# laclouis5/StructureDetector

Measured on AMD Instinct MI355X. Metric: images/sec (train fwd+bwd) and decode us/img at 512x512, higher is better.
Workload: dtype f32

## Files before the change

### include/sdnet_hip.h

```cpp
#ifndef SDNET_HIP_H
#define SDNET_HIP_H

#include <stddef.h>
#include <stdint.h>

#ifdef __cplusplus
extern "C" {
#endif

#define SD_ERR_INVALID   (-1)
#define SD_ERR_WORKSPACE (-2)
#define SD_ERR_ALIGN     (-3)

#define SD_MAX_TOPK 1024

typedef void* sd_stream_t;

int         sd_version(void);
const char* sd_last_error(void);
int         sd_build_flags(void);


int sd_clamped_sigmoid(const float* x, float* y, int64_t n, sd_stream_t stream);

// ... 137 lines not shown
int sd_loss_bwd(const sd_loss_desc* d, const float* out8, const float* grad_out, float* dhead, sd_stream_t stream);



typedef struct sd_conv_desc {
    int B, Hi, Wi, Cin, Ho, Wo, Cout, R, S, stride, pad;
} sd_conv_desc;

size_t sd_conv2d_fwd_workspace_bytes(const sd_conv_desc* d);
int sd_conv2d_fwd(const float* x_nhwc, const float* w_krsc, float* y_nhwc, const sd_conv_desc* d,
                  const float* scale, const float* shift, const float* residual, int res_up2, int relu,
                  void* workspace, size_t workspace_bytes, sd_stream_t stream);
size_t sd_conv2d_stem_fwd_workspace_bytes(const sd_conv_desc* d);
int sd_conv2d_stem_fwd(const float* x_nchw, const float* w_krsc, void* y_nhwc, const sd_conv_desc* d,
                       const float* scale, const float* shift, int relu, int out_bf16, void* workspace,
                       size_t workspace_bytes, sd_stream_t stream);

int    sd_conv2d_fwd_sb_supported(const sd_conv_desc* d, int bf16);
size_t sd_conv2d_fwd_sb_workspace_bytes(const sd_conv_desc* d, int bf16);
size_t sd_conv2d_fwd_sb_state_bytes(const sd_conv_desc* d, int bf16);
int sd_conv2d_fwd_sb(const void* x_nhwc, const void* w_krsc, void* y_nhwc, const sd_conv_desc* d, const float* scale, const float* shift,
                     const void* residual, int res_up2, int relu, int bf16, void* workspace, size_t workspace_bytes, void* state,
                     size_t state_bytes, sd_stream_t stream);

size_t sd_conv2d_stem_fwd_bn_stats_workspace_bytes(const sd_conv_desc* d);
int sd_conv2d_stem_fwd_bn_stats(const float* x_nchw, const float* w, float* y, const sd_conv_desc* d, float eps, float momentum,
                                float* running_mean, float* running_var, float* mean, float* invstd, void* workspace,
                                size_t workspace_bytes, sd_stream_t stream);

size_t sd_conv2d_fwd_bn_stats_workspace_bytes(const sd_conv_desc* d);
int sd_conv2d_fwd_bn_stats(const float* x, const float* w, float* y, const sd_conv_desc* d, float eps, float momentum,
                           float* running_mean, float* running_var, float* mean, float* invstd, void* workspace,
                           size_t workspace_bytes, sd_stream_t stream);
int sd_bn_finalize_scratch_rows(int rows);
int sd_bn_finalize_stats(const float* partial, int rows, int64_t M, int C, float eps, float momentum, float* running_mean,
                         float* running_var, float* mean, float* invstd, float* scratch, sd_stream_t stream);

size_t sd_conv2d_dgrad_bn_reduce_workspace_bytes(const sd_conv_desc* d);
int sd_conv2d_dgrad_bn_reduce(const float* dy, const float* w_t, float* dx, const sd_conv_desc* d, const float* residual,
                              const float* bn_x, const float* bn_y, int relu, const float* mean, const float* invstd,
                              const float* gamma, const float* beta, float* dgamma, float* dbeta, int accumulate,
                              float* means_out, void* workspace, size_t workspace_bytes, sd_stream_t stream);
int sd_bn_bwd_finalize(const float* partial, int rows, int64_t M, int C, float* dgamma, float* dbeta, int accumulate,
                       float* means_out, float* scratch, sd_stream_t stream);
int sd_bn_bwd_apply(const float* dy, const float* x, const float* y, int relu, int64_t M, int C, const float* mean,
                    const float* invstd, const float* gamma, const float* beta, const float* means, float* dx, float* g_out,
                    sd_stream_t stream);

int sd_set_option(const char* name, int value);

const char* sd_conv2d_kernel_name(const sd_conv_desc* d, int pass);

int sd_cast_f32_to_bf16(const float* x, void* y_bf16, int64_t n, sd_stream_t stream);
size_t sd_conv2d_fwd_bf16_workspace_bytes(const sd_conv_desc* d);
int sd_conv2d_fwd_bf16(const void* x_nhwc_bf16, const void* w_krsc_bf16, void* y_nhwc_bf16, const sd_conv_desc* d,
                       const float* scale, const float* shift, const void* residual_bf16, int res_up2, int relu,
                       void* workspace, size_t workspace_bytes, sd_stream_t stream);
int sd_maxpool3x3s2_fwd_bf16(const void* x_bf16, void* y_bf16, int B, int Hi, int Wi, int C, sd_stream_t stream);
int sd_stem_bn_relu_maxpool_fwd_bf16(const float* x_nchw, const float* w, const float* scale, const float* shift, void* y_bf16,
                                     const sd_conv_desc* d, sd_stream_t stream);

int sd_cast_bf16_to_f32(const void* x_bf16, float* y, int64_t n, sd_stream_t stream);
size_t sd_conv2d_fwd_bf16_bn_stats_workspace_bytes(const sd_conv_desc* d);
int sd_conv2d_fwd_bf16_bn_stats(const void* x_nhwc_bf16, const void* w_krsc_bf16, void* y_nhwc_bf16, const sd_conv_desc* d, float eps,
                                float momentum, float* running_mean, float* running_var, float* mean, float* invstd,
                                void* workspace, size_t workspace_bytes, sd_stream_t stream);
int sd_conv2d_stem_fwd_bn_stats_bf16mm(const float* x_nchw, const float* w, float* y, const sd_conv_desc* d, float eps, float momentum,
                                       float* running_mean, float* running_var, float* mean, float* invstd,
                                       void* workspace, size_t workspace_bytes, sd_stream_t stream);
int sd_conv2d_stem_fwd_bn_stats_bf16(const float* x_nchw, const float* w, void* y_bf16, const sd_conv_desc* d, float eps, float momentum,
                                     float* running_mean, float* running_var, float* mean, float* invstd, void* workspace,
                                     size_t workspace_bytes, sd_stream_t stream);
int sd_bn_relu_maxpool_fwd_bf16(const void* x_bf16, int B, int Hi, int Wi, int C, const float* mean, const float* invstd, const float* gamma,
                                const float* beta, void* y_pool_bf16, uint8_t* idx, sd_stream_t stream);
int sd_maxpool_bn_relu_bwd_bf16(const void* dpool_bf16, const uint8_t* idx, const void* x_bf16, int B, int Hi, int Wi, int C, const float* mean,
                                const float* invstd, const float* gamma, const float* beta, float* dx, float* dgamma, float* dbeta, int accumulate,
                                void* workspace, size_t workspace_bytes, sd_stream_t stream);
int sd_maxpool_bn_relu_bwd_bf16_dx16(const void* dpool_bf16, const uint8_t* idx, const void* x_bf16, int B, int Hi, int Wi, int C, const float* mean,
                                     const float* invstd, const float* gamma, const float* beta, void* dx_bf16, float* dgamma, float* dbeta,
                                     int accumulate, void* workspace, size_t workspace_bytes, sd_stream_t stream);
int sd_conv2d_transpose_weights_bf16(const float* w, void* w_t_bf16, int Cout, int taps, int Cin, sd_stream_t stream);

int sd_conv2d_fwd_bf16_head_supported(const sd_conv_desc* d, int head_co);
size_t sd_head_split_bf16_bytes(void);
int sd_head_split_bf16(const float* head_w, const float* head_bias, int head_co, void* prepared, sd_stream_t stream);
int sd_conv2d_fwd_bf16_head(const void* x_bf16, const void* w_bf16, const sd_conv_desc* d, const float* scale, const float* shift, int relu,
                            const void* head_prepared, int head_co, float* head_y, sd_stream_t stream);
int sd_conv2d_dgrad_bf16(const void* dy_bf16, const void* w_t_bf16, void* dx_bf16, const sd_conv_desc* d, const void* residual_bf16,
                         int res_mode, sd_stream_t stream);
size_t sd_conv2d_wgrad_bf16_workspace_bytes(const sd_conv_desc* d);
int sd_conv2d_wgrad_bf16(const void* dy_bf16, const void* x_nhwc_bf16, float* dw_krsc, const sd_conv_desc* d, int accumulate,
                         void* workspace, size_t workspace_bytes, sd_stream_t stream);
int sd_bn_apply_bf16(const void* x, void* y, int64_t M, int C, const float* mean, const float* invstd, const float* gamma,
                     const float* beta, const void* residual, int relu, uint8_t* relu_mask_out, sd_stream_t stream);
int sd_bn_bwd_bf16(const void* dy, const void* x, const void* y, int relu, int64_t M, int C, const float* mean, const float* invstd,
                   const float* gamma, const float* beta, void* dx, void* g_out, float* dgamma, float* dbeta, int accumulate,
                   void* workspace, size_t workspace_bytes, sd_stream_t stream);
int sd_bn_train_stats_bf16(const void* x, int64_t M, int C, float eps, float momentum, float* running_mean, float* running_var,
                           float* mean, float* invstd, void* workspace, size_t workspace_bytes, sd_stream_t stream);
int sd_col_sum_bf16(const void* x, int64_t M, int C, float* out, int accumulate, void* workspace, size_t workspace_bytes, sd_stream_t stream);
int sd_upsample2x_bwd_bf16(const void* dy, const void* add, void* dx, int B, int H, int W, int C, sd_stream_t stream);
int sd_head_fwd_bf16(const void* x_nhwc_bf16, const float* w, const float* bias, float* y_nchw, int B, int HW, int C,
                     int Co, sd_stream_t stream);
int sd_conv2d_dgrad(const float* dy_nhwc, const float* w_t, float* dx_nhwc, const sd_conv_desc* d,
                    const float* residual, sd_stream_t stream);
int sd_conv2d_dgrad_half_res(const float* dy, const float* w_t, float* dx, const sd_conv_desc* d, const float* residual_half,
                             sd_stream_t stream);
int sd_conv2d_transpose_weights(const float* w, float* w_t, int Cout, int taps, int Cin, sd_stream_t stream);
int sd_conv2d_transpose_weights_batched(const float* w_base, void* w_t_base, const int* table, int nconv, int total_blocks, int out_bf16,
                                        sd_stream_t stream);
size_t sd_conv2d_wgrad_workspace_bytes(const sd_conv_desc* d);
int sd_conv2d_wgrad(const float* dy_nhwc, const float* x_nhwc, float* dw_krsc, const sd_conv_desc* d,
                    int accumulate, void* workspace, size_t workspace_bytes, sd_stream_t stream);
size_t sd_conv2d_stem_wgrad_workspace_bytes(const sd_conv_desc* d);
int sd_conv2d_stem_wgrad(const float* dy_nhwc, const float* x_nchw, float* dw_krsc, const sd_conv_desc* d,
                         int accumulate, void* workspace, size_t workspace_bytes, sd_stream_t stream);
int sd_conv2d_stem_wgrad_bf16mm(const float* dy, const float* x_nchw, float* dw, const sd_conv_desc* d, int accumulate, void* workspace,
                                size_t workspace_bytes, sd_stream_t stream);
int sd_conv2d_stem_wgrad_bf16(const void* dy_bf16, const float* x_nchw, float* dw, const sd_conv_desc* d, int accumulate, void* workspace,
                              size_t workspace_bytes, sd_stream_t stream);

size_t sd_col_reduce_workspace_bytes(int64_t M, int C);
int sd_bn_train_stats(const float* x, int64_t M, int C, float eps, float momentum, float* running_mean,
                      float* running_var, float* mean, float* invstd, void* workspace, size_t workspace_bytes,
                      sd_stream_t stream);
int sd_bn_apply(const float* x, float* y, int64_t M, int C, const float* mean, const float* invstd,
                const float* gamma, const float* beta, const float* residual, int relu, uint8_t* relu_mask_out,
                sd_stream_t stream);
int sd_bn_fold(const float* gamma, const float* beta, const float* running_mean, const float* running_var,
               float eps, int C, float* scale, float* shift, sd_stream_t stream);
int sd_bn_bwd(const float* dy, const float* x, const float* y, int relu, int64_t M, int C, const float* mean,
              const float* invstd, const float* gamma, const float* beta, float* dx, float* g_out, float* dgamma,
              float* dbeta, int accumulate, void* workspace, size_t workspace_bytes, sd_stream_t stream);
int sd_col_sum(const float* x, int64_t M, int C, float* out, int accumulate, void* workspace,
               size_t workspace_bytes, sd_stream_t stream);

int sd_maxpool3x3s2_fwd(const float* x, float* y, uint8_t* idx, int B, int Hi, int Wi, int C, sd_stream_t stream);
int sd_maxpool3x3s2_bwd(const float* dy, const uint8_t* idx, float* dx, int B, int Hi, int Wi, int C, sd_stream_t stream);
int sd_bn_relu_maxpool_fwd(const float* x, int B, int Hi, int Wi, int C, const float* mean, const float* invstd, const float* gamma,
                           const float* beta, float* y_pool, uint8_t* idx, sd_stream_t stream);
int sd_maxpool_bn_relu_bwd(const float* dpool, const uint8_t* idx, const float* x, int B, int Hi, int Wi, int C, const float* mean,
                           const float* invstd, const float* gamma, const float* beta, float* dx, float* dgamma, float* dbeta,
                           int accumulate, void* workspace, size_t workspace_bytes, sd_stream_t stream);
int sd_upsample2x_bwd(const float* dy, const float* add, float* dx, int B, int H, int W, int C, sd_stream_t stream);

#define SD_HEAD_MAX_CO 256
int sd_head_fwd(const float* x_nhwc, const float* w, const float* bias, float* y_nchw, int B, int HW, int C, int Co,
                sd_stream_t stream);
size_t sd_head_bwd_workspace_bytes(int B, int HW, int C, int Co);
int sd_head_bwd(const float* dy_nchw, const float* x_nhwc, const float* w, float* dx_nhwc, float* dw, float* dbias,
                int B, int HW, int C, int Co, int accumulate, void* workspace, size_t workspace_bytes, sd_stream_t stream);
int sd_head_bwd_bf16(const float* dy, const void* x_bf16, const float* w, void* dx_bf16, float* dw, float* dbias, int B, int HW, int C, int Co,
                     int accumulate, void* workspace, size_t workspace_bytes, sd_stream_t stream);

int sd_adam_step(float* param, const float* grad, float* exp_avg, float* exp_avg_sq, int64_t n, int step,
                 float lr, float beta1, float beta2, float eps, float grad_scale, sd_stream_t stream);

#define SD_OPTIM_STATUS_BYTES 16
size_t sd_grad_sumsq_workspace_bytes(int64_t n);
int sd_grad_sumsq(const float* grad, int64_t n, void* workspace, size_t workspace_bytes, sd_stream_t stream);
int sd_optim_step(float* param, const float* grad, float* exp_avg, float* exp_avg_sq, int64_t n, int step,
                  float lr, float beta1, float beta2, float eps, float grad_scale, float weight_decay,
                  const uint8_t* decay_mask, float max_norm, const void* partials, int npartials, float* ema,
                  float ema_decay, void* status, sd_stream_t stream);

#define SD_COMM_ID_BYTES 128
int sd_allreduce_unique_id(void* id_out);
int sd_allreduce_init(const void* id, int rank, int world, void** comm_out);
int sd_allreduce_run(void* comm, float* buf, int64_t count, sd_stream_t stream);
int sd_allreduce_destroy(void* comm);

int sd_comm_sim_copy(const void* src, void* dst, size_t src_bytes, size_t move_bytes, int workgroups, float gbps, sd_stream_t stream);

double sd_mfma_bf16_stream_flops(int iters);
int    sd_mfma_bf16_stream(const void* operands64k, float* out, int iters, sd_stream_t stream);

int sd_bn_stats_from_sums(const double* sums, int C, float eps, float momentum, float* running_mean, float* running_var, float* mean,
                          float* invstd, sd_stream_t stream);
int sd_bn_bwd_means_from_sums(const double* sums, int C, float* means_out, sd_stream_t stream);
int sd_bn_stats_sums(const float* partial, int rows, int64_t M, int C, double* sums, float* scratch, sd_stream_t stream);
int sd_bn_bwd_sums(const float* partial, int rows, int64_t M, int C, float* dgamma, float* dbeta, int accumulate, double* sums,
                   float* scratch, sd_stream_t stream);
int sd_bn_train_sums(const float* x, int64_t M, int C, double* sums, void* workspace, size_t workspace_bytes, sd_stream_t stream);
int sd_bn_train_sums_bf16(const void* x, int64_t M, int C, double* sums, void* workspace, size_t workspace_bytes, sd_stream_t stream);
int sd_conv2d_fwd_bn_stats_rows(const sd_conv_desc* d, int bf16);
int sd_conv2d_fwd_bn_sums(const float* x, const float* w, float* y, const sd_conv_desc* d, double* sums, void* workspace,
                          size_t workspace_bytes, sd_stream_t stream);
int sd_conv2d_fwd_bf16_bn_sums(const void* x, const void* w, void* y, const sd_conv_desc* d, double* sums, void* workspace,
                               size_t workspace_bytes, sd_stream_t stream);
int sd_conv2d_stem_fwd_bn_sums(const float* x_nchw, const float* w, float* y, const sd_conv_desc* d, double* sums, void* workspace,
                               size_t workspace_bytes, sd_stream_t stream);
int sd_conv2d_stem_fwd_bn_sums_bf16mm(const float* x_nchw, const float* w, float* y, const sd_conv_desc* d, double* sums, void* workspace,
                                      size_t workspace_bytes, sd_stream_t stream);
int sd_conv2d_stem_fwd_bn_sums_bf16(const float* x_nchw, const float* w, void* y_bf16, const sd_conv_desc* d, double* sums, void* workspace,
                                    size_t workspace_bytes, sd_stream_t stream);
int sd_conv2d_dgrad_bn_reduce_sums(const float* dy, const float* w_t, float* dx, const sd_conv_desc* d, const float* residual,
                                   const float* bn_x, const float* bn_y, int relu, const float* mean, const float* invstd,
                                   const float* gamma, const float* beta, float* dgamma, float* dbeta, int accumulate,
                                   double* sums, void* workspace, size_t workspace_bytes, sd_stream_t stream);
int sd_bn_bwd_reduce(const float* dy, const float* x, const float* y, int relu, int64_t M, int C, const float* mean, const float* invstd,
                     const float* gamma, const float* beta, float* dgamma, float* dbeta, int accumulate, double* sums, void* workspace,
                     size_t workspace_bytes, sd_stream_t stream);
int sd_bn_bwd_reduce_bf16(const void* dy, const void* x, const void* y, int relu, int64_t M, int C, const float* mean, const float* invstd,
                          const float* gamma, const float* beta, float* dgamma, float* dbeta, int accumulate, double* sums, void* workspace,
                          size_t workspace_bytes, sd_stream_t stream);
int sd_bn_bwd_apply_bf16(const void* dy, const void* x, const void* y, int relu, int64_t M, int C, const float* mean, const float* invstd,
                         const float* gamma, const float* beta, const float* means, void* dx, void* g_out, sd_stream_t stream);
int sd_maxpool_bn_relu_bwd_reduce(const float* dpool, const uint8_t* idx, const float* x, int B, int Hi, int Wi, int C, const float* mean,
                                  const float* invstd, const float* gamma, const float* beta, float* dgamma, float* dbeta, int accumulate,
                                  double* sums, void* workspace, size_t workspace_bytes, sd_stream_t stream);
int sd_maxpool_bn_relu_bwd_reduce_bf16(const void* dpool_bf16, const uint8_t* idx, const void* x_bf16, int B, int Hi, int Wi, int C,
                                       const float* mean, const float* invstd, const float* gamma, const float* beta, float* dgamma,
                                       float* dbeta, int accumulate, double* sums, void* workspace, size_t workspace_bytes, sd_stream_t stream);
int sd_maxpool_bn_relu_bwd_apply(const float* dpool, const uint8_t* idx, const float* x, int B, int Hi, int Wi, int C, const float* mean,
                                 const float* invstd, const float* gamma, const float* beta, const float* means, float* dx, sd_stream_t stream);
int sd_maxpool_bn_relu_bwd_apply_bf16(const void* dpool_bf16, const uint8_t* idx, const void* x_bf16, int B, int Hi, int Wi, int C,
                                      const float* mean, const float* invstd, const float* gamma, const float* beta, const float* means, float* dx,
                                      sd_stream_t stream);
int sd_maxpool_bn_relu_bwd_apply_bf16_dx16(const void* dpool_bf16, const uint8_t* idx, const void* x_bf16, int B, int Hi, int Wi, int C,
                                           const float* mean, const float* invstd, const float* gamma, const float* beta, const float* means,
                                           void* dx_bf16, sd_stream_t stream);

int         sd_range_enabled(void);
const char* sd_range_library(void);
int         sd_range_push(const char* name);
int         sd_range_pop(void);
int         sd_range_mark(const char* name);

#ifdef __cplusplus
}
#endif
#endif
```

### structuredetector_amd/_lib.py

```python
from __future__ import annotations

import ctypes as C
import os
from pathlib import Path

import torch

_HERE = Path(__file__).resolve().parent
LIB_PATH = Path(os.environ.get("SDNET_HIP_LIB", _HERE / "csrc" / "libsdnet_hip.so"))

_lib = None

c_f32p = C.c_void_p
c_i64 = C.c_int64
c_int = C.c_int
c_float = C.c_float
c_size = C.c_size_t
c_vp = C.c_void_p


class SdError(RuntimeError):
    pass


class LossDesc(C.Structure):
    _fields_ = [
        ("anchor_hm", c_vp), ("a_sb", c_i64), ("a_sc", c_i64),
        ("part_hm", c_vp), ("p_sb", c_i64), ("p_sc", c_i64),
        ("offsets", c_vp), ("o_sb", c_i64), ("o_sc", c_i64),
        ("embeddings", c_vp), ("e_sb", c_i64), ("e_sc", c_i64),
        ("t_anchor_hm", c_vp), ("ta_sb", c_i64), ("ta_sc", c_i64),
        ("t_part_hm", c_vp), ("tp_sb", c_i64), ("tp_sc", c_i64),
        ("anchor_inds", c_vp), ("part_inds", c_vp),
        ("anchor_offsets", c_vp), ("part_offsets", c_vp), ("t_embeddings", c_vp),
        ("anchor_mask", c_vp), ("part_mask", c_vp),
        ("B", c_int), ("M", c_int), ("N", c_int), ("h", c_int), ("w", c_int), ("K", c_int), ("P", c_int),
        ("hm_loss_fn", c_int),
        ("hm_weight", c_float), ("offset_weight", c_float), ("embedding_weight", c_float),
    ]


class ConvDesc(C.Structure):
    _fields_ = [(n, c_int) for n in ("B", "Hi", "Wi", "Cin", "Ho", "Wo", "Cout", "R", "S", "stride", "pad")]


_MAP = [c_vp, c_i64, c_i64]
_PEAK_OUT = [c_vp, c_vp, c_vp, c_vp, c_vp]

_SIGNATURES = {
    "sd_version": (c_int, []),
    "sd_last_error": (C.c_char_p, []),
    "sd_build_flags": (c_int, []),
    "sd_clamped_sigmoid": (c_int, [c_vp, c_vp, c_i64, c_vp]),
    "sd_nms5": (c_int, _MAP + [c_vp, c_int, c_int, c_int, c_int, c_int, c_vp]),
    "sd_topk_workspace_bytes": (c_size, [c_int] * 5),
    "sd_topk": (c_int, _MAP + [c_int] * 5 + _PEAK_OUT + [c_vp, c_size, c_vp]),
    "sd_transpose_and_gather": (c_int, _MAP + [c_int, c_int, c_i64, c_vp, c_int, c_vp, c_vp]),
    "sd_hypot": (c_int, [c_vp, c_vp, c_i64, c_vp]),
    "sd_decode_peaks_workspace_bytes": (c_size, [c_int] * 5),
    "sd_decode_peaks": (c_int, _MAP + [c_int] * 5 + _PEAK_OUT + [c_vp, c_size, c_vp]),
    "sd_decode_workspace_bytes": (c_size, [c_int] * 7),
    "sd_decode_packed_words": (c_size, [c_int] * 3),
    "sd_decode": (c_int, _MAP * 4 + [c_int] * 7 + [c_float, c_float, c_int, c_vp, c_vp, c_size, c_vp]),
    "sd_decode_state_bytes": (c_size, [c_int] * 5),
    "sd_decode_fused_supported": (c_int, [c_int] * 7),
    "sd_decode_fused_recommended": (c_int, [c_int] * 8),
    "sd_stream_synchronize": (c_int, [c_vp]),
    "sd_selfcheck_sigmoid": (c_int, [c_vp, c_vp]),
    "sd_decode_fused_workspace_bytes": (c_size, [c_int] * 7),
    "sd_decode_fused": (c_int, _MAP * 4 + [c_int] * 7 + [c_float, c_float, c_int, c_vp, c_vp, c_size, c_vp, c_size, c_vp]),
    "sd_decode_group": (c_int, [c_vp] * 6 + _MAP * 2 + [c_int] * 5 + [c_float, c_float, c_vp, c_vp]),
    "sd_tta_views": (c_int, [c_vp, c_vp, c_int, c_int, c_int, c_int, c_vp, c_vp]),
    "sd_tta_merge_nms": (c_int, _MAP + [c_vp, c_int, c_int, c_int, c_int, c_int, c_vp, c_vp]),
    "sd_tta_scale_merge_nms": (c_int, [c_vp] * 6 + [c_int] * 6 + [c_vp, c_vp]),
    "sd_preprocess_workspace_bytes": (c_size, [c_int] * 4),
    "sd_preprocess_images": (c_int, [c_vp] + [c_int] * 5 + [c_vp, c_vp, c_int, c_vp, c_vp, c_int, c_vp, C.POINTER(c_float), C.POINTER(c_float),
                                                c_vp, c_vp, c_size, c_vp]),
    "sd_preprocess_jitter_workspace_bytes": (c_size, [c_int] * 5),
    "sd_preprocess_images_jitter": (c_int, [c_vp] + [c_int] * 5 + [c_vp, c_vp, c_int, c_vp, c_vp, c_int, c_vp, c_vp, c_vp, C.POINTER(c_float), C.POINTER(c_float),
                                            c_vp, c_vp, c_size, c_vp]),
    "sd_preprocess_images_list": (c_int, [c_vp] + [c_int] * 5 + [c_vp, c_vp, c_int, c_vp, c_vp, c_int, c_vp, C.POINTER(c_float), C.POINTER(c_float),
                                                     c_vp, c_vp, c_size, c_vp]),
    "sd_preprocess_images_list_jitter": (c_int, [c_vp] + [c_int] * 5 + [c_vp, c_vp, c_int, c_vp, c_vp, c_int, c_vp, c_vp, c_vp, C.POINTER(c_float),
                                                            C.POINTER(c_float), c_vp, c_vp, c_size, c_vp]),
    "sd_preprocess_affine_workspace_bytes": (c_size, [c_int] * 5),
    "sd_preprocess_images_affine": (c_int, [c_vp] + [c_int] * 5 + [c_vp, c_vp, c_int, c_vp, c_vp, c_int, c_vp, c_vp, c_vp, c_vp, C.POINTER(C.c_ubyte),
                                            C.POINTER(c_float), C.POINTER(c_float), c_vp, c_vp, c_size, c_vp]),
    "sd_preprocess_images_list_affine": (c_int, [c_vp] + [c_int] * 5 + [c_vp, c_vp, c_int, c_vp, c_vp, c_int, c_vp, c_vp, c_vp, c_vp, C.POINTER(C.c_ubyte),
                                                 C.POINTER(c_float), C.POINTER(c_float), c_vp, c_vp, c_size, c_vp]),
    "sd_preprocess_mosaic_workspace_bytes": (c_size, [c_int] * 5),
    "sd_preprocess_images_mosaic": (c_int, [c_vp] + [c_int] * 5 + [c_vp, c_vp, c_int, c_vp, c_vp, c_int, c_vp, c_vp, c_vp, c_vp, c_vp, c_vp,
                                            C.POINTER(C.c_ubyte), C.POINTER(c_float), C.POINTER(c_float), c_vp, c_vp, c_size, c_vp]),
    "sd_preprocess_images_list_mosaic": (c_int, [c_vp] + [c_int] * 5 + [c_vp, c_vp, c_int, c_vp, c_vp, c_int, c_vp, c_vp, c_vp, c_vp, c_vp, c_vp,
                                                 C.POINTER(C.c_ubyte), C.POINTER(c_float), C.POINTER(c_float), c_vp, c_vp, c_size, c_vp]),
    "sd_render_targets": (c_int, [c_vp, c_vp, c_vp, c_int, c_int, c_int, c_int, c_float, c_vp, c_vp]),
    "sd_loss_workspace_bytes": (c_size, [c_int] * 5),
    "sd_loss_fwd": (c_int, [C.POINTER(LossDesc), c_vp, c_vp, c_size, c_vp]),
    "sd_loss_fwd_per_image": (c_int, [C.POINTER(LossDesc), c_vp, c_vp, c_size, c_vp]),
    "sd_loss_bwd": (c_int, [C.POINTER(LossDesc), c_vp, c_vp, c_vp, c_vp]),
    "sd_conv2d_fwd_workspace_bytes": (c_size, [C.POINTER(ConvDesc)]),
    "sd_conv2d_fwd": (c_int, [c_vp, c_vp, c_vp, C.POINTER(ConvDesc), c_vp, c_vp, c_vp, c_int, c_int, c_vp, c_size, c_vp]),
    "sd_conv2d_fwd_sb_supported": (c_int, [C.POINTER(ConvDesc), c_int]),
    "sd_conv2d_fwd_sb_workspace_bytes": (c_size, [C.POINTER(ConvDesc), c_int]),
    "sd_conv2d_fwd_sb_state_bytes": (c_size, [C.POINTER(ConvDesc), c_int]),
    "sd_conv2d_fwd_sb": (c_int, [c_vp, c_vp, c_vp, C.POINTER(ConvDesc), c_vp, c_vp, c_vp, c_int, c_int, c_int, c_vp, c_size, c_vp, c_size, c_vp]),
    "sd_conv2d_stem_fwd_workspace_bytes": (c_size, [C.POINTER(ConvDesc)]),
    "sd_conv2d_stem_fwd": (c_int, [c_vp, c_vp, c_vp, C.POINTER(ConvDesc), c_vp, c_vp, c_int, c_int, c_vp, c_size, c_vp]),
    "sd_cast_f32_to_bf16": (c_int, [c_vp, c_vp, c_i64, c_vp]),
    "sd_conv2d_fwd_bf16_workspace_bytes": (c_size, [C.POINTER(ConvDesc)]),
    "sd_conv2d_fwd_bf16": (c_int, [c_vp, c_vp, c_vp, C.POINTER(ConvDesc), c_vp, c_vp, c_vp, c_int, c_int, c_vp, c_size, c_vp]),
    "sd_conv2d_fwd_bf16_head_supported": (c_int, [C.POINTER(ConvDesc), c_int]),
    "sd_head_split_bf16_bytes": (c_size, []),
    "sd_head_split_bf16": (c_int, [c_vp, c_vp, c_int, c_vp, c_vp]),
    "sd_conv2d_fwd_bf16_head": (c_int, [c_vp, c_vp, C.POINTER(ConvDesc), c_vp, c_vp, c_int, c_vp, c_int, c_vp, c_vp]),
    "sd_cast_bf16_to_f32": (c_int, [c_vp, c_vp, c_i64, c_vp]),
    "sd_conv2d_fwd_bf16_bn_stats_workspace_bytes": (c_size, [c_vp]),
    "sd_conv2d_fwd_bf16_bn_stats": (c_int, [c_vp, c_vp, c_vp, c_vp, c_float, c_float, c_vp, c_vp, c_vp, c_vp, c_vp, c_size, c_vp]),
    "sd_conv2d_wgrad_bf16_workspace_bytes": (c_size, [c_vp]),
    "sd_conv2d_wgrad_bf16": (c_int, [c_vp, c_vp, c_vp, c_vp, c_int, c_vp, c_size, c_vp]),
    "sd_conv2d_transpose_weights_bf16": (c_int, [c_vp, c_vp, c_int, c_int, c_int, c_vp]),
    "sd_conv2d_dgrad_bf16": (c_int, [c_vp, c_vp, c_vp, c_vp, c_vp, c_int, c_vp]),
    "sd_bn_apply_bf16": (c_int, [c_vp, c_vp, c_i64, c_int, c_vp, c_vp, c_vp, c_vp, c_vp, c_int, c_vp, c_vp]),
    "sd_bn_bwd_bf16": (c_int, [c_vp, c_vp, c_vp, c_int, c_i64, c_int, c_vp, c_vp, c_vp, c_vp, c_vp, c_vp, c_vp, c_vp, c_int, c_vp, c_size, c_vp]),
    "sd_bn_train_stats_bf16": (c_int, [c_vp, c_i64, c_int, c_float, c_float, c_vp, c_vp, c_vp, c_vp, c_vp, c_size, c_vp]),
    "sd_col_sum_bf16": (c_int, [c_vp, c_i64, c_int, c_vp, c_int, c_vp, c_size, c_vp]),
    "sd_upsample2x_bwd_bf16": (c_int, [c_vp, c_vp, c_vp, c_int, c_int, c_int, c_int, c_vp]),
    "sd_maxpool3x3s2_fwd_bf16": (c_int, [c_vp, c_vp, c_int, c_int, c_int, c_int, c_vp]),
    "sd_stem_bn_relu_maxpool_fwd_bf16": (c_int, [c_vp, c_vp, c_vp, c_vp, c_vp, c_vp, c_vp]),
    "sd_head_fwd_bf16": (c_int, [c_vp, c_vp, c_vp, c_vp, c_int, c_int, c_int, c_int, c_vp]),
    "sd_conv2d_dgrad": (c_int, [c_vp, c_vp, c_vp, C.POINTER(ConvDesc), c_vp, c_vp]),
    "sd_conv2d_transpose_weights": (c_int, [c_vp, c_vp, c_int, c_int, c_int, c_vp]),
    "sd_conv2d_transpose_weights_batched": (c_int, [c_vp, c_vp, c_vp, c_int, c_int, c_int, c_vp]),
    "sd_conv2d_wgrad_workspace_bytes": (c_size, [C.POINTER(ConvDesc)]),
    "sd_conv2d_wgrad": (c_int, [c_vp, c_vp, c_vp, C.POINTER(ConvDesc), c_int, c_vp, c_size, c_vp]),
    "sd_conv2d_stem_wgrad_workspace_bytes": (c_size, [C.POINTER(ConvDesc)]),
    "sd_conv2d_stem_wgrad": (c_int, [c_vp, c_vp, c_vp, C.POINTER(ConvDesc), c_int, c_vp, c_size, c_vp]),
    "sd_conv2d_stem_wgrad_bf16mm": (c_int, [c_vp, c_vp, c_vp, C.POINTER(ConvDesc), c_int, c_vp, c_size, c_vp]),
    "sd_conv2d_stem_wgrad_bf16": (c_int, [c_vp, c_vp, c_vp, C.POINTER(ConvDesc), c_int, c_vp, c_size, c_vp]),
    "sd_col_reduce_workspace_bytes": (c_size, [c_i64, c_int]),
    "sd_bn_train_stats": (c_int, [c_vp, c_i64, c_int, c_float, c_float, c_vp, c_vp, c_vp, c_vp, c_vp, c_size, c_vp]),
    "sd_bn_apply": (c_int, [c_vp, c_vp, c_i64, c_int, c_vp, c_vp, c_vp, c_vp, c_vp, c_int, c_vp, c_vp]),
    "sd_bn_fold": (c_int, [c_vp, c_vp, c_vp, c_vp, c_float, c_int, c_vp, c_vp, c_vp]),
    "sd_bn_bwd": (c_int, [c_vp, c_vp, c_vp, c_int, c_i64, c_int, c_vp, c_vp, c_vp, c_vp, c_vp, c_vp, c_vp, c_vp, c_int, c_vp, c_size, c_vp]),
    "sd_col_sum": (c_int, [c_vp, c_i64, c_int, c_vp, c_int, c_vp, c_size, c_vp]),
    "sd_maxpool3x3s2_fwd": (c_int, [c_vp, c_vp, c_vp, c_int, c_int, c_int, c_int, c_vp]),
    "sd_maxpool3x3s2_bwd": (c_int, [c_vp, c_vp, c_vp, c_int, c_int, c_int, c_int, c_vp]),
    "sd_upsample2x_bwd": (c_int, [c_vp, c_vp, c_vp, c_int, c_int, c_int, c_int, c_vp]),
    "sd_head_fwd": (c_int, [c_vp, c_vp, c_vp, c_vp, c_int, c_int, c_int, c_int, c_vp]),
    "sd_head_bwd_workspace_bytes": (c_size, [c_int] * 4),
    "sd_head_bwd": (c_int, [c_vp] * 6 + [c_int] * 5 + [c_vp, c_size, c_vp]),
    "sd_head_bwd_bf16": (c_int, [c_vp] * 6 + [c_int] * 5 + [c_vp, c_size, c_vp]),
    "sd_adam_step": (c_int, [c_vp, c_vp, c_vp, c_vp, c_i64, c_int, c_float, c_float, c_float, c_float, c_float, c_vp]),
    "sd_grad_sumsq_workspace_bytes": (c_size, [c_i64]),
    "sd_grad_sumsq": (c_int, [c_vp, c_i64, c_vp, c_size, c_vp]),
    "sd_optim_step": (c_int, [c_vp, c_vp, c_vp, c_vp, c_i64, c_int, c_float, c_float, c_float, c_float, c_float, c_float, c_vp, c_float, c_vp, c_int,
                              c_vp, c_float, c_vp, c_vp]),
    "sd_conv2d_kernel_name": (C.c_char_p, [c_vp, c_int]),
    "sd_set_option": (c_int, [C.c_char_p, c_int]),
    "sd_decode_set_option": (c_int, [C.c_char_p, c_int]),
    "sd_decode_kernel_names": (C.c_char_p, [c_int] * 9),
    "sd_conv2d_stem_fwd_bn_stats_workspace_bytes": (c_size, [c_vp]),
    "sd_conv2d_stem_fwd_bn_stats": (c_int, [c_vp, c_vp, c_vp, c_vp, c_float, c_float, c_vp, c_vp, c_vp, c_vp, c_vp, c_size, c_vp]),
    "sd_conv2d_stem_fwd_bn_stats_bf16mm": (c_int, [c_vp, c_vp, c_vp, c_vp, c_float, c_float, c_vp, c_vp, c_vp, c_vp, c_vp, c_size, c_vp]),
    "sd_conv2d_stem_fwd_bn_stats_bf16": (c_int, [c_vp, c_vp, c_vp, c_vp, c_float, c_float, c_vp, c_vp, c_vp, c_vp, c_vp, c_size, c_vp]),
    "sd_conv2d_dgrad_half_res": (c_int, [c_vp] * 6),
    "sd_bn_relu_maxpool_fwd": (c_int, [c_vp, c_int, c_int, c_int, c_int] + [c_vp] * 7),
    "sd_bn_relu_maxpool_fwd_bf16": (c_int, [c_vp, c_int, c_int, c_int, c_int] + [c_vp] * 7),
    "sd_maxpool_bn_relu_bwd": (c_int, [c_vp, c_vp, c_vp, c_int, c_int, c_int, c_int] + [c_vp] * 7 + [c_int, c_vp, c_size, c_vp]),
    "sd_maxpool_bn_relu_bwd_bf16": (c_int, [c_vp, c_vp, c_vp, c_int, c_int, c_int, c_int] + [c_vp] * 7 + [c_int, c_vp, c_size, c_vp]),
    "sd_maxpool_bn_relu_bwd_bf16_dx16": (c_int, [c_vp, c_vp, c_vp, c_int, c_int, c_int, c_int] + [c_vp] * 7 + [c_int, c_vp, c_size, c_vp]),
    "sd_conv2d_fwd_bn_stats_workspace_bytes": (c_size, [c_vp]),
    "sd_conv2d_fwd_bn_stats": (c_int, [c_vp, c_vp, c_vp, c_vp, c_float, c_float, c_vp, c_vp, c_vp, c_vp, c_vp, c_size, c_vp]),
    "sd_conv2d_dgrad_bn_reduce_workspace_bytes": (c_size, [c_vp]),
    "sd_conv2d_dgrad_bn_reduce": (c_int, [c_vp] * 5 + [c_vp, c_vp, c_int] + [c_vp] * 6 + [c_int, c_vp, c_vp, c_size, c_vp]),
    "sd_bn_bwd_finalize": (c_int, [c_vp, c_int, c_i64, c_int, c_vp, c_vp, c_int, c_vp, c_vp, c_vp]),
    "sd_bn_bwd_apply": (c_int, [c_vp, c_vp, c_vp, c_int, c_i64, c_int] + [c_vp] * 8),
    "sd_bn_finalize_scratch_rows": (c_int, [c_int]),
    "sd_bn_finalize_stats": (c_int, [c_vp, c_int, c_i64, c_int, c_float, c_float, c_vp, c_vp, c_vp, c_vp, c_vp, c_vp]),
    "sd_bn_stats_from_sums": (c_int, [c_vp, c_int, c_float, c_float, c_vp, c_vp, c_vp, c_vp, c_vp]),
    "sd_bn_bwd_means_from_sums": (c_int, [c_vp, c_int, c_vp, c_vp]),
    "sd_bn_stats_sums": (c_int, [c_vp, c_int, c_i64, c_int, c_vp, c_vp, c_vp]),
    "sd_bn_bwd_sums": (c_int, [c_vp, c_int, c_i64, c_int, c_vp, c_vp, c_int, c_vp, c_vp, c_vp]),
    "sd_bn_train_sums": (c_int, [c_vp, c_i64, c_int, c_vp, c_vp, c_size, c_vp]),
    "sd_bn_train_sums_bf16": (c_int, [c_vp, c_i64, c_int, c_vp, c_vp, c_size, c_vp]),
    "sd_conv2d_fwd_bn_stats_rows": (c_int, [c_vp, c_int]),
    "sd_conv2d_fwd_bn_sums": (c_int, [c_vp, c_vp, c_vp, c_vp, c_vp, c_vp, c_size, c_vp]),
    "sd_conv2d_fwd_bf16_bn_sums": (c_int, [c_vp, c_vp, c_vp, c_vp, c_vp, c_vp, c_size, c_vp]),
    "sd_conv2d_stem_fwd_bn_sums": (c_int, [c_vp, c_vp, c_vp, c_vp, c_vp, c_vp, c_size, c_vp]),
    "sd_conv2d_stem_fwd_bn_sums_bf16mm": (c_int, [c_vp, c_vp, c_vp, c_vp, c_vp, c_vp, c_size, c_vp]),
    "sd_conv2d_stem_fwd_bn_sums_bf16": (c_int, [c_vp, c_vp, c_vp, c_vp, c_vp, c_vp, c_size, c_vp]),
    "sd_conv2d_dgrad_bn_reduce_sums": (c_int, [c_vp, c_vp, c_vp, c_vp, c_vp, c_vp, c_vp, c_int] + [c_vp] * 6 + [c_int, c_vp, c_vp, c_size, c_vp]),
    "sd_bn_bwd_reduce": (c_int, [c_vp, c_vp, c_vp, c_int, c_i64, c_int] + [c_vp] * 6 + [c_int, c_vp, c_vp, c_size, c_vp]),
    "sd_bn_bwd_reduce_bf16": (c_int, [c_vp, c_vp, c_vp, c_int, c_i64, c_int] + [c_vp] * 6 + [c_int, c_vp, c_vp, c_size, c_vp]),
    "sd_bn_bwd_apply_bf16": (c_int, [c_vp, c_vp, c_vp, c_int, c_i64, c_int] + [c_vp] * 8),
    "sd_maxpool_bn_relu_bwd_reduce": (c_int, [c_vp, c_vp, c_vp, c_int, c_int, c_int, c_int] + [c_vp] * 6 + [c_int, c_vp, c_vp, c_size, c_vp]),
    "sd_maxpool_bn_relu_bwd_reduce_bf16": (c_int, [c_vp, c_vp, c_vp, c_int, c_int, c_int, c_int] + [c_vp] * 6 + [c_int, c_vp, c_vp, c_size, c_vp]),
    "sd_maxpool_bn_relu_bwd_apply": (c_int, [c_vp, c_vp, c_vp, c_int, c_int, c_int, c_int] + [c_vp] * 7),
    "sd_maxpool_bn_relu_bwd_apply_bf16": (c_int, [c_vp, c_vp, c_vp, c_int, c_int, c_int, c_int] + [c_vp] * 7),
    "sd_maxpool_bn_relu_bwd_apply_bf16_dx16": (c_int, [c_vp, c_vp, c_vp, c_int, c_int, c_int, c_int] + [c_vp] * 7),
    "sd_allreduce_unique_id": (c_int, [c_vp]),
    "sd_allreduce_init": (c_int, [c_vp, c_int, c_int, C.POINTER(c_vp)]),
    "sd_allreduce_run": (c_int, [c_vp, c_vp, c_i64, c_vp]),
    "sd_allreduce_destroy": (c_int, [c_vp]),
    "sd_mfma_bf16_stream_flops": (C.c_double, [c_int]),
    "sd_mfma_bf16_stream": (c_int, [c_vp, c_vp, c_int, c_vp]),
    "sd_comm_sim_copy": (c_int, [c_vp, c_vp, c_size, c_size, c_int, c_float, c_vp]),
    "sd_range_enabled": (c_int, []),
    "sd_range_library": (C.c_char_p, []),
    "sd_range_push": (c_int, [C.c_char_p]),
    "sd_range_pop": (c_int, []),
    "sd_range_mark": (c_int, [C.c_char_p]),
}


def declared_symbols():
    return sorted(_SIGNATURES)


def lib():
    global _lib
    if _lib is None:
        if not LIB_PATH.exists():
            raise SdError(
                f"{LIB_PATH} not found: build it with `python -c 'import __graft_entry__ as g; g.build()'` "
                f"(or `make -C {LIB_PATH.parent}`); structuredetector_amd has no CPU / eager fallback.")
        handle = C.CDLL(str(LIB_PATH))
        for name, (res, args) in _SIGNATURES.items():
            fn = getattr(handle, name)
            fn.restype = res
            fn.argtypes = args
        flags = handle.sd_build_flags()
        if flags and os.environ.get("SDNET_ALLOW_ABLATION") != "1":
            raise SdError(f"{LIB_PATH} is a timing-only ablation build (sd_build_flags = {flags}: SD_ABLATE_* switches make the conv "
                          "kernels compute wrong results on purpose); rebuild without EXTRA=-DSD_ABLATE_... "
                          "(set SDNET_ALLOW_ABLATION=1 only for timing experiments)")
        _lib = handle
    return _lib


def check(rc: int, what: str = ""):
    if rc != 0:
        msg = lib().sd_last_error().decode(errors="replace")
        raise SdError(f"{what or 'libsdnet_hip'} failed (code {rc}): {msg}")


def stream() -> int:
    try:
        return torch._C._cuda_getCurrentRawStream(torch.cuda.current_device())
    except AttributeError:
        return torch.cuda.current_stream().cuda_stream


def require_cuda(*tensors):
    for t in tensors:
        if not t.is_cuda:
            raise SdError("structuredetector_amd ops need tensors on the GPU (device 'cuda'); got a "
                          f"{t.device} tensor and there is no CPU fallback")


def map_view(t: torch.Tensor):
    if t.dtype != torch.float32:
        t = t.float()
    B, Cc, h, w = t.shape
    s0, s1, s2, s3 = t.stride()
    ptr = t.data_ptr()
    if not (s3 == 1 and s2 == w and s1 >= h * w and (B == 1 or s0 >= h * w) and s1 % 4 == 0 and s0 % 4 == 0 and ptr % 16 == 0):
        t = t.contiguous()
        s0, s1 = t.stride(0), t.stride(1)
        ptr = t.data_ptr()
    return t, ptr, s0, s1


_ws_cache: dict = {}


def workspace(nbytes: int, device) -> torch.Tensor:
    key = (device.index if device.index is not None else torch.cuda.current_device(), stream())
    buf = _ws_cache.get(key)
    if buf is None or buf.numel() < nbytes:
        buf = torch.empty(max(nbytes, 1 << 20), dtype=torch.uint8, device=device)
        _ws_cache[key] = buf
    return buf


_state_cache: dict = {}


def zero_state(nbytes: int, device, tag: str = "conv") -> torch.Tensor:
    key = (device.index if device.index is not None else torch.cuda.current_device(), stream(), tag)
    buf = _state_cache.get(key)
    if buf is None or buf.numel() < nbytes:
        if buf is not None:
            torch.cuda.current_stream().synchronize()
        buf = torch.zeros(max(nbytes, 1 << 16), dtype=torch.uint8, device=device)
        _state_cache[key] = buf
    return buf
```

### structuredetector_amd/csrc/sd_nn.hip

```cpp
#include "sd_common.h"
#include "sd_mfma.h"
#include <type_traits>

namespace sd {

constexpr int RED_ROWS_PER_BLOCK = 256;

template <int MODE, typename T = float>
__global__ __launch_bounds__(256) void k_col_reduce(const T* __restrict__ a, const T* __restrict__ b, const T* __restrict__ y,
                                                     const float* __restrict__ mean, const float* __restrict__ invstd,
                                                     const float* __restrict__ gamma, const float* __restrict__ beta, int relu,
                                                     int64_t M, int C, float* __restrict__ partial, int rpb) {
    __shared__ float4 red[2][256];
    const int cols = C >> 2;
    const int lanes = 256 / cols;
    const int col = threadIdx.x % cols, rl = threadIdx.x / cols;
    const int64_t r0 = (int64_t)blockIdx.x * rpb;
    const int64_t r1 = min(r0 + rpb, M);
    float4 s0 = make_float4(0.f, 0.f, 0.f, 0.f), s1 = s0;
    float4 mu = s0, is = s0, ga = s0, be = s0;
    if (MODE == 1 && rl < lanes) {
        mu = reinterpret_cast<const float4*>(mean)[col];
        is = reinterpret_cast<const float4*>(invstd)[col];
        if (relu == 2) { ga = reinterpret_cast<const float4*>(gamma)[col]; be = reinterpret_cast<const float4*>(beta)[col]; }
    }
    if (rl < lanes) {
#pragma unroll 4
        for (int64_t r = r0 + rl; r < r1; r += lanes) {
            const float4 v = ld4(a, r * cols + col);
            if (MODE == 0) {
                s0.x += v.x; s0.y += v.y; s0.z += v.z; s0.w += v.w;
                s1.x += v.x * v.x; s1.y += v.y * v.y; s1.z += v.z * v.z; s1.w += v.w * v.w;
            } else if (MODE == 2) {
                s0.x += v.x; s0.y += v.y; s0.z += v.z; s0.w += v.w;
            } else {
                float4 g = v;
                const float4 xv = ld4(b, r * cols + col);
                if (relu == 1) {
                    const float4 yy = ld4(y, r * cols + col);
                    g.x = yy.x > 0.f ? g.x : 0.f; g.y = yy.y > 0.f ? g.y : 0.f;
                    g.z = yy.z > 0.f ? g.z : 0.f; g.w = yy.w > 0.f ? g.w : 0.f;
                } else if (relu == 2) {
                    g.x = ((xv.x - mu.x) * is.x * ga.x + be.x) > 0.f ? g.x : 0.f; g.y = ((xv.y - mu.y) * is.y * ga.y + be.y) > 0.f ? g.y : 0.f;
                    g.z = ((xv.z - mu.z) * is.z * ga.z + be.z) > 0.f ? g.z : 0.f; g.w = ((xv.w - mu.w) * is.w * ga.w + be.w) > 0.f ? g.w : 0.f;
                } else if (relu == 3) {
                    const uint8_t mb = reinterpret_cast<const uint8_t*>(y)[r * cols + col];
                    g.x = (mb & 1) ? g.x : 0.f; g.y = (mb & 2) ? g.y : 0.f; g.z = (mb & 4) ? g.z : 0.f; g.w = (mb & 8) ? g.w : 0.f;
                }
                s0.x += g.x; s0.y += g.y; s0.z += g.z; s0.w += g.w;
                s1.x += g.x * ((xv.x - mu.x) * is.x); s1.y += g.y * ((xv.y - mu.y) * is.y);
                s1.z += g.z * ((xv.z - mu.z) * is.z); s1.w += g.w * ((xv.w - mu.w) * is.w);
            }
        }
    }
    red[0][threadIdx.x] = s0;
    red[1][threadIdx.x] = s1;
    __syncthreads();
    if (rl == 0) {
        for (int l = 1; l < lanes; ++l) {
            const float4 u = red[0][l * cols + col], w = red[1][l * cols + col];
            s0.x += u.x; s0.y += u.y; s0.z += u.z; s0.w += u.w;
            s1.x += w.x; s1.y += w.y; s1.z += w.z; s1.w += w.w;
        }
        float* dst = partial + (int64_t)blockIdx.x * 2 * C;
        reinterpret_cast<float4*>(dst)[col] = s0;
        reinterpret_cast<float4*>(dst + C)[col] = s1;
    }
}

__global__ __launch_bounds__(256) void k_rows_fold(const float* __restrict__ in, int rows, int W, int slab, float* __restrict__ out) {
    __shared__ float4 red[256];
    const int cols = W >> 2, lanes = 256 / cols;
    const int col = threadIdx.x % cols, rl = threadIdx.x / cols;
    const int r0 = blockIdx.x * slab, r1 = min(r0 + slab, rows);
    float4 s = make_float4(0.f, 0.f, 0.f, 0.f);
    if (rl < lanes) {
#pragma unroll 4
        for (int r = r0 + rl; r < r1; r += lanes) {
            const float4 v = reinterpret_cast<const float4*>(in + (int64_t)r * W)[col];
            s.x += v.x; s.y += v.y; s.z += v.z; s.w += v.w;
        }
    }
    red[threadIdx.x] = s;
    __syncthreads();
    if (rl == 0) {
        for (int l = 1; l < lanes; ++l) { const float4 u = red[l * cols + col]; s.x += u.x; s.y += u.y; s.z += u.z; s.w += u.w; }
        reinterpret_cast<float4*>(out + (int64_t)blockIdx.x * W)[col] = s;
    }
}

__device__ __forceinline__ bool col_pair_sums(const float* __restrict__ partial, int nblocks, int C, double (&r0)[4][4], double (&r1)[4][4],
                                              double& s0, double& s1) {
    const int lc = threadIdx.x & 3, lr = threadIdx.x >> 2;
    const int c = blockIdx.x * 4 + lc;
    s0 = 0.0; s1 = 0.0;
    if (c < C) {
        double t0[8] = {0, 0, 0, 0, 0, 0, 0, 0}, t1[8] = {0, 0, 0, 0, 0, 0, 0, 0};
        for (int b = lr; b < nblocks; b += 64 * 8) {
            float v0[8], v1[8];
#pragma unroll
            for (int u = 0; u < 8; ++u) {
                const int row = b + 64 * u;
                const int64_t o = (int64_t)(row < nblocks ? row : 0) * 2 * C + c;
                v0[u] = partial[o];
                v1[u] = partial[o + C];
            }
#pragma unroll
            for (int u = 0; u < 8; ++u) {
                const bool ok = b + 64 * u < nblocks;
                t0[u] += ok ? (double)v0[u] : 0.0; t1[u] += ok ? (double)v1[u] : 0.0;
            }
        }
        s0 = ((t0[0] + t0[1]) + (t0[2] + t0[3])) + ((t0[4] + t0[5]) + (t0[6] + t0[7]));
        s1 = ((t1[0] + t1[1]) + (t1[2] + t1[3])) + ((t1[4] + t1[5]) + (t1[6] + t1[7]));
    }
#pragma unroll
    for (int o = 4; o < 64; o <<= 1) { s0 += __shfl_xor(s0, o); s1 += __shfl_xor(s1, o); }
    if ((threadIdx.x & 63) < 4) { r0[threadIdx.x >> 6][lc] = s0; r1[threadIdx.x >> 6][lc] = s1; }
    __syncthreads();
    if (lr != 0 || c >= C) return false;
    s0 = (r0[0][lc] + r0[1][lc]) + (r0[2][lc] + r0[3][lc]);
    s1 = (r1[0][lc] + r1[1][lc]) + (r1[2][lc] + r1[3][lc]);
    return true;
}

__device__ __forceinline__ void bn_stats_tail(double s0, double s1, double M, float eps, float momentum, int c, float* __restrict__ mean_out,
                                              float* __restrict__ invstd_out, float* __restrict__ run_mean, float* __restrict__ run_var) {
    const double mean = s0 / M;
    const double var = fmax(s1 / M - mean * mean, 0.0);
    mean_out[c] = (float)mean;
    invstd_out[c] = (float)(1.0 / sqrt(var + (double)eps));
    if (run_mean) {
        const double unb = M > 1.0 ? var * M / (M - 1.0) : var;
        run_mean[c] = (float)((1.0 - momentum) * run_mean[c] + momentum * mean);
        run_var[c] = (float)((1.0 - momentum) * run_var[c] + momentum * unb);
    }
}

template <int FIN>
__global__ __launch_bounds__(256) void k_col_finalize(const float* __restrict__ partial, int nblocks, int C, double M, float eps,
                                                       float momentum, float* __restrict__ out0, float* __restrict__ out1,
                                                       float* __restrict__ run_mean, float* __restrict__ run_var,
                                                       float* __restrict__ aux0, float* __restrict__ aux1, int accumulate) {
    __shared__ double r0[4][4], r1[4][4];
    double s0, s1;
    if (!col_pair_sums(partial, nblocks, C, r0, r1, s0, s1)) return;
    const int c = blockIdx.x * 4 + (threadIdx.x & 3);
    if (FIN == 0) {
        bn_stats_tail(s0, s1, M, eps, momentum, c, out0, out1, run_mean, run_var);
    } else if (FIN == 1) {
        out0[c] = (accumulate ? out0[c] : 0.f) + (float)s1;
        out1[c] = (accumulate ? out1[c] : 0.f) + (float)s0;
        aux0[c] = (float)(s0 / M);
        aux1[c] = (float)(s1 / M);
    } else {
        out0[c] = (accumulate ? out0[c] : 0.f) + (float)s0;
    }
}

template <int FIN>
__global__ __launch_bounds__(256) void k_col_sums(const float* __restrict__ partial, int nblocks, int C, double M, float* __restrict__ dgamma,
                                                   float* __restrict__ dbeta, int accumulate, double* __restrict__ sums) {
    __shared__ double r0[4][4], r1[4][4];
    double s0, s1;
    if (!col_pair_sums(partial, nblocks, C, r0, r1, s0, s1)) return;
    const int c = blockIdx.x * 4 + (threadIdx.x & 3);
    sums[c] = s0;
    sums[C + c] = s1;
    if (c == 0) sums[2 * C] = M;
    if (FIN == 1) {
        dgamma[c] = (accumulate ? dgamma[c] : 0.f) + (float)s1;
        dbeta[c] = (accumulate ? dbeta[c] : 0.f) + (float)s0;
    }
}

__global__ __launch_bounds__(256) void k_bn_stats_from_sums(const double* __restrict__ sums, int C, float eps, float momentum,
                                                             float* __restrict__ mean, float* __restrict__ invstd,
                                                             float* __restrict__ run_mean, float* __restrict__ run_var) {
    const int c = blockIdx.x * 256 + threadIdx.x;
    if (c >= C) return;
    bn_stats_tail(sums[c], sums[C + c], sums[2 * C], eps, momentum, c, mean, invstd, run_mean, run_var);
}

__global__ __launch_bounds__(256) void k_bn_bwd_means_from_sums(const double* __restrict__ sums, int C, float* __restrict__ means) {
    const int c = blockIdx.x * 256 + threadIdx.x;
    if (c >= C) return;
    const double M = sums[2 * C];
    means[c] = (float)(sums[c] / M);
    means[C + c] = (float)(sums[C + c] / M);
}

template <typename T>
__global__ __launch_bounds__(256) void k_bn_apply(const T* __restrict__ x, T* __restrict__ y, int64_t n4, int C,
                                                   const float* __restrict__ mean, const float* __restrict__ invstd,
                                                   const float* __restrict__ gamma, const float* __restrict__ beta,
                                                   const T* __restrict__ res, int relu, uint8_t* __restrict__ mask) {
    const int64_t stride = (int64_t)gridDim.x * 256;
    const int cols = C >> 2;
    const bool fixed = stride % cols == 0;
    const int col0 = (int)(((int64_t)blockIdx.x * 256 + threadIdx.x) % cols);
    float4 mu = reinterpret_cast<const float4*>(mean)[col0], is = reinterpret_cast<const float4*>(invstd)[col0];
    float4 g = reinterpret_cast<const float4*>(gamma)[col0], b = reinterpret_cast<const float4*>(beta)[col0];
    for (int64_t i = (int64_t)blockIdx.x * 256 + threadIdx.x; i < n4; i += stride) {
        const float4 v = ld4(x, i);
        if (!fixed) {
            const int col = (int)(i % cols);
            mu = reinterpret_cast<const float4*>(mean)[col]; is = reinterpret_cast<const float4*>(invstd)[col];
            g = reinterpret_cast<const float4*>(gamma)[col]; b = reinterpret_cast<const float4*>(beta)[col];
        }
        float4 o;
        o.x = (v.x - mu.x) * is.x * g.x + b.x; o.y = (v.y - mu.y) * is.y * g.y + b.y;
        o.z = (v.z - mu.z) * is.z * g.z + b.z; o.w = (v.w - mu.w) * is.w * g.w + b.w;
        if (res) {
            const float4 r = ld4(res, i);
            o.x += r.x; o.y += r.y; o.z += r.z; o.w += r.w;
        }
        if (mask) mask[i] = (uint8_t)((o.x > 0.f ? 1 : 0) | (o.y > 0.f ? 2 : 0) | (o.z > 0.f ? 4 : 0) | (o.w > 0.f ? 8 : 0));
        if (relu) { o.x = fmaxf(o.x, 0.f); o.y = fmaxf(o.y, 0.f); o.z = fmaxf(o.z, 0.f); o.w = fmaxf(o.w, 0.f); }
        st4(y, i, o);
    }
}

__global__ __launch_bounds__(256) void k_bn_fold(const float* gamma, const float* beta, const float* rm, const float* rv, float eps,
                                                  int C, float* scale, float* shift) {
    const int c = blockIdx.x * 256 + threadIdx.x;
    if (c >= C) return;
    const float s = gamma[c] / sqrtf(rv[c] + eps);
    scale[c] = s;
    shift[c] = beta[c] - rm[c] * s;
}

template <typename T>
__global__ __launch_bounds__(256) void k_bn_bwd_apply(const T* __restrict__ dy, const T* __restrict__ x, const T* __restrict__ y,
                                                       int relu, int64_t n4, int C, const float* __restrict__ mean,
                                                       const float* __restrict__ invstd, const float* __restrict__ gamma,
                                                       const float* __restrict__ beta, const float* __restrict__ mg,
                                                       const float* __restrict__ mgx, T* __restrict__ dx, T* __restrict__ g_out) {
    const int64_t stride = (int64_t)gridDim.x * 256;
    const int cols = C >> 2;
    const bool fixed = stride % cols == 0;
    const int col0 = (int)(((int64_t)blockIdx.x * 256 + threadIdx.x) % cols);
    float4 mu = reinterpret_cast<const float4*>(mean)[col0], is = reinterpret_cast<const float4*>(invstd)[col0];
    float4 ga = reinterpret_cast<const float4*>(gamma)[col0];
    float4 be = relu == 2 ? reinterpret_cast<const float4*>(beta)[col0] : make_float4(0.f, 0.f, 0.f, 0.f);
    float4 a = reinterpret_cast<const float4*>(mg)[col0], b = reinterpret_cast<const float4*>(mgx)[col0];
    for (int64_t i = (int64_t)blockIdx.x * 256 + threadIdx.x; i < n4; i += stride) {
        float4 g = ld4(dy, i);
        const float4 xv = ld4(x, i);
        if (!fixed) {
            const int col = (int)(i % cols);
            mu = reinterpret_cast<const float4*>(mean)[col]; is = reinterpret_cast<const float4*>(invstd)[col];
            ga = reinterpret_cast<const float4*>(gamma)[col];
            if (relu == 2) be = reinterpret_cast<const float4*>(beta)[col];
            a = reinterpret_cast<const float4*>(mg)[col]; b = reinterpret_cast<const float4*>(mgx)[col];
        }
        if (relu == 1) {
            const float4 yy = ld4(y, i);
            g.x = yy.x > 0.f ? g.x : 0.f; g.y = yy.y > 0.f ? g.y : 0.f; g.z = yy.z > 0.f ? g.z : 0.f; g.w = yy.w > 0.f ? g.w : 0.f;
        } else if (relu == 3) {
            const uint8_t mb = reinterpret_cast<const uint8_t*>(y)[i];
            g.x = (mb & 1) ? g.x : 0.f; g.y = (mb & 2) ? g.y : 0.f; g.z = (mb & 4) ? g.z : 0.f; g.w = (mb & 8) ? g.w : 0.f;
        } else if (relu == 2) {
            g.x = ((xv.x - mu.x) * is.x * ga.x + be.x) > 0.f ? g.x : 0.f; g.y = ((xv.y - mu.y) * is.y * ga.y + be.y) > 0.f ? g.y : 0.f;
            g.z = ((xv.z - mu.z) * is.z * ga.z + be.z) > 0.f ? g.z : 0.f; g.w = ((xv.w - mu.w) * is.w * ga.w + be.w) > 0.f ? g.w : 0.f;
        }
        float4 o;
        o.x = ga.x * is.x * (g.x - a.x - (xv.x - mu.x) * is.x * b.x);
        o.y = ga.y * is.y * (g.y - a.y - (xv.y - mu.y) * is.y * b.y);
        o.z = ga.z * is.z * (g.z - a.z - (xv.z - mu.z) * is.z * b.z);
        o.w = ga.w * is.w * (g.w - a.w - (xv.w - mu.w) * is.w * b.w);
        st4(dx, i, o);
        if (g_out) st4(g_out, i, g);
    }
}

__global__ __launch_bounds__(256) void k_maxpool_fwd(const float* __restrict__ x, float* __restrict__ y, uint8_t* __restrict__ idx, int B,
                                                      int Hi, int Wi, int Ho, int Wo, int C) {
    const int cols = C >> 2;
    const int64_t n4 = (int64_t)B * Ho * Wo * cols;
    const int64_t i = (int64_t)blockIdx.x * 256 + threadIdx.x;
    if (i >= n4) return;
    const int col = (int)(i % cols);
    int64_t t = i / cols;
    const int ox = (int)(t % Wo); t /= Wo;
    const int oy = (int)(t % Ho);
    const int b = (int)(t / Ho);
    float4 m = make_float4(-INFINITY, -INFINITY, -INFINITY, -INFINITY);
    uchar4 w = make_uchar4(0, 0, 0, 0);
#pragma unroll
    for (int r = 0; r < 3; ++r) {
#pragma unroll
        for (int s = 0; s < 3; ++s) {
            const int iy = oy * 2 - 1 + r, ix = ox * 2 - 1 + s;
            if (iy < 0 || iy >= Hi || ix < 0 || ix >= Wi) continue;
            const float4 v = reinterpret_cast<const float4*>(x + (((int64_t)b * Hi + iy) * Wi + ix) * C)[col];
            const uint8_t tap = (uint8_t)(r * 3 + s);
            if (v.x > m.x) { m.x = v.x; w.x = tap; }
            if (v.y > m.y) { m.y = v.y; w.y = tap; }
            if (v.z > m.z) { m.z = v.z; w.z = tap; }
            if (v.w > m.w) { m.w = v.w; w.w = tap; }
        }
    }
    reinterpret_cast<float4*>(y)[i] = m;
    reinterpret_cast<uchar4*>(idx)[i] = w;
}

__global__ __launch_bounds__(256) void k_maxpool_bwd(const float* __restrict__ dy, const uint8_t* __restrict__ idx, float* __restrict__ dx,
                                                      int B, int Hi, int Wi, int Ho, int Wo, int C) {
    const int cols = C >> 2;
    const int64_t n4 = (int64_t)B * Hi * Wi * cols;
    const int64_t i = (int64_t)blockIdx.x * 256 + threadIdx.x;
    if (i >= n4) return;
    const int col = (int)(i % cols);
    int64_t t = i / cols;
    const int ix = (int)(t % Wi); t /= Wi;
    const int iy = (int)(t % Hi);
    const int b = (int)(t / Hi);
    float4 acc = make_float4(0.f, 0.f, 0.f, 0.f);
    for (int oy = (iy + 1) / 2 - ((iy + 1) % 2 == 0 ? 1 : 0); oy <= (iy + 1) / 2; ++oy) {
        if (oy < 0 || oy >= Ho) continue;
        const int r = iy - (oy * 2 - 1);
        if (r < 0 || r > 2) continue;
        for (int ox = (ix + 1) / 2 - ((ix + 1) % 2 == 0 ? 1 : 0); ox <= (ix + 1) / 2; ++ox) {
            if (ox < 0 || ox >= Wo) continue;
            const int s = ix - (ox * 2 - 1);
            if (s < 0 || s > 2) continue;
            const int64_t o = (((int64_t)b * Ho + oy) * Wo + ox) * cols + col;
            const uchar4 w = reinterpret_cast<const uchar4*>(idx)[o];
            const float4 g = reinterpret_cast<const float4*>(dy)[o];
            const uint8_t tap = (uint8_t)(r * 3 + s);
            if (w.x == tap) acc.x += g.x;
            if (w.y == tap) acc.y += g.y;
            if (w.z == tap) acc.z += g.z;
            if (w.w == tap) acc.w += g.w;
        }
    }
    reinterpret_cast<float4*>(dx)[i] = acc;
}

template <typename XT, typename PT>
__global__ __launch_bounds__(256) void k_bn_relu_maxpool_fwd(const XT* __restrict__ x, const float* __restrict__ mean,
                                                              const float* __restrict__ invstd, const float* __restrict__ gamma,
                                                              const float* __restrict__ beta, PT* __restrict__ y,
                                                              uint8_t* __restrict__ idx, int B, int Hi, int Wi, int Ho, int Wo, int C) {
    const int cols = C >> 2;
    const int64_t n4 = (int64_t)B * Ho * Wo * cols;
    const int64_t i = (int64_t)blockIdx.x * 256 + threadIdx.x;
    if (i >= n4) return;
    const int col = (int)(i % cols);
    int64_t t = i / cols;
    const int ox = (int)(t % Wo); t /= Wo;
    const int oy = (int)(t % Ho);
    const int b = (int)(t / Ho);
    const float4 mu = reinterpret_cast<const float4*>(mean)[col], is = reinterpret_cast<const float4*>(invstd)[col];
    const float4 ga = reinterpret_cast<const float4*>(gamma)[col], be = reinterpret_cast<const float4*>(beta)[col];
    float4 m = make_float4(-INFINITY, -INFINITY, -INFINITY, -INFINITY);
    uchar4 w = make_uchar4(0, 0, 0, 0);
#pragma unroll
    for (int r = 0; r < 3; ++r) {
#pragma unroll
        for (int s = 0; s < 3; ++s) {
            const int iy = oy * 2 - 1 + r, ix = ox * 2 - 1 + s;
            if (iy < 0 || iy >= Hi || ix < 0 || ix >= Wi) continue;
            const float4 xv = ld4(x, (((int64_t)b * Hi + iy) * Wi + ix) * cols + col);
            float4 v;
            v.x = fmaxf((xv.x - mu.x) * is.x * ga.x + be.x, 0.f); v.y = fmaxf((xv.y - mu.y) * is.y * ga.y + be.y, 0.f);
            v.z = fmaxf((xv.z - mu.z) * is.z * ga.z + be.z, 0.f); v.w = fmaxf((xv.w - mu.w) * is.w * ga.w + be.w, 0.f);
            const uint8_t tap = (uint8_t)(r * 3 + s);
            if (v.x > m.x) { m.x = v.x; w.x = tap; }
            if (v.y > m.y) { m.y = v.y; w.y = tap; }
            if (v.z > m.z) { m.z = v.z; w.z = tap; }
            if (v.w > m.w) { m.w = v.w; w.w = tap; }
        }
    }
    st4(y, i, m);
    reinterpret_cast<uchar4*>(idx)[i] = w;
}

template <int VEC> struct PoolVec { float v[VEC]; };
__device__ __forceinline__ PoolVec<4> pool_ld(const float* p, int64_t e) {
    const float4 r = *reinterpret_cast<const float4*>(p + e);
    return PoolVec<4>{{r.x, r.y, r.z, r.w}};
}
__device__ __forceinline__ PoolVec<8> pool_ld(const uint16_t* p, int64_t e) {
    const uint4 r = *reinterpret_cast<const uint4*>(p + e);
    return PoolVec<8>{{bf16_to_f32((uint16_t)(r.x & 0xffff)), bf16_to_f32((uint16_t)(r.x >> 16)), bf16_to_f32((uint16_t)(r.y & 0xffff)), bf16_to_f32((uint16_t)(r.y >> 16)),
                       bf16_to_f32((uint16_t)(r.z & 0xffff)), bf16_to_f32((uint16_t)(r.z >> 16)), bf16_to_f32((uint16_t)(r.w & 0xffff)), bf16_to_f32((uint16_t)(r.w >> 16))}};
}
__device__ __forceinline__ void pool_st(float* p, int64_t e, const PoolVec<4>& m) { *reinterpret_cast<float4*>(p + e) = make_float4(m.v[0], m.v[1], m.v[2], m.v[3]); }
__device__ __forceinline__ void pool_st(uint16_t* p, int64_t e, const PoolVec<8>& m) {
    uint4 r;
    r.x = (uint32_t)f32_to_bf16(m.v[0]) | ((uint32_t)f32_to_bf16(m.v[1]) << 16); r.y = (uint32_t)f32_to_bf16(m.v[2]) | ((uint32_t)f32_to_bf16(m.v[3]) << 16);
    r.z = (uint32_t)f32_to_bf16(m.v[4]) | ((uint32_t)f32_to_bf16(m.v[5]) << 16); r.w = (uint32_t)f32_to_bf16(m.v[6]) | ((uint32_t)f32_to_bf16(m.v[7]) << 16);
    *reinterpret_cast<uint4*>(p + e) = r;
}
template <typename XT, typename PT, int VEC>
__global__ __launch_bounds__(256) void k_bn_relu_maxpool_fwd_pair(const XT* __restrict__ x, const float* __restrict__ mean,
                                                                   const float* __restrict__ invstd, const float* __restrict__ gamma,
                                                                   const float* __restrict__ beta, PT* __restrict__ y,
                                                                   uint8_t* __restrict__ idx, int B, int Hi, int Wi, int Ho, int Wo, int C) {
    const int cols = C / VEC, Wp = Wo >> 1;
    const int64_t n = (int64_t)B * Ho * Wp * cols;
    const int64_t i = (int64_t)blockIdx.x * 256 + threadIdx.x;
    if (i >= n) return;
    const int col = (int)(i % cols);
    int64_t t = i / cols;
    const int oxp = (int)(t % Wp); t /= Wp;
    const int oy = (int)(t % Ho);
    const int b = (int)(t / Ho);
    float mu[VEC], is[VEC], ga[VEC], be[VEC];
#pragma unroll
    for (int k = 0; k < VEC; ++k) { mu[k] = mean[col * VEC + k]; is[k] = invstd[col * VEC + k]; ga[k] = gamma[col * VEC + k]; be[k] = beta[col * VEC + k]; }
    PoolVec<VEC> m0, m1;
    uint8_t w0[VEC], w1[VEC];
#pragma unroll
    for (int k = 0; k < VEC; ++k) { m0.v[k] = m1.v[k] = -INFINITY; w0[k] = w1[k] = 0; }
#pragma unroll
    for (int r = 0; r < 3; ++r) {
        const int iy = oy * 2 - 1 + r;
        if (iy < 0 || iy >= Hi) continue;
#pragma unroll
        for (int c = 0; c < 5; ++c) {
            const int ix = oxp * 4 - 1 + c;
            if (ix < 0 || ix >= Wi) continue;
            const PoolVec<VEC> xv = pool_ld(x, (((int64_t)b * Hi + iy) * Wi + ix) * C + col * VEC);
#pragma unroll
// ... 144 lines not shown
    const float4 ga = reinterpret_cast<const float4*>(gamma)[col], be = reinterpret_cast<const float4*>(beta)[col];
    const float4 a = reinterpret_cast<const float4*>(mg)[col], bb = reinterpret_cast<const float4*>(mgx)[col];
    const int64_t p00 = (((int64_t)b * Hi + 2 * k) * Wi + 2 * j) * cols + col;
    const int64_t off[4] = {p00, p00 + cols, p00 + (int64_t)Wi * cols, p00 + (int64_t)(Wi + 1) * cols};
    float4 xv[4], g[4];
#pragma unroll
    for (int u = 0; u < 4; ++u) xv[u] = ld4(x, off[u]);
    pool_relu_grad_quad(dpool, idx, b, k, j, col, cols, Ho, Wo, xv, mu, is, ga, be, g);
#pragma unroll
    for (int u = 0; u < 4; ++u) {
        float4 o;
        o.x = ga.x * is.x * (g[u].x - a.x - (xv[u].x - mu.x) * is.x * bb.x);
        o.y = ga.y * is.y * (g[u].y - a.y - (xv[u].y - mu.y) * is.y * bb.y);
        o.z = ga.z * is.z * (g[u].z - a.z - (xv[u].z - mu.z) * is.z * bb.z);
        o.w = ga.w * is.w * (g[u].w - a.w - (xv[u].w - mu.w) * is.w * bb.w);
        st4(dx, off[u], o);
    }
}
#undef SD_ADD4

__global__ __launch_bounds__(256) void k_pool_bn_bwd_reduce(const float* __restrict__ dpool, const uint8_t* __restrict__ idx,
                                                             const float* __restrict__ x, const float* __restrict__ mean,
                                                             const float* __restrict__ invstd, const float* __restrict__ gamma,
                                                             const float* __restrict__ beta, int Hi, int Wi, int Ho, int Wo, int64_t M,
                                                             int C, float* __restrict__ partial) {
    __shared__ float4 red[2][256];
    const int cols = C >> 2, lanes = 256 / cols;
    const int col = threadIdx.x % cols, rl = threadIdx.x / cols;
    const int64_t r0 = (int64_t)blockIdx.x * RED_ROWS_PER_BLOCK, r1 = min(r0 + RED_ROWS_PER_BLOCK, M);
    float4 s0 = make_float4(0.f, 0.f, 0.f, 0.f), s1 = s0;
    if (rl < lanes) {
        const float4 mu = reinterpret_cast<const float4*>(mean)[col], is = reinterpret_cast<const float4*>(invstd)[col];
        const float4 ga = reinterpret_cast<const float4*>(gamma)[col], be = reinterpret_cast<const float4*>(beta)[col];
        for (int64_t r = r0 + rl; r < r1; r += lanes) {
            const int ix = (int)(r % Wi);
            const int64_t t = r / Wi;
            const int iy = (int)(t % Hi), b = (int)(t / Hi);
            const float4 xv = reinterpret_cast<const float4*>(x + r * C)[col];
            const float4 g = pool_relu_grad(dpool, idx, b, iy, ix, col, cols, Ho, Wo, xv, mu, is, ga, be);
            s0.x += g.x; s0.y += g.y; s0.z += g.z; s0.w += g.w;
            s1.x += g.x * ((xv.x - mu.x) * is.x); s1.y += g.y * ((xv.y - mu.y) * is.y);
            s1.z += g.z * ((xv.z - mu.z) * is.z); s1.w += g.w * ((xv.w - mu.w) * is.w);
        }
    }
    red[0][threadIdx.x] = s0;
    red[1][threadIdx.x] = s1;
    __syncthreads();
    if (rl == 0) {
        for (int l = 1; l < lanes; ++l) {
            const float4 u = red[0][l * cols + col], w = red[1][l * cols + col];
            s0.x += u.x; s0.y += u.y; s0.z += u.z; s0.w += u.w;
            s1.x += w.x; s1.y += w.y; s1.z += w.z; s1.w += w.w;
        }
        float* dst = partial + (int64_t)blockIdx.x * 2 * C;
        reinterpret_cast<float4*>(dst)[col] = s0;
        reinterpret_cast<float4*>(dst + C)[col] = s1;
    }
}

__global__ __launch_bounds__(256) void k_pool_bn_bwd_apply(const float* __restrict__ dpool, const uint8_t* __restrict__ idx,
                                                            const float* __restrict__ x, const float* __restrict__ mean,
                                                            const float* __restrict__ invstd, const float* __restrict__ gamma,
                                                            const float* __restrict__ beta, const float* __restrict__ mg,
                                                            const float* __restrict__ mgx, int Hi, int Wi, int Ho, int Wo, int64_t n4, int C,
                                                            float* __restrict__ dx) {
    const int64_t i = (int64_t)blockIdx.x * 256 + threadIdx.x;
    if (i >= n4) return;
    const int cols = C >> 2;
    const int col = (int)(i % cols);
    const int64_t r = i / cols;
    const int ix = (int)(r % Wi);
    const int64_t t = r / Wi;
    const int iy = (int)(t % Hi), b = (int)(t / Hi);
    const float4 mu = reinterpret_cast<const float4*>(mean)[col], is = reinterpret_cast<const float4*>(invstd)[col];
    const float4 ga = reinterpret_cast<const float4*>(gamma)[col], be = reinterpret_cast<const float4*>(beta)[col];
    const float4 xv = reinterpret_cast<const float4*>(x)[i];
    const float4 g = pool_relu_grad(dpool, idx, b, iy, ix, col, cols, Ho, Wo, xv, mu, is, ga, be);
    const float4 a = reinterpret_cast<const float4*>(mg)[col], bb = reinterpret_cast<const float4*>(mgx)[col];
    float4 o;
    o.x = ga.x * is.x * (g.x - a.x - (xv.x - mu.x) * is.x * bb.x);
    o.y = ga.y * is.y * (g.y - a.y - (xv.y - mu.y) * is.y * bb.y);
    o.z = ga.z * is.z * (g.z - a.z - (xv.z - mu.z) * is.z * bb.z);
    o.w = ga.w * is.w * (g.w - a.w - (xv.w - mu.w) * is.w * bb.w);
    reinterpret_cast<float4*>(dx)[i] = o;
}

template <typename T>
__global__ __launch_bounds__(256) void k_up2_bwd(const T* __restrict__ dy, const T* __restrict__ add, T* __restrict__ dx, int B,
                                                  int H, int W, int C) {
    const int cols = C >> 2;
    const int64_t n4 = (int64_t)B * H * W * cols;
    const int64_t i = (int64_t)blockIdx.x * 256 + threadIdx.x;
    if (i >= n4) return;
    const int col = (int)(i % cols);
    int64_t t = i / cols;
    const int x = (int)(t % W); t /= W;
    const int y = (int)(t % H);
    const int b = (int)(t / H);
    const T* base = dy + (((int64_t)b * 2 * H + 2 * y) * 2 * W + 2 * x) * C;
    const float4 v0 = ld4(base, col), v1 = ld4(base + C, col);
    const float4 v2 = ld4(base + (int64_t)2 * W * C, col);
    const float4 v3 = ld4(base + (int64_t)2 * W * C + C, col);
    float4 o = make_float4(v0.x + v1.x + v2.x + v3.x, v0.y + v1.y + v2.y + v3.y, v0.z + v1.z + v2.z + v3.z, v0.w + v1.w + v2.w + v3.w);
    if (add) {
        const float4 a = ld4(add, i);
        o.x += a.x; o.y += a.y; o.z += a.z; o.w += a.w;
    }
    st4(dx, i, o);
}

__global__ __launch_bounds__(256) void k_head_fwd(const float* __restrict__ x, const float* __restrict__ w, const float* __restrict__ bias,
                                                   float* __restrict__ y, int64_t M, int HW, int C, int Co) {
    extern __shared__ __attribute__((aligned(16))) float lds[];
    const int LD = C + 4;
    float* xs = lds;
    float* ws = lds + 64 * LD;
    const int64_t m0 = (int64_t)blockIdx.x * 64;
    const int c4 = C >> 2;
    for (int i = threadIdx.x; i < 64 * c4; i += 256) {
        const int row = i / c4, col = i - row * c4;
        const int64_t m = m0 + row;
        const float4 v = m < M ? reinterpret_cast<const float4*>(x + m * C)[col] : make_float4(0.f, 0.f, 0.f, 0.f);
        *reinterpret_cast<float4*>(xs + row * LD + col * 4) = v;
    }
    for (int i = threadIdx.x; i < Co * C; i += 256) ws[i] = w[i];
    __syncthreads();
    const int px = threadIdx.x & 63, grp = threadIdx.x >> 6;
    float acc[HEAD_NARROW_MAX_CO / 4];
#pragma unroll
    for (int j = 0; j < HEAD_NARROW_MAX_CO / 4; ++j) acc[j] = 0.f;
    for (int c = 0; c < C; c += 4) {
        const float4 v = *reinterpret_cast<const float4*>(xs + px * LD + c);
#pragma unroll
        for (int j = 0; j < HEAD_NARROW_MAX_CO / 4; ++j) {
            const int co = grp + 4 * j;
            if (co < Co) {
                const float4 ww = *reinterpret_cast<const float4*>(ws + co * C + c);
                acc[j] += v.x * ww.x + v.y * ww.y + v.z * ww.z + v.w * ww.w;
            }
        }
    }
    const int64_t m = m0 + px;
    if (m < M) {
        const int64_t b = m / HW, pix = m - b * HW;
#pragma unroll
        for (int j = 0; j < HEAD_NARROW_MAX_CO / 4; ++j) {
            const int co = grp + 4 * j;
            if (co < Co) y[(b * Co + co) * HW + pix] = acc[j] + bias[co];
        }
    }
}

constexpr int HF_NST = 4;
__global__ __launch_bounds__(256) void k_head_fwd_f32_c128(const float* __restrict__ x, const float* __restrict__ w, const float* __restrict__ bias,
                                                            float* __restrict__ y, int HW, int Co, int ntiles) {
    extern __shared__ __attribute__((aligned(16))) float hf_lds[];
    const int lane = threadIdx.x & 63, wave = __builtin_amdgcn_readfirstlane(threadIdx.x >> 6);
    float* const T = hf_lds + wave * (HF_NST * 2048);
    const uint32_t t_base = lds_addr(T);
    const int row = lane & 15, kq = lane >> 4;
    f32x4 bw[8];
#pragma unroll
    for (int j = 0; j < 8; ++j) {
        bw[j] = f32x4{0.f, 0.f, 0.f, 0.f};
        if (row < Co) bw[j] = *reinterpret_cast<const f32x4*>(w + row * 128 + 16 * j + 4 * kq);
    }
    const float bv = row < Co ? bias[row] : 0.f;
    const int nwaves = gridDim.x * 4;
    const int dr = lane >> 5, dsl = lane & 31;
#define HF_ISSUE(t_, st_)                                                                                          \
    {                                                                                                              \
        const int64_t m0_ = (int64_t)min((t_), ntiles - 1) * 16;                                                  \
        _Pragma("unroll") for (int d = 0; d < 8; ++d) {                                                            \
            const int r = 2 * d + dr;                                                                              \
            lds_dma16(x + (m0_ + r) * 128 + ((dsl ^ (r & 15)) << 2), T + (st_) * 2048 + d * 256);                   \
        }                                                                                                          \
    }
    int tile = blockIdx.x * 4 + wave;
#pragma unroll
    for (int s = 0; s < HF_NST - 1; ++s) HF_ISSUE(tile + s * nwaves, s)
    int stage = 0;
    for (; tile < ntiles; tile += nwaves) {
        const int nst = stage == 0 ? HF_NST - 1 : stage - 1;
        HF_ISSUE(tile + (HF_NST - 1) * nwaves, nst)
        wait_vmcnt<8 * (HF_NST - 1)>();
        const uint32_t a0 = t_base + (uint32_t)stage * 8192u + (uint32_t)row * 512u;
        f32x4 a[8];
#pragma unroll
        for (int j = 0; j < 8; ++j) a[j] = lds_read128_async<0>(a0 + (uint32_t)(((4 * j + kq) ^ row) << 4));
        SD_LDS_WAIT4(0, a[0], a[1], a[2], a[3]);
        SD_LDS_WAIT4(0, a[4], a[5], a[6], a[7]);
        f32x4 acc0 = {0.f, 0.f, 0.f, 0.f}, acc1 = {0.f, 0.f, 0.f, 0.f};
#pragma unroll
        for (int j = 0; j < 8; j += 2)
#pragma unroll
            for (int t = 0; t < 4; ++t) {
                acc0 = __builtin_amdgcn_mfma_f32_16x16x4f32(a[j][t], bw[j][t], acc0, 0, 0, 0);
                acc1 = __builtin_amdgcn_mfma_f32_16x16x4f32(a[j + 1][t], bw[j + 1][t], acc1, 0, 0, 0);
            }
        if (row < Co) {
            const uint32_t m0 = (uint32_t)tile * 16u;
            const uint32_t b = m0 / (uint32_t)HW, pix = m0 - b * (uint32_t)HW;
            const f32x4 o = {acc0[0] + acc1[0] + bv, acc0[1] + acc1[1] + bv, acc0[2] + acc1[2] + bv, acc0[3] + acc1[3] + bv};
            *reinterpret_cast<f32x4*>(y + ((int64_t)b * Co + row) * HW + pix + 4 * kq) = o;
        }
        stage = stage + 1 == HF_NST ? 0 : stage + 1;
    }
    wait_vmcnt<0>();
#undef HF_ISSUE
}

constexpr int HEAD_WG_PIX = 1024;
template <typename T>
__global__ __launch_bounds__(256) void k_head_dgrad(const float* __restrict__ dy, const float* __restrict__ w, T* __restrict__ dx,
                                                     int64_t M, int HW, int C, int Co) {
    __shared__ float gs[HEAD_NARROW_MAX_CO][64];
    extern __shared__ __attribute__((aligned(16))) float lds[];
    float* ws = lds;
    const int64_t m0 = (int64_t)blockIdx.x * 64;
    for (int i = threadIdx.x; i < Co * 64; i += 256) {
        const int co = i >> 6, px = i & 63;
        const int64_t m = m0 + px;
        float v = 0.f;
        if (m < M) { const int64_t b = m / HW, pix = m - b * HW; v = dy[(b * Co + co) * HW + pix]; }
        gs[co][px] = v;
    }
    for (int i = threadIdx.x; i < Co * C; i += 256) ws[i] = w[i];
    __syncthreads();
    const int c4 = C >> 2;
    for (int i = threadIdx.x; i < 64 * c4; i += 256) {
        const int row = i / c4, col = i - row * c4;
        const int64_t m = m0 + row;
        if (m >= M) continue;
        float4 o = make_float4(0.f, 0.f, 0.f, 0.f);
        for (int co = 0; co < Co; ++co) {
            const float g = gs[co][row];
            const float4 ww = *reinterpret_cast<const float4*>(ws + co * C + col * 4);
            o.x += g * ww.x; o.y += g * ww.y; o.z += g * ww.z; o.w += g * ww.w;
        }
        if constexpr (sizeof(T) == 2) {
            uint2 pk;
            pk.x = (uint32_t)f32_to_bf16(o.x) | ((uint32_t)f32_to_bf16(o.y) << 16);
            pk.y = (uint32_t)f32_to_bf16(o.z) | ((uint32_t)f32_to_bf16(o.w) << 16);
            reinterpret_cast<uint2*>(dx + m * C)[col] = pk;
        } else {
            reinterpret_cast<float4*>(dx + m * C)[col] = o;
        }
    }
}

template <int CO>
__global__ __launch_bounds__(256) void k_head_wgrad_bf16(const float* __restrict__ dy, const uint16_t* __restrict__ x, float* __restrict__ partial,
                                                          int64_t M, int HW, int C, int Co) {
    __shared__ float gs[CO][64];
    __shared__ float comb[4][CO * 128];
    const int64_t mb = (int64_t)blockIdx.x * HEAD_WG_PIX;
    const int CG = C >> 3, PL = 256 / CG;
    const int cg = threadIdx.x % CG, pl = threadIdx.x / CG;
    float acc[CO][8];
#pragma unroll
    for (int j = 0; j < CO; ++j)
#pragma unroll
        for (int k = 0; k < 8; ++k) acc[j][k] = 0.f;
    float bsum = 0.f;
    for (int64_t m0 = mb; m0 < min(mb + HEAD_WG_PIX, M); m0 += 64) {
        __syncthreads();
        for (int i = threadIdx.x; i < Co * 64; i += 256) {
            const int co = i >> 6, px = i & 63;
            const int64_t m = m0 + px;
            float v = 0.f;
            if (m < M) { const int64_t b = m / HW, pix = m - b * HW; v = dy[(b * Co + co) * HW + pix]; }
            gs[co][px] = v;
        }
        __syncthreads();
        for (int p0 = 0; p0 < 64; p0 += 4 * PL) {
            uint4 xv[4];
#pragma unroll
            for (int u = 0; u < 4; ++u) {
                const int px = p0 + u * PL + pl;
                const int64_t m = m0 + px;
                xv[u] = reinterpret_cast<const uint4*>(x + (px < 64 && m < M ? m : mb) * C)[cg];
            }
#pragma unroll
            for (int u = 0; u < 4; ++u) {
                const int px = p0 + u * PL + pl;
                if (px >= 64) continue;
                const float f[8] = {__uint_as_float(xv[u].x << 16), __uint_as_float(xv[u].x & 0xffff0000u), __uint_as_float(xv[u].y << 16),
                                    __uint_as_float(xv[u].y & 0xffff0000u), __uint_as_float(xv[u].z << 16), __uint_as_float(xv[u].z & 0xffff0000u),
                                    __uint_as_float(xv[u].w << 16), __uint_as_float(xv[u].w & 0xffff0000u)};
#pragma unroll
                for (int j = 0; j < CO; ++j) {
                    if (j < Co) {
                        const float g = gs[j][px];
#pragma unroll
                        for (int k = 0; k < 8; ++k) acc[j][k] += g * f[k];
                    }
                }
            }
        }
        if (threadIdx.x < Co) {
            for (int px = 0; px < 64; ++px) bsum += gs[threadIdx.x][px];
        }
    }
    const int lane = threadIdx.x & 63, wave = threadIdx.x >> 6;
#pragma unroll
    for (int j = 0; j < CO; ++j)
#pragma unroll
        for (int k = 0; k < 8; ++k) {
            float v = acc[j][k];
            for (int o = CG; o < 64; o <<= 1) v += __shfl_xor(v, o);
            acc[j][k] = v;
        }
    if (lane < CG) {
#pragma unroll
        for (int j = 0; j < CO; ++j)
            if (j < Co) {
#pragma unroll
                for (int k = 0; k < 8; ++k) comb[wave][j * C + lane * 8 + k] = acc[j][k];
            }
    }
    __syncthreads();
    float* dst = partial + (int64_t)blockIdx.x * (Co * C + Co);
    for (int i = threadIdx.x; i < Co * C; i += 256) dst[i] = (comb[0][i] + comb[1][i]) + (comb[2][i] + comb[3][i]);
    if (threadIdx.x < Co) dst[Co * C + threadIdx.x] = bsum;
}

__global__ __launch_bounds__(256) void k_head_wgrad(const float* __restrict__ dy, const float* __restrict__ x, float* __restrict__ partial,
                                                     int64_t M, int HW, int C, int Co) {
    __shared__ float gs[HEAD_NARROW_MAX_CO][64];
    __shared__ float comb[HEAD_NARROW_MAX_CO][256];
    const int64_t mb = (int64_t)blockIdx.x * HEAD_WG_PIX;
    const int halves = max(1, 256 / C);
    const int c = threadIdx.x % C, hf = threadIdx.x / C;
    const int span = 64 / halves;
    float acc[HEAD_NARROW_MAX_CO];
#pragma unroll
    for (int j = 0; j < HEAD_NARROW_MAX_CO; ++j) acc[j] = 0.f;
    float bsum = 0.f;
    for (int64_t m0 = mb; m0 < min(mb + HEAD_WG_PIX, M); m0 += 64) {
        __syncthreads();
        for (int i = threadIdx.x; i < Co * 64; i += 256) {
            const int co = i >> 6, px = i & 63;
            const int64_t m = m0 + px;
            float v = 0.f;
            if (m < M) { const int64_t b = m / HW, pix = m - b * HW; v = dy[(b * Co + co) * HW + pix]; }
            gs[co][px] = v;
        }
        __syncthreads();
        if (hf < halves) {
            const int p0 = hf * span;
#pragma unroll 1
            for (int pb = 0; pb < span; pb += 8) {
                float xv[8];
#pragma unroll
                for (int u = 0; u < 8; ++u) {
                    const int64_t m = m0 + p0 + pb + u;
                    xv[u] = x[(m < M ? m : mb) * C + c];
                }
#pragma unroll
                for (int u = 0; u < 8; ++u)
#pragma unroll
                    for (int j = 0; j < HEAD_NARROW_MAX_CO; ++j)
                        if (j < Co) acc[j] += gs[j][p0 + pb + u] * xv[u];
            }
        }
        if (threadIdx.x < Co) {
            for (int px = 0; px < 64; ++px) bsum += gs[threadIdx.x][px];
        }
    }
    for (int j = 0; j < Co; ++j) comb[j][threadIdx.x] = (hf < halves) ? acc[j] : 0.f;
    __syncthreads();
    float* dst = partial + (int64_t)blockIdx.x * (Co * C + Co);
    if (threadIdx.x < C) {
        for (int j = 0; j < Co; ++j) {
            float t = 0.f;
            for (int h2 = 0; h2 < halves; ++h2) t += comb[j][h2 * C + threadIdx.x];
            dst[j * C + threadIdx.x] = t;
        }
    }
    if (threadIdx.x < Co) dst[Co * C + threadIdx.x] = bsum;
}

constexpr int HWG_STAGE = 2048 + 256;
__global__ __launch_bounds__(256) void k_head_wgrad_f32_c128(const float* __restrict__ dy, const float* __restrict__ x, float* __restrict__ partial,
                                                              int HW, int Co, int ntiles) {
    extern __shared__ __attribute__((aligned(16))) float hw_lds[];
    const int lane = threadIdx.x & 63, wave = __builtin_amdgcn_readfirstlane(threadIdx.x >> 6);
    float* const T = hw_lds + wave * (HF_NST * HWG_STAGE);
    const uint32_t t_base = lds_addr(T);
    const int n = lane & 15, kq = lane >> 4;
    const int gw = blockIdx.x * 4 + wave, nwaves = gridDim.x * 4;
    const int dr = lane >> 5, dsl = lane & 31;
    const int nco = min(n, Co - 1);
#define HWG_ISSUE(t_, st_)                                                                                         \
    {                                                                                                              \
        const uint32_t m0_ = (uint32_t)min((t_), ntiles - 1) * 16u;                              \
        const uint32_t b_ = m0_ / (uint32_t)HW, pix_ = m0_ - b_ * (uint32_t)HW;                                     \
        _Pragma("unroll") for (int d = 0; d < 8; ++d) {                                                            \
            const int r = 2 * d + dr;                                                                              \
            lds_dma16(x + ((int64_t)m0_ + r) * 128 + ((dsl ^ (r & 15)) << 2), T + (st_) * HWG_STAGE + d * 256);     \
        }                                                                                                          \
        lds_dma16(dy + ((int64_t)b_ * Co + nco) * HW + pix_ + 4 * kq, T + (st_) * HWG_STAGE + 2048);               \
    }
    f32x4 acc[8];
#pragma unroll
    for (int cb = 0; cb < 8; ++cb) acc[cb] = f32x4{0.f, 0.f, 0.f, 0.f};
    float bsum = 0.f;
    int tile = gw;
#pragma unroll
    for (int s = 0; s < HF_NST - 1; ++s) HWG_ISSUE(tile + s * nwaves, s)
    int stage = 0;
    for (; tile < ntiles; tile += nwaves) {
        const int nst = stage == 0 ? HF_NST - 1 : stage - 1;
        HWG_ISSUE(tile + (HF_NST - 1) * nwaves, nst)
        wait_vmcnt<9 * (HF_NST - 1)>();
        const uint32_t s0 = t_base + (uint32_t)stage * (HWG_STAGE * 4);
        f32x4 a = lds_read128_async<0>(s0 + 8192u + (uint32_t)lane * 16u);
        f32x4 xa[4], xb[4];
#pragma unroll
        for (int i = 0; i < 4; ++i) {
            const uint32_t row = (uint32_t)(4 * kq + i);
            xa[i] = lds_read128_async<0>(s0 + row * 512u + (((uint32_t)n ^ (row & 15u)) << 4));
            xb[i] = lds_read128_async<0>(s0 + row * 512u + (((uint32_t)(16 + n) ^ (row & 15u)) << 4));
        }
        SD_LDS_WAIT4(0, xa[0], xa[1], xa[2], xa[3]);
        SD_LDS_WAIT4(0, xb[0], xb[1], xb[2], xb[3]);
        SD_LDS_WAIT2(0, a, xa[0]);
        if (n >= Co) a = f32x4{0.f, 0.f, 0.f, 0.f};
#pragma unroll
        for (int i = 0; i < 4; ++i)
#pragma unroll
            for (int cb = 0; cb < 4; ++cb) {
                acc[cb] = __builtin_amdgcn_mfma_f32_16x16x4f32(a[i], xa[i][cb], acc[cb], 0, 0, 0);
                acc[4 + cb] = __builtin_amdgcn_mfma_f32_16x16x4f32(a[i], xb[i][cb], acc[4 + cb], 0, 0, 0);
            }
        bsum += (a[0] + a[1]) + (a[2] + a[3]);
        stage = stage + 1 == HF_NST ? 0 : stage + 1;
    }
    wait_vmcnt<0>();
#undef HWG_ISSUE
    float* dst = partial + (int64_t)gw * (Co * 128 + Co);
#pragma unroll
    for (int r = 0; r < 4; ++r) {
        const int co = 4 * kq + r;
        if (co < Co) {
#pragma unroll
            for (int cb = 0; cb < 4; ++cb) { dst[co * 128 + 4 * n + cb] = acc[cb][r]; dst[co * 128 + 64 + 4 * n + cb] = acc[4 + cb][r]; }
        }
    }
    bsum += __shfl_xor(bsum, 16);
    bsum += __shfl_xor(bsum, 32);
    if (kq == 0 && n < Co) dst[Co * 128 + n] = bsum;
}

__global__ __launch_bounds__(256) void k_head_wgrad_fin(const float* __restrict__ partial, int nblocks, int n, float* __restrict__ dw,
                                                         float* __restrict__ db, int nw, int accumulate) {
    __shared__ double red[32][8];
    const int lo = threadIdx.x & 7, lr = threadIdx.x >> 3;
    const int i = blockIdx.x * 8 + lo;
    double s = 0.0;
    if (i < n)
        for (int b = lr; b < nblocks; b += 32) s += (double)partial[(int64_t)b * n + i];
    red[lr][lo] = s;
    __syncthreads();
    if (lr != 0 || i >= n) return;
    for (int k = 1; k < 32; ++k) s += red[k][lo];
    float* dst = i < nw ? dw + i : db + (i - nw);
    *dst = (accumulate ? *dst : 0.f) + (float)s;
}

__global__ __launch_bounds__(256) void k_adam(float* __restrict__ p, const float* __restrict__ g, float* __restrict__ m,
                                               float* __restrict__ v, int64_t n4, float lr, float b1, float b2, float eps, float bc1,
                                               float bc2_sqrt, float gscale) {
    const int64_t stride = (int64_t)gridDim.x * 256;
    for (int64_t i = (int64_t)blockIdx.x * 256 + threadIdx.x; i < n4; i += stride) {
        float4 pp = reinterpret_cast<float4*>(p)[i];
        const float4 gg = reinterpret_cast<const float4*>(g)[i];
        float4 mm = reinterpret_cast<float4*>(m)[i], vv = reinterpret_cast<float4*>(v)[i];
        float* P = &pp.x; const float* G = &gg.x; float* Mo = &mm.x; float* V = &vv.x;
#pragma unroll
        for (int j = 0; j < 4; ++j) {
            const float gr = G[j] * gscale;
            Mo[j] = b1 * Mo[j] + (1.f - b1) * gr;
            V[j] = b2 * V[j] + (1.f - b2) * gr * gr;
            const float denom = sqrtf(V[j]) / bc2_sqrt + eps;
            P[j] -= (lr / bc1) * (Mo[j] / denom);
        }
        reinterpret_cast<float4*>(p)[i] = pp;
        reinterpret_cast<float4*>(m)[i] = mm;
        reinterpret_cast<float4*>(v)[i] = vv;
    }
}

constexpr int SUMSQ_MAX_BLOCKS = 512;

__device__ __forceinline__ double sumsq4(const float4 a) {
    return ((double)a.x * a.x + (double)a.y * a.y) + ((double)a.z * a.z + (double)a.w * a.w);
}

__device__ __forceinline__ double block_sum_256(double s, double* red4) {
    s = wave_sum(s);
    if ((threadIdx.x & 63) == 0) red4[threadIdx.x >> 6] = s;
    __syncthreads();
    return ((red4[0] + red4[1]) + red4[2]) + red4[3];
}

__global__ __launch_bounds__(256) void k_grad_sumsq(const float* __restrict__ g, int64_t n4, double* __restrict__ partial) {
    __shared__ double red[4];
    const int64_t stride = (int64_t)gridDim.x * 256;
    const float4* G = reinterpret_cast<const float4*>(g);
    double s = 0.0;
    for (int64_t i = (int64_t)blockIdx.x * 256 + threadIdx.x; i < n4; i += 8 * stride) {
        float4 a[8];
#pragma unroll
        for (int k = 0; k < 8; ++k) a[k] = G[min(i + k * stride, n4 - 1)];
#pragma unroll
        for (int k = 0; k < 8; ++k) s += i + k * stride < n4 ? sumsq4(a[k]) : 0.0;
    }
    s = block_sum_256(s, red);
    if (threadIdx.x == 0) partial[blockIdx.x] = s;
}

template <bool DECAY, bool CLIP, bool EMA>
__global__ __launch_bounds__(256) void k_optim(float* __restrict__ p, const float* __restrict__ g, float* __restrict__ m,
                                                float* __restrict__ v, int64_t n4, float lr, float b1, float b2, float eps, float bc1,
                                                float bc2_sqrt, float gscale, float decay_mul, const uint8_t* __restrict__ mask,
                                                float max_norm, const double* __restrict__ partial, int npartial,
                                                float* __restrict__ ema, float ema_decay, uint32_t* __restrict__ status) {
    float coef = 1.f;
    if (CLIP) {
        __shared__ double red[4];
        double s = 0.0;
        for (int k = threadIdx.x; k < npartial; k += 256) s += partial[k];
        s = block_sum_256(s, red);
        const float norm = (float)(fabs((double)gscale) * sqrt(s));
        const bool finite = (__float_as_uint(norm) & 0x7f800000u) != 0x7f800000u;
        coef = finite ? fminf(1.f, max_norm / (norm + 1e-6f)) : 0.f;
        if (blockIdx.x == 0 && threadIdx.x == 0) {
            status[0] = __float_as_uint(norm);
            status[1] = __float_as_uint(coef);
            if (!finite) status[2] = status[2] + 1u;
        }
        if (!finite) return;
    }
    const int64_t stride = (int64_t)gridDim.x * 256;
    for (int64_t i = (int64_t)blockIdx.x * 256 + threadIdx.x; i < n4; i += stride) {
        float4 pp = reinterpret_cast<float4*>(p)[i];
        const float4 gg = reinterpret_cast<const float4*>(g)[i];
        float4 mm = reinterpret_cast<float4*>(m)[i], vv = reinterpret_cast<float4*>(v)[i];
        float4 ee = make_float4(0.f, 0.f, 0.f, 0.f);
        if (EMA) ee = reinterpret_cast<float4*>(ema)[i];
        const bool decay = DECAY && (mask == nullptr || mask[i] != 0);
        float* P = &pp.x; const float* G = &gg.x; float* Mo = &mm.x; float* V = &vv.x; float* E = &ee.x;
#pragma unroll
        for (int j = 0; j < 4; ++j) {
            float gr = G[j] * gscale;
            if (CLIP) gr *= coef;
            if (decay) P[j] *= decay_mul;
            Mo[j] = b1 * Mo[j] + (1.f - b1) * gr;
            V[j] = b2 * V[j] + (1.f - b2) * gr * gr;
            const float denom = sqrtf(V[j]) / bc2_sqrt + eps;
            P[j] -= (lr / bc1) * (Mo[j] / denom);
            if (EMA) E[j] = ema_decay * E[j] + (1.f - ema_decay) * P[j];
        }
        reinterpret_cast<float4*>(p)[i] = pp;
        reinterpret_cast<float4*>(m)[i] = mm;
        reinterpret_cast<float4*>(v)[i] = vv;
        if (EMA) reinterpret_cast<float4*>(ema)[i] = ee;
    }
}

__device__ __forceinline__ float bf2f_(uint16_t v) { return __uint_as_float((uint32_t)v << 16); }
__device__ __forceinline__ uint16_t f2bf_(float v) { return __builtin_bit_cast(uint16_t, (__bf16)v); }

__global__ __launch_bounds__(256) void k_cast_bf16(const float* __restrict__ x, uint16_t* __restrict__ y, int64_t n4) {
    const int64_t stride = (int64_t)gridDim.x * 256;
    for (int64_t i = (int64_t)blockIdx.x * 256 + threadIdx.x; i < n4; i += stride) {
        const float4 v = reinterpret_cast<const float4*>(x)[i];
        reinterpret_cast<ushort4*>(y)[i] = make_ushort4(f2bf_(v.x), f2bf_(v.y), f2bf_(v.z), f2bf_(v.w));
    }
}

__global__ __launch_bounds__(256) void k_cast_f32(const uint16_t* __restrict__ x, float* __restrict__ y, int64_t n4) {
    const int64_t stride = (int64_t)gridDim.x * 256;
    for (int64_t i = (int64_t)blockIdx.x * 256 + threadIdx.x; i < n4; i += stride) st4(y, i, ld4(x, i));
}

__global__ __launch_bounds__(256) void k_maxpool_fwd_bf16(const uint16_t* __restrict__ x, uint16_t* __restrict__ y, int B, int Hi, int Wi,
                                                           int Ho, int Wo, int C) {
    const int cols = C >> 3;
    const int64_t n8 = (int64_t)B * Ho * Wo * cols;
    const int64_t i = (int64_t)blockIdx.x * 256 + threadIdx.x;
    if (i >= n8) return;
    const int col = (int)(i % cols);
    int64_t t = i / cols;
    const int ox = (int)(t % Wo); t /= Wo;
    const int oy = (int)(t % Ho);
    const int b = (int)(t / Ho);
    float m[8];
#pragma unroll
    for (int j = 0; j < 8; ++j) m[j] = -INFINITY;
#pragma unroll
    for (int r = 0; r < 3; ++r)
#pragma unroll
        for (int s = 0; s < 3; ++s) {
// ... 818 lines not shown

int sd_bn_bwd_bf16(const void* dy, const void* x, const void* y, int relu, int64_t M, int C, const float* mean, const float* invstd,
                   const float* gamma, const float* beta, void* dx, void* g_out, float* dgamma, float* dbeta, int accumulate, void* workspace,
                   size_t workspace_bytes, sd_stream_t stream) {
    SD_REQUIRE(dx, SD_ERR_INVALID, "sd_bn_bwd_bf16: null pointer");
    hipStream_t st = (hipStream_t)stream;
    const bool wide = C % 8 == 0 && relu != 1 && aligned16(dy) && aligned16(x) && aligned16(dx) && aligned16(g_out);
    if (int e = bn_bwd_reduce_any<uint16_t>("sd_bn_bwd_bf16", (const uint16_t*)dy, (const uint16_t*)x, y, relu, M, C, mean, invstd, gamma, beta,
                                            dgamma, dbeta, accumulate, nullptr, wide, workspace, workspace_bytes, st)) return e;
    const int nb = cdiv(M, red_rows(M));
    const float* mg = (const float*)workspace + (size_t)nb * 2 * C;
    return bn_bwd_apply_bf16(dy, x, y, relu, M, C, mean, invstd, gamma, beta, mg, dx, g_out, wide, st);
}

int sd_bn_bwd_reduce_bf16(const void* dy, const void* x, const void* y, int relu, int64_t M, int C, const float* mean, const float* invstd,
                          const float* gamma, const float* beta, float* dgamma, float* dbeta, int accumulate, double* sums, void* workspace,
                          size_t workspace_bytes, sd_stream_t stream) {
    SD_REQUIRE(sums, SD_ERR_INVALID, "sd_bn_bwd_reduce_bf16: null pointer");
    const bool wide = C % 8 == 0 && relu != 1 && aligned16(dy) && aligned16(x);
    return bn_bwd_reduce_any<uint16_t>("sd_bn_bwd_reduce_bf16", (const uint16_t*)dy, (const uint16_t*)x, y, relu, M, C, mean, invstd, gamma, beta,
                                       dgamma, dbeta, accumulate, sums, wide, workspace, workspace_bytes, (hipStream_t)stream);
}

int sd_bn_bwd_apply_bf16(const void* dy, const void* x, const void* y, int relu, int64_t M, int C, const float* mean, const float* invstd,
                         const float* gamma, const float* beta, const float* means, void* dx, void* g_out, sd_stream_t stream) {
    if (int e = check_mc("sd_bn_bwd_apply_bf16", M, C)) return e;
    SD_REQUIRE(relu >= 0 && relu <= 3, SD_ERR_INVALID, "sd_bn_bwd_apply_bf16: relu must be 0 (none), 1 (mask from y), 2 (mask recomputed from x) or 3 (mask bytes)");
    SD_REQUIRE(dy && x && mean && invstd && gamma && means && dx && ((relu != 1 && relu != 3) || y) && (relu != 2 || beta), SD_ERR_INVALID,
               "sd_bn_bwd_apply_bf16: null pointer");
    const bool wide = C % 8 == 0 && relu != 1 && aligned16(dy) && aligned16(x) && aligned16(dx) && aligned16(g_out);
    return bn_bwd_apply_bf16(dy, x, y, relu, M, C, mean, invstd, gamma, beta, means, dx, g_out, wide, (hipStream_t)stream);
}

int sd_col_sum_bf16(const void* x, int64_t M, int C, float* out, int accumulate, void* workspace, size_t workspace_bytes, sd_stream_t stream) {
    if (int e = check_mc("sd_col_sum_bf16", M, C)) return e;
    SD_REQUIRE(x && out && workspace, SD_ERR_INVALID, "sd_col_sum_bf16: null pointer");
    SD_REQUIRE(workspace_bytes >= sd_col_reduce_workspace_bytes(M, C), SD_ERR_WORKSPACE, "sd_col_sum_bf16: workspace too small");
    const int rpb = red_rows(M), nb = cdiv(M, rpb);
    hipStream_t st = (hipStream_t)stream;
    hipLaunchKernelGGL((k_col_reduce<2, uint16_t>), dim3(nb), dim3(256), 0, st, (const uint16_t*)x, (const uint16_t*)nullptr, (const uint16_t*)nullptr,
                       (const float*)nullptr, (const float*)nullptr, (const float*)nullptr, (const float*)nullptr, 0, M, C, (float*)workspace, rpb);
    SD_LAUNCH_CHECK();
    int rows = nb;
    const float* fin = fold_partials((const float*)workspace, rows, C, (float*)workspace + ((size_t)nb + 1) * 2 * C, st);
    hipLaunchKernelGGL(k_col_finalize<2>, dim3(cdiv(C, 4)), dim3(256), 0, st, fin, rows, C, (double)M, 0.f, 0.f, out,
                       (float*)nullptr, (float*)nullptr, (float*)nullptr, (float*)nullptr, (float*)nullptr, accumulate);
    SD_LAUNCH_CHECK();
    return 0;
}

int sd_upsample2x_bwd_bf16(const void* dy, const void* add, void* dx, int B, int H, int W, int C, sd_stream_t stream) {
    SD_REQUIRE(dy && dx && B > 0 && H > 0 && W > 0 && C > 0 && C % 4 == 0, SD_ERR_INVALID, "sd_upsample2x_bwd_bf16: bad arguments");
    const int64_t n4 = (int64_t)B * H * W * C / 4;
    hipLaunchKernelGGL(k_up2_bwd<uint16_t>, dim3(cdiv(n4, 256)), dim3(256), 0, (hipStream_t)stream, (const uint16_t*)dy, (const uint16_t*)add,
                       (uint16_t*)dx, B, H, W, C);
    SD_LAUNCH_CHECK();
    return 0;
}

int sd_maxpool3x3s2_fwd_bf16(const void* x, void* y, int B, int Hi, int Wi, int C, sd_stream_t stream) {
    SD_REQUIRE(x && y && B > 0 && Hi > 0 && Wi > 0 && C > 0 && C % 8 == 0, SD_ERR_INVALID, "sd_maxpool3x3s2_fwd_bf16: bad arguments");
    const int Ho = (Hi + 2 - 3) / 2 + 1, Wo = (Wi + 2 - 3) / 2 + 1;
    const int64_t n8 = (int64_t)B * Ho * Wo * C / 8;
    hipLaunchKernelGGL(k_maxpool_fwd_bf16, dim3(cdiv(n8, 256)), dim3(256), 0, (hipStream_t)stream, (const uint16_t*)x, (uint16_t*)y, B, Hi, Wi, Ho, Wo, C);
    SD_LAUNCH_CHECK();
    return 0;
}

int sd_head_fwd_bf16(const void* x, const float* w, const float* bias, float* y, int B, int HW, int C, int Co, sd_stream_t stream) {
    SD_REQUIRE(x && w && bias && y && B > 0 && HW > 0, SD_ERR_INVALID, "sd_head_fwd_bf16: bad arguments");
    if (Co > HEAD_NARROW_MAX_CO) return head_wide_fwd_bf16(x, w, bias, y, B, HW, C, Co, (hipStream_t)stream);
    SD_REQUIRE(C % 8 == 0 && C <= 512 && Co > 0 && Co <= HEAD_NARROW_MAX_CO, SD_ERR_INVALID, "sd_head_fwd_bf16: needs C %% 8 == 0, C <= 512, Co <= %d", HEAD_NARROW_MAX_CO);
    const int64_t M = (int64_t)B * HW;
    if (C == 128 && HW % 4 == 0 && aligned16(x) && aligned16(y)) {
        const int ntiles = (int)cdiv(M, 64), blocks = std::max(1, std::min(cdiv(ntiles, 4), 1024));
        if (Co <= 16) hipLaunchKernelGGL(k_head_fwd_bf16_c128<false>, dim3(blocks), dim3(256), 0, (hipStream_t)stream, (const uint16_t*)x, w, bias, y, M, HW, Co, ntiles);
        else hipLaunchKernelGGL(k_head_fwd_bf16_c128<true>, dim3(blocks), dim3(256), 0, (hipStream_t)stream, (const uint16_t*)x, w, bias, y, M, HW, Co, ntiles);
        SD_LAUNCH_CHECK();
        return 0;
    }
    const size_t lds = ((size_t)64 * (C + 4) + (size_t)Co * C) * sizeof(float);
    hipLaunchKernelGGL(k_head_fwd_bf16, dim3(cdiv(M, 64)), dim3(256), lds, (hipStream_t)stream, (const uint16_t*)x, w, bias, y, M, HW, C, Co);
    SD_LAUNCH_CHECK();
    return 0;
}

int sd_head_fwd(const float* x, const float* w, const float* bias, float* y, int B, int HW, int C, int Co, sd_stream_t stream) {
    SD_REQUIRE(x && w && bias && y && B > 0 && HW > 0, SD_ERR_INVALID, "sd_head_fwd: bad arguments");
    if (Co > HEAD_NARROW_MAX_CO) return head_wide_fwd(x, w, bias, y, B, HW, C, Co, (hipStream_t)stream);
    SD_REQUIRE(C % 4 == 0 && C <= 512 && Co > 0 && Co <= HEAD_NARROW_MAX_CO, SD_ERR_INVALID, "sd_head_fwd: needs C %% 4 == 0, C <= 512, Co <= %d", HEAD_NARROW_MAX_CO);
    const int64_t M = (int64_t)B * HW;
    if (C == 128 && Co <= 16 && HW % 16 == 0 && M < (1ll << 31) && aligned16(x) && aligned16(w) && aligned16(y)) {
        const int ntiles = (int)(M / 16);
        const size_t lds_b = (size_t)4 * HF_NST * 2048 * sizeof(float);
        static const hipError_t attr_once = hipFuncSetAttribute(reinterpret_cast<const void*>(&k_head_fwd_f32_c128), hipFuncAttributeMaxDynamicSharedMemorySize, (int)lds_b);
        SD_HIP(attr_once);
        hipLaunchKernelGGL(k_head_fwd_f32_c128, dim3(std::min(cdiv(ntiles, 4), 256)), dim3(256), lds_b, (hipStream_t)stream, x, w, bias, y, HW, Co, ntiles);
        SD_LAUNCH_CHECK();
        return 0;
    }
    const size_t lds = ((size_t)64 * (C + 4) + (size_t)Co * C) * sizeof(float);
    hipLaunchKernelGGL(k_head_fwd, dim3(cdiv(M, 64)), dim3(256), lds, (hipStream_t)stream, x, w, bias, y, M, HW, C, Co);
    SD_LAUNCH_CHECK();
    return 0;
}

static int head_wgrad_wave_rows(int64_t M) { return (int)std::min<int64_t>(1024, (cdiv(M, 16) + 3) / 4 * 4); }
size_t sd_head_bwd_workspace_bytes(int B, int HW, int C, int Co) {
    const int64_t M = (int64_t)B * HW;
    if (Co > HEAD_NARROW_MAX_CO) return head_wide_bwd_workspace_bytes(M, C, Co);
    return align_up((size_t)std::max<int64_t>(cdiv(M, HEAD_WG_PIX), head_wgrad_wave_rows(M)) * (Co * C + Co) * sizeof(float), 256);
}

int sd_head_bwd(const float* dy, const float* x, const float* w, float* dx, float* dw, float* dbias, int B, int HW, int C, int Co,
                int accumulate, void* workspace, size_t workspace_bytes, sd_stream_t stream) {
    SD_REQUIRE(dy && x && w && dx && dw && dbias && workspace && B > 0 && HW > 0, SD_ERR_INVALID, "sd_head_bwd: bad arguments");
    if (Co > HEAD_NARROW_MAX_CO) {
        const int64_t P = (int64_t)B * HW;
        if (int e = head_wide_check("sd_head_bwd", P, C, Co)) return e;
        SD_REQUIRE(workspace_bytes >= sd_head_bwd_workspace_bytes(B, HW, C, Co), SD_ERR_WORKSPACE, "sd_head_bwd: workspace too small");
        hipStream_t st = (hipStream_t)stream;
        int rows = 0;
        if (int e = head_wide_wgrad(dy, x, (float*)workspace, B, HW, C, Co, st, rows)) return e;
        const int n = Co * C + Co;
        hipLaunchKernelGGL(k_head_wgrad_fin, dim3(cdiv(n, 8)), dim3(256), 0, st, (const float*)workspace, rows, n, dw, dbias, Co * C, accumulate);
        SD_LAUNCH_CHECK();
        return head_wide_dgrad(dy, w, dx, B, HW, C, Co, st);
    }
    SD_REQUIRE(C % 4 == 0 && C <= 256 && (256 % C == 0) && (64 % (256 / C) == 0) && ((64 / (256 / C)) % 8 == 0) && Co > 0 && Co <= HEAD_NARROW_MAX_CO,
               SD_ERR_INVALID, "sd_head_bwd: needs C in {64, 128, 256} and Co <= %d", HEAD_NARROW_MAX_CO);
    SD_REQUIRE(workspace_bytes >= sd_head_bwd_workspace_bytes(B, HW, C, Co), SD_ERR_WORKSPACE, "sd_head_bwd: workspace too small");
    const int64_t M = (int64_t)B * HW;
    hipStream_t st = (hipStream_t)stream;
    int nb = cdiv(M, HEAD_WG_PIX);
    if (C == 128 && Co <= 16 && HW % 16 == 0 && M < (1ll << 31) && aligned16(x) && aligned16(dy)) {
        nb = head_wgrad_wave_rows(M);
        const int blocks = nb / 4;
        const size_t lds_b = (size_t)4 * HF_NST * HWG_STAGE * sizeof(float);
        static const hipError_t attr_once = hipFuncSetAttribute(reinterpret_cast<const void*>(&k_head_wgrad_f32_c128), hipFuncAttributeMaxDynamicSharedMemorySize, (int)lds_b);
        SD_HIP(attr_once);
        hipLaunchKernelGGL(k_head_wgrad_f32_c128, dim3(blocks), dim3(256), lds_b, st, dy, x, (float*)workspace, HW, Co, (int)(M / 16));
    } else {
        hipLaunchKernelGGL(k_head_wgrad, dim3(nb), dim3(256), 0, st, dy, x, (float*)workspace, M, HW, C, Co);
    }
    SD_LAUNCH_CHECK();
    const int n = Co * C + Co;
    hipLaunchKernelGGL(k_head_wgrad_fin, dim3(cdiv(n, 8)), dim3(256), 0, st, (const float*)workspace, nb, n, dw, dbias, Co * C, accumulate);
    SD_LAUNCH_CHECK();
    hipLaunchKernelGGL(k_head_dgrad<float>, dim3(cdiv(M, 64)), dim3(256), (size_t)Co * C * sizeof(float), st, dy, w, dx, M, HW, C, Co);
    SD_LAUNCH_CHECK();
    return 0;
}

int sd_head_bwd_bf16(const float* dy, const void* x_bf16, const float* w, void* dx_bf16, float* dw, float* dbias, int B, int HW, int C, int Co,
                     int accumulate, void* workspace, size_t workspace_bytes, sd_stream_t stream) {
    SD_REQUIRE(dy && x_bf16 && w && dx_bf16 && dw && dbias && workspace && B > 0 && HW > 0, SD_ERR_INVALID, "sd_head_bwd_bf16: bad arguments");
    SD_REQUIRE((C == 64 || C == 128) && Co > 0 && Co <= 8, SD_ERR_INVALID, "sd_head_bwd_bf16: needs C in {64, 128} and Co <= 8 (got %d, %d)", C, Co);
    SD_REQUIRE(aligned16(x_bf16) && aligned16(dx_bf16), SD_ERR_ALIGN, "sd_head_bwd_bf16: x and dx must be 16-byte aligned");
    SD_REQUIRE(workspace_bytes >= sd_head_bwd_workspace_bytes(B, HW, C, Co), SD_ERR_WORKSPACE, "sd_head_bwd_bf16: workspace too small");
    const int64_t M = (int64_t)B * HW;
    hipStream_t st = (hipStream_t)stream;
    hipLaunchKernelGGL(k_head_dgrad<uint16_t>, dim3(cdiv(M, 64)), dim3(256), (size_t)Co * C * sizeof(float), st, dy, w, (uint16_t*)dx_bf16, M, HW, C, Co);
    SD_LAUNCH_CHECK();
    const int nb = cdiv(M, HEAD_WG_PIX);
    hipLaunchKernelGGL(k_head_wgrad_bf16<8>, dim3(nb), dim3(256), 0, st, dy, (const uint16_t*)x_bf16, (float*)workspace, M, HW, C, Co);
    SD_LAUNCH_CHECK();
    const int n = Co * C + Co;
    hipLaunchKernelGGL(k_head_wgrad_fin, dim3(cdiv(n, 8)), dim3(256), 0, st, (const float*)workspace, nb, n, dw, dbias, Co * C, accumulate);
    SD_LAUNCH_CHECK();
    return 0;
}

int sd_adam_step(float* param, const float* grad, float* exp_avg, float* exp_avg_sq, int64_t n, int step, float lr, float beta1, float beta2,
                 float eps, float grad_scale, sd_stream_t stream) {
    SD_REQUIRE(param && grad && exp_avg && exp_avg_sq && n > 0 && n % 4 == 0 && step >= 1, SD_ERR_INVALID, "sd_adam_step: bad arguments (n %% 4 == 0, step >= 1)");
    SD_REQUIRE(aligned16(param) && aligned16(grad) && aligned16(exp_avg) && aligned16(exp_avg_sq), SD_ERR_ALIGN, "sd_adam_step: pointers must be 16-byte aligned");
    const double bc1 = 1.0 - pow((double)beta1, step), bc2 = 1.0 - pow((double)beta2, step);
    hipLaunchKernelGGL(k_adam, dim3(ew_grid(n / 4)), dim3(256), 0, (hipStream_t)stream, param, grad, exp_avg, exp_avg_sq, n / 4, lr, beta1, beta2, eps,
                       (float)bc1, (float)sqrt(bc2), grad_scale);
    SD_LAUNCH_CHECK();
    return 0;
}

static inline int sumsq_blocks(int64_t n) { return n > 0 ? (int)std::min<int64_t>(cdiv(n / 4, 256), SUMSQ_MAX_BLOCKS) : 0; }

size_t sd_grad_sumsq_workspace_bytes(int64_t n) { return (size_t)sumsq_blocks(n) * sizeof(double); }

int sd_grad_sumsq(const float* grad, int64_t n, void* workspace, size_t workspace_bytes, sd_stream_t stream) {
    SD_REQUIRE(grad && workspace && n > 0 && n % 4 == 0, SD_ERR_INVALID, "sd_grad_sumsq: bad arguments (n %% 4 == 0)");
    SD_REQUIRE(aligned16(grad) && (reinterpret_cast<uintptr_t>(workspace) & 7u) == 0, SD_ERR_ALIGN,
               "sd_grad_sumsq: grad must be 16-byte aligned, the workspace 8-byte aligned");
    SD_REQUIRE(workspace_bytes >= sd_grad_sumsq_workspace_bytes(n), SD_ERR_WORKSPACE, "sd_grad_sumsq: workspace too small");
    hipLaunchKernelGGL(k_grad_sumsq, dim3(sumsq_blocks(n)), dim3(256), 0, (hipStream_t)stream, grad, n / 4, (double*)workspace);
    SD_LAUNCH_CHECK();
    return 0;
}

int sd_optim_step(float* param, const float* grad, float* exp_avg, float* exp_avg_sq, int64_t n, int step, float lr, float beta1, float beta2,
                  float eps, float grad_scale, float weight_decay, const uint8_t* decay_mask, float max_norm, const void* partials,
                  int npartials, float* ema, float ema_decay, void* status, sd_stream_t stream) {
    SD_REQUIRE(param && grad && exp_avg && exp_avg_sq && n > 0 && n % 4 == 0 && step >= 1, SD_ERR_INVALID, "sd_optim_step: bad arguments (n %% 4 == 0, step >= 1)");
    SD_REQUIRE(aligned16(param) && aligned16(grad) && aligned16(exp_avg) && aligned16(exp_avg_sq) && aligned16(ema), SD_ERR_ALIGN,
               "sd_optim_step: pointers must be 16-byte aligned");
    SD_REQUIRE(weight_decay >= 0.f, SD_ERR_INVALID, "sd_optim_step: weight_decay must be >= 0 (got %g)", (double)weight_decay);
    SD_REQUIRE(max_norm >= 0.f, SD_ERR_INVALID, "sd_optim_step: max_norm must be >= 0 (got %g; 0 = no clipping)", (double)max_norm);
    SD_REQUIRE(ema_decay >= 0.f && ema_decay < 1.f, SD_ERR_INVALID, "sd_optim_step: ema_decay must be in [0, 1) (got %g)", (double)ema_decay);
    const bool decay = weight_decay > 0.f, clip = max_norm > 0.f, avg = ema != nullptr;
    if (clip) {
        SD_REQUIRE(partials && npartials > 0 && status, SD_ERR_INVALID,
                   "sd_optim_step: max_norm > 0 needs the partials of sd_grad_sumsq (pointer and count) and the status block");
        SD_REQUIRE(npartials == sumsq_blocks(n), SD_ERR_INVALID, "sd_optim_step: %d partials, sd_grad_sumsq writes %d for n = %lld "
                   "(sd_grad_sumsq_workspace_bytes(n) / 8)", npartials, sumsq_blocks(n), (long long)n);
        SD_REQUIRE((reinterpret_cast<uintptr_t>(partials) & 7u) == 0 && (reinterpret_cast<uintptr_t>(status) & 3u) == 0, SD_ERR_ALIGN,
                   "sd_optim_step: partials must be 8-byte aligned, the status block 4-byte aligned");
    }
    const double bc1 = 1.0 - pow((double)beta1, step), bc2 = 1.0 - pow((double)beta2, step);
    const int64_t n4 = n / 4;
    hipStream_t st = (hipStream_t)stream;
    if (!decay && !clip && !avg) {
        hipLaunchKernelGGL(k_adam, dim3(ew_grid(n4)), dim3(256), 0, st, param, grad, exp_avg, exp_avg_sq, n4, lr, beta1, beta2, eps, (float)bc1,
                           (float)sqrt(bc2), grad_scale);
        SD_LAUNCH_CHECK();
        return 0;
    }
    using kernel_t = decltype(&k_optim<true, true, true>);
    static const kernel_t variants[8] = {nullptr,                      k_optim<true, false, false>, k_optim<false, true, false>,
                                         k_optim<true, true, false>,   k_optim<false, false, true>, k_optim<true, false, true>,
                                         k_optim<false, true, true>,   k_optim<true, true, true>};
    const float decay_mul = (float)(1.0 - (double)lr * (double)weight_decay);
    hipLaunchKernelGGL(variants[(int)decay | (int)clip << 1 | (int)avg << 2], dim3(ew_grid(n4)), dim3(256), 0, st, param, grad, exp_avg, exp_avg_sq, n4,
                       lr, beta1, beta2, eps, (float)bc1, (float)sqrt(bc2), grad_scale, decay_mul, decay_mask, max_norm, (const double*)partials,
                       npartials, ema, ema_decay, (uint32_t*)status);
    SD_LAUNCH_CHECK();
    return 0;
}

}
```

### structuredetector_amd/model/network.py

```python
from __future__ import annotations

import ctypes as C
import math
import warnings

import torch
import torch.nn as nn

from .. import _lib as L
from ..utils import trace as T

BN_EPS = 1e-5
BN_MOMENTUM = 0.1


class ConvParams(nn.Module):
    def __init__(self, cin, cout, k, stride=1, pad=0, bias=False):
        super().__init__()
        self.cin, self.cout, self.k, self.stride, self.pad = cin, cout, k, stride, pad
        w = torch.empty((cout, cin, k, k), memory_format=torch.channels_last)
        self.weight = nn.Parameter(w)
        self.bias = nn.Parameter(torch.zeros(cout)) if bias else None


class BNParams(nn.Module):
    def __init__(self, c):
        super().__init__()
        self.c = c
        self.weight = nn.Parameter(torch.ones(c))
        self.bias = nn.Parameter(torch.zeros(c))
        self.register_buffer("running_mean", torch.zeros(c))
        self.register_buffer("running_var", torch.ones(c))
        self.register_buffer("num_batches_tracked", torch.tensor(0, dtype=torch.long))


class Slot(nn.Module):
    """Parameter-less position (ReLU / MaxPool / Upsample) kept so Sequential indices match the reference."""


class BasicBlock(nn.Module):
    def __init__(self, cin, cout, stride):
        super().__init__()
        self.conv1 = ConvParams(cin, cout, 3, stride, 1)
        self.bn1 = BNParams(cout)
        self.relu = Slot()
        self.conv2 = ConvParams(cout, cout, 3, 1, 1)
        self.bn2 = BNParams(cout)
        self.downsample = None
        if stride != 1 or cin != cout:
            self.downsample = nn.Sequential(ConvParams(cin, cout, 1, stride, 0), BNParams(cout))


class Fpn(nn.Module):

    def __init__(self, in_channels, out_channels):
        super().__init__()
        self.up = Slot()
        self.lateral = ConvParams(in_channels, out_channels, 1, bias=True)
        self.conv = nn.Sequential(ConvParams(out_channels, out_channels, 3, 1, 1), BNParams(out_channels), Slot())


class Head(nn.Module):

    def __init__(self, in_channels, out_channels):
        super().__init__()
        self.conv = ConvParams(in_channels, out_channels, 1, bias=True)


BACKBONE_FILE_GLOB = "resnet34-*.pth"


def find_backbone_weights(args=None):
    import os
    from pathlib import Path
    for given in (getattr(args, "backbone_weights", None), os.environ.get("SDNET_BACKBONE_WEIGHTS")):
        if given:
            path = Path(given).expanduser()
            if not path.is_file():
                raise L.SdError(f"backbone weights file not found: {path}")
            return path
    homes = []
    if os.environ.get("TORCH_HOME"):
        homes.append(Path(os.environ["TORCH_HOME"]))
    homes.append(Path(os.environ.get("XDG_CACHE_HOME", "~/.cache")).expanduser() / "torch")
    for home in homes:
        hits = sorted((home / "hub" / "checkpoints").glob(BACKBONE_FILE_GLOB))
        if hits:
            return hits[0]
    return None


def _layer(cin, cout, n, stride):
    return nn.Sequential(*[BasicBlock(cin if i == 0 else cout, cout, stride if i == 0 else 1) for i in range(n)])


def _desc(B, Hi, Wi, conv: ConvParams):
    d = L.ConvDesc()
    d.B, d.Hi, d.Wi, d.Cin, d.Cout, d.R, d.S, d.stride, d.pad = B, Hi, Wi, conv.cin, conv.cout, conv.k, conv.k, conv.stride, conv.pad
    d.Ho = (Hi + 2 * conv.pad - conv.k) // conv.stride + 1
    d.Wo = (Wi + 2 * conv.pad - conv.k) // conv.stride + 1
    return d


def _ptr(t):
    return 0 if t is None else t.data_ptr()


class _Engine:

    def __init__(self, net: "Network"):
        self.net = net
        self.lib = L.lib()
        self.prof = None
        self.prof_shapes = None
        self._nbt = []
        self.overlap_wgrad = False
        self._side = None
        self.fuse_bn_bwd = False
        self._wt_plan, self._wt_flat, self._wt_valid = None, {}, None
        self._head_ok = {}
        self.stem_ring = True
        self.fuse_head = True
        self.small_batch_kernel = True

    def _kname(self, d, which):
        if self.prof is None:
            return ""
        if self.prof_shapes is not None:
            self.prof_shapes.append((d.B, d.Hi, d.Wi, d.Cin, d.Cout, d.R, d.stride, d.Ho, d.Wo))
        return self.lib.sd_conv2d_kernel_name(C.byref(d), which).decode()

    def _timed(self, kind, flops, fn, phase="fwd"):
        if self.prof is None:
            return fn()
        e0, e1 = torch.cuda.Event(enable_timing=True), torch.cuda.Event(enable_timing=True)
        e0.record()
        fn()
        e1.record()
        self.prof.append((kind, flops, e0, e1, phase))

    def _ws(self, nbytes, dev):
        return L.workspace(max(int(nbytes), 256), dev)

    def _to_bf16(self, t):
        out = torch.empty(t.shape, dtype=torch.bfloat16, device=t.device)
        L.check(self.lib.sd_cast_f32_to_bf16(t.data_ptr(), out.data_ptr(), t.numel(), L.stream()), "sd_cast_f32_to_bf16")
        return out

    def _to_f32(self, t):
        out = torch.empty(t.shape, dtype=torch.float32, device=t.device)
        L.check(self.lib.sd_cast_bf16_to_f32(t.data_ptr(), out.data_ptr(), t.numel(), L.stream()), "sd_cast_bf16_to_f32")
        return out

    def refresh_bf16_weights(self):
        net = self.net
        if net.flat_params_bf16 is None:
            net.flat_params_bf16 = torch.empty(net.flat_params.numel(), dtype=torch.bfloat16, device=net.flat_params.device)
        L.check(self.lib.sd_cast_f32_to_bf16(net.flat_params.data_ptr(), net.flat_params_bf16.data_ptr(), net.flat_params.numel(), L.stream()),
                "sd_cast_f32_to_bf16")

    def _w16(self, conv):
        off, n = self.net._flat_off[id(conv.weight)]
        return self.net.flat_params_bf16[off:off + n]

    def _conv_sb(self, x, w, y, d, scale, shift, res, res_up2, relu, bf16):
        nws = self.lib.sd_conv2d_fwd_sb_workspace_bytes(C.byref(d), bf16)
        ws = self._ws(nws, x.device) if nws else None
        st = L.zero_state(self.lib.sd_conv2d_fwd_sb_state_bytes(C.byref(d), bf16), x.device) if nws else None
        L.check(self.lib.sd_conv2d_fwd_sb(x.data_ptr(), w.data_ptr(), y.data_ptr(), C.byref(d), _ptr(scale), _ptr(shift), _ptr(res), int(res_up2),
                                          int(relu), bf16, _ptr(ws), ws.numel() if nws else 0, _ptr(st), st.numel() if nws else 0, L.stream()),
                "sd_conv2d_fwd_sb")

    def conv(self, x, conv, B, Hi, Wi, scale=None, shift=None, res=None, res_up2=False, relu=False, amp=False, sb=False):
        d = _desc(B, Hi, Wi, conv)
        if amp:
            y = torch.empty((B, d.Ho, d.Wo, conv.cout), dtype=torch.bfloat16, device=x.device)
            flops = 2.0 * B * d.Ho * d.Wo * conv.cout * conv.cin * conv.k * conv.k
            self._timed("bf16:" + self._kname(d, 16), flops, lambda: L.check(
                self.lib.sd_conv2d_fwd_bf16(x.data_ptr(), self._w16(conv).data_ptr(), y.data_ptr(), C.byref(d), _ptr(scale), _ptr(shift),
                                            _ptr(res), int(res_up2), int(relu), 0, 0, L.stream()), "sd_conv2d_fwd_bf16"))
            return y, d
        y = torch.empty((B, d.Ho, d.Wo, conv.cout), dtype=torch.float32, device=x.device)
        flops = 2.0 * B * d.Ho * d.Wo * conv.cout * conv.cin * conv.k * conv.k
        if sb and self.small_batch_kernel and self.lib.sd_conv2d_fwd_sb_supported(C.byref(d), 0):
            self._timed("k_conv_fwd_sb<false>" if self.prof is not None else "", flops,
                        lambda: self._conv_sb(x, conv.weight, y, d, scale, shift, res, res_up2, relu, 0))
            return y, d
        nws = self.lib.sd_conv2d_fwd_workspace_bytes(C.byref(d))
        ws = self._ws(nws, x.device) if nws else None
        self._timed(self._kname(d, 0), flops, lambda: L.check(
            self.lib.sd_conv2d_fwd(x.data_ptr(), conv.weight.data_ptr(), y.data_ptr(), C.byref(d), _ptr(scale), _ptr(shift),
                                   _ptr(res), int(res_up2), int(relu), _ptr(ws), ws.numel() if nws else 0, L.stream()),
            "sd_conv2d_fwd"))
        return y, d

    def conv_stats(self, x, conv, B, Hi, Wi, bn: BNParams, update_running=True, amp=False, sync=None):
        d = _desc(B, Hi, Wi, conv)
        y = torch.empty((B, d.Ho, d.Wo, conv.cout), dtype=torch.bfloat16 if amp else torch.float32, device=x.device)
        mean = torch.empty(conv.cout, dtype=torch.float32, device=x.device)
        invstd = torch.empty_like(mean)
        flops = 2.0 * B * d.Ho * d.Wo * conv.cout * conv.cin * conv.k * conv.k
        if sync is not None:
            sums = sync.take(conv.cout)
            if sync.log is not None:
                fused = self.lib.sd_conv2d_fwd_bn_stats_rows(C.byref(d), int(amp)) > 0
                sync.log.append(("sd_conv2d_fwd_bf16_bn_sums" if amp else "sd_conv2d_fwd_bn_sums") + ("" if fused else ":two-pass"))
            if amp:
                ws = self._ws(self.lib.sd_conv2d_fwd_bf16_bn_stats_workspace_bytes(C.byref(d)), x.device)
                self._timed("bf16:" + self._kname(d, 16), flops, lambda: L.check(
                    self.lib.sd_conv2d_fwd_bf16_bn_sums(x.data_ptr(), self._w16(conv).data_ptr(), y.data_ptr(), C.byref(d), sums.data_ptr(),
                                                        ws.data_ptr(), ws.numel(), L.stream()), "sd_conv2d_fwd_bf16_bn_sums"))
            else:
                ws = self._ws(self.lib.sd_conv2d_fwd_bn_stats_workspace_bytes(C.byref(d)), x.device)
                self._timed(self._kname(d, 0), flops, lambda: L.check(
                    self.lib.sd_conv2d_fwd_bn_sums(x.data_ptr(), conv.weight.data_ptr(), y.data_ptr(), C.byref(d), sums.data_ptr(),
                                                   ws.data_ptr(), ws.numel(), L.stream()), "sd_conv2d_fwd_bn_sums"))
            self._stats_from_sums(sync, sums, bn, mean, invstd, update_running)
            return y, d, (mean, invstd)
        if amp:
            ws = self._ws(self.lib.sd_conv2d_fwd_bf16_bn_stats_workspace_bytes(C.byref(d)), x.device)
            self._timed("bf16:" + self._kname(d, 16), flops, lambda: L.check(
                self.lib.sd_conv2d_fwd_bf16_bn_stats(x.data_ptr(), self._w16(conv).data_ptr(), y.data_ptr(), C.byref(d), BN_EPS, BN_MOMENTUM,
                                                     bn.running_mean.data_ptr() if update_running else 0,
                                                     bn.running_var.data_ptr() if update_running else 0,
                                                     mean.data_ptr(), invstd.data_ptr(), ws.data_ptr(), ws.numel(), L.stream()),
                "sd_conv2d_fwd_bf16_bn_stats"))
            return y, d, (mean, invstd)
        ws = self._ws(self.lib.sd_conv2d_fwd_bn_stats_workspace_bytes(C.byref(d)), x.device)
        self._timed(self._kname(d, 0), flops, lambda: L.check(
            self.lib.sd_conv2d_fwd_bn_stats(x.data_ptr(), conv.weight.data_ptr(), y.data_ptr(), C.byref(d), BN_EPS, BN_MOMENTUM,
                                            bn.running_mean.data_ptr() if update_running else 0,
                                            bn.running_var.data_ptr() if update_running else 0,
                                            mean.data_ptr(), invstd.data_ptr(), ws.data_ptr(), ws.numel(), L.stream()),
            "sd_conv2d_fwd_bn_stats"))
        return y, d, (mean, invstd)

    def _stats_from_sums(self, sync, sums, bn: BNParams, mean, invstd, update_running=True):
        sync.reduce(sums)
        L.check(self.lib.sd_bn_stats_from_sums(sums.data_ptr(), bn.c, BN_EPS, BN_MOMENTUM,
                                               bn.running_mean.data_ptr() if update_running else 0,
                                               bn.running_var.data_ptr() if update_running else 0,
                                               mean.data_ptr(), invstd.data_ptr(), L.stream()), "sd_bn_stats_from_sums")

    def _means_from_sums(self, sync, sums, Cc, device):
        sync.reduce(sums)
        means = torch.empty(2 * Cc, dtype=torch.float32, device=device)
        L.check(self.lib.sd_bn_bwd_means_from_sums(sums.data_ptr(), Cc, means.data_ptr(), L.stream()), "sd_bn_bwd_means_from_sums")
        return means

    def bn_train(self, x, bn: BNParams, res=None, relu=True, update_running=True, stats=None, want_mask=False, sync=None):
        Mrows, Cc = x.numel() // x.shape[-1], x.shape[-1]
        if stats is not None:
            mean, invstd = stats
        elif sync is not None:
            mean = torch.empty(Cc, dtype=torch.float32, device=x.device)
            invstd = torch.empty_like(mean)
            sums = sync.take(Cc)
            sync.record("sd_bn_train_sums")
            ws = self._ws(self.lib.sd_col_reduce_workspace_bytes(Mrows, Cc), x.device)
            train_sums = self.lib.sd_bn_train_sums_bf16 if x.dtype == torch.bfloat16 else self.lib.sd_bn_train_sums
            L.check(train_sums(x.data_ptr(), Mrows, Cc, sums.data_ptr(), ws.data_ptr(), ws.numel(), L.stream()), "sd_bn_train_sums")
            self._stats_from_sums(sync, sums, bn, mean, invstd, update_running)
        else:
            mean = torch.empty(Cc, dtype=torch.float32, device=x.device)
            invstd = torch.empty_like(mean)
            ws = self._ws(self.lib.sd_col_reduce_workspace_bytes(Mrows, Cc), x.device)
            L.check(self.lib.sd_bn_train_stats(x.data_ptr(), Mrows, Cc, BN_EPS, BN_MOMENTUM,
                                               bn.running_mean.data_ptr() if update_running else 0,
                                               bn.running_var.data_ptr() if update_running else 0,
                                               mean.data_ptr(), invstd.data_ptr(), ws.data_ptr(), ws.numel(), L.stream()), "sd_bn_train_stats")
        y = torch.empty_like(x)
        mask = torch.empty(x.numel() // 4, dtype=torch.uint8, device=x.device) if want_mask else None
        apply = self.lib.sd_bn_apply_bf16 if x.dtype == torch.bfloat16 else self.lib.sd_bn_apply
        L.check(apply(x.data_ptr(), y.data_ptr(), Mrows, Cc, mean.data_ptr(), invstd.data_ptr(), bn.weight.data_ptr(),
                      bn.bias.data_ptr(), _ptr(res), int(relu), _ptr(mask), L.stream()), "sd_bn_apply")
        if update_running:
            self._nbt.append(bn.num_batches_tracked)
        return (y, mean, invstd, mask) if want_mask else (y, mean, invstd)

    def bn_fold(self, bn: BNParams):
        cached = self.net._folded.get(id(bn))
        if cached is not None:
            return cached
        scale = torch.empty(bn.c, dtype=torch.float32, device=bn.weight.device)
        shift = torch.empty_like(scale)
        L.check(self.lib.sd_bn_fold(bn.weight.data_ptr(), bn.bias.data_ptr(), bn.running_mean.data_ptr(), bn.running_var.data_ptr(),
                                    BN_EPS, bn.c, scale.data_ptr(), shift.data_ptr(), L.stream()), "sd_bn_fold")
        self.net._folded[id(bn)] = (scale, shift)
        return scale, shift

    def forward(self, x, training, tape=None, amp=False):
        net, lib = self.net, self.lib
        if amp:
            if not training:
                raise L.SdError("amp=True is the mixed-precision TRAINING forward; inference uses forward_bf16")
            self.refresh_bf16_weights()
        if x.dim() != 4 or x.shape[1] != 3:
            raise L.SdError(f"Network expects (B, 3, H, W) input, got {tuple(x.shape)}")
        L.require_cuda(x)
        x = x.contiguous().float()
        B, _, H, W = x.shape
        if H % 32 or W % 32:
            raise L.SdError("input height/width must be multiples of 32 (args.py:181-186)")
        rec = tape is not None
        sx = tape.get("bn_sync") if (rec and training) else None
        if sx is not None:
            sx.begin("fwd")

        T.push("fwd:stem")
        stem, bn0 = net.adpater[0], net.adpater[1]
        d0 = _desc(B, H, W, stem)
        amp_stem = bool(amp and training and d0.Ho % 2 == 0 and d0.Wo % 2 == 0)
        s0 = torch.empty((B, d0.Ho, d0.Wo, 64), dtype=torch.bfloat16 if amp_stem else torch.float32, device=x.device)
        wss = self._ws(lib.sd_conv2d_stem_fwd_workspace_bytes(C.byref(d0)), x.device)
        Hp, Wp = (d0.Ho + 2 - 3) // 2 + 1, (d0.Wo + 2 - 3) // 2 + 1
        p1 = torch.empty((B, Hp, Wp, 64), dtype=torch.bfloat16 if amp_stem else torch.float32, device=x.device)
        pidx = torch.empty((B, Hp, Wp, 64), dtype=torch.uint8, device=x.device)
        if training:
            m0 = torch.empty(64, dtype=torch.float32, device=x.device)
            i0 = torch.empty_like(m0)
            ws = self._ws(lib.sd_conv2d_stem_fwd_bn_stats_workspace_bytes(C.byref(d0)), x.device)
            if sx is None:
                stem_fwd = (lib.sd_conv2d_stem_fwd_bn_stats_bf16 if amp_stem else lib.sd_conv2d_stem_fwd_bn_stats_bf16mm) if amp \
                    else lib.sd_conv2d_stem_fwd_bn_stats
                L.check(stem_fwd(x.data_ptr(), stem.weight.data_ptr(), s0.data_ptr(), C.byref(d0), BN_EPS, BN_MOMENTUM,
                                 bn0.running_mean.data_ptr(), bn0.running_var.data_ptr(), m0.data_ptr(), i0.data_ptr(),
                                 ws.data_ptr(), ws.numel(), L.stream()), "sd_conv2d_stem_fwd_bn_stats")
            else:
                sums = sx.take(64)
                stem_sums = (lib.sd_conv2d_stem_fwd_bn_sums_bf16 if amp_stem else lib.sd_conv2d_stem_fwd_bn_sums_bf16mm) if amp \
                    else lib.sd_conv2d_stem_fwd_bn_sums
                sx.record("sd_conv2d_stem_fwd_bn_sums")
                L.check(stem_sums(x.data_ptr(), stem.weight.data_ptr(), s0.data_ptr(), C.byref(d0), sums.data_ptr(), ws.data_ptr(), ws.numel(),
                                  L.stream()), "sd_conv2d_stem_fwd_bn_sums")
                self._stats_from_sums(sx, sums, bn0, m0, i0)
            self._nbt.append(bn0.num_batches_tracked)
            pool_fwd = lib.sd_bn_relu_maxpool_fwd_bf16 if amp_stem else lib.sd_bn_relu_maxpool_fwd
            L.check(pool_fwd(s0.data_ptr(), B, d0.Ho, d0.Wo, 64, m0.data_ptr(), i0.data_ptr(), bn0.weight.data_ptr(),
                             bn0.bias.data_ptr(), p1.data_ptr(), pidx.data_ptr(), L.stream()), "sd_bn_relu_maxpool_fwd")
        else:
            sc, sh = self.bn_fold(bn0)
            L.check(lib.sd_conv2d_stem_fwd(x.data_ptr(), stem.weight.data_ptr(), s0.data_ptr(), C.byref(d0), sc.data_ptr(), sh.data_ptr(), 1, 0,
                                           wss.data_ptr(), wss.numel(), L.stream()), "stem")
            m0 = i0 = None
            L.check(lib.sd_maxpool3x3s2_fwd(s0.data_ptr(), p1.data_ptr(), pidx.data_ptr(), B, d0.Ho, d0.Wo, 64, L.stream()), "maxpool")
        if rec:
            tape["x"], tape["stem"], tape["amp"] = x, (d0, s0, m0, i0, pidx), bool(amp)
        if amp and not amp_stem:
            p1 = self._to_bf16(p1)

        T.pop()
        feats, cur, Hc, Wc = [], p1, Hp, Wp
        blocks_tape = []
        for li, layer in enumerate((net.down1, net.down2, net.down3, net.down4), start=1):
            T.push(f"fwd:down{li}")
            for blk in layer:
                if training:
                    c1, d1, st1 = self.conv_stats(cur, blk.conv1, B, Hc, Wc, blk.bn1, amp=amp, sync=sx)
                    a1, m1, i1 = self.bn_train(c1, blk.bn1, stats=st1)
                    c2, d2, st2 = self.conv_stats(a1, blk.conv2, B, d1.Ho, d1.Wo, blk.bn2, amp=amp, sync=sx)
                    if blk.downsample is not None:
                        cd, dd, std_ = self.conv_stats(cur, blk.downsample[0], B, Hc, Wc, blk.downsample[1], amp=amp, sync=sx)
                        idt, md, idd = self.bn_train(cd, blk.downsample[1], relu=False, stats=std_)
                    else:
                        cd = dd = md = idd = None
                        idt = cur
                    out, m2, i2, msk = self.bn_train(c2, blk.bn2, res=idt, relu=True, stats=st2, want_mask=True)
                    if rec:
                        blocks_tape.append((blk, cur, (Hc, Wc), d1, c1, a1, m1, i1, d2, c2, m2, i2, out, dd, cd, md, idd, msk))
                else:
                    s1, h1 = self.bn_fold(blk.bn1)
                    a1, d1 = self.conv(cur, blk.conv1, B, Hc, Wc, scale=s1, shift=h1, relu=True, sb=True)
                    if blk.downsample is not None:
                        sd_, hd = self.bn_fold(blk.downsample[1])
                        idt, _ = self.conv(cur, blk.downsample[0], B, Hc, Wc, scale=sd_, shift=hd, sb=True)
                    else:
                        idt = cur
                    s2, h2 = self.bn_fold(blk.bn2)
                    out, _ = self.conv(a1, blk.conv2, B, d1.Ho, d1.Wo, scale=s2, shift=h2, res=idt, relu=True, sb=True)
                cur, Hc, Wc = out, d1.Ho, d1.Wo
            feats.append((cur, Hc, Wc))
            T.pop()
        (p2, H2, W2), (p3, H3, W3), (p4, H4, W4), (p5, H5, W5) = feats

        T.push("fwd:fpn")
        f, _ = self.conv(p5, net.up1, B, H5, W5, shift=net.up1.bias, amp=amp, sb=not training)
        fpn_tape = []
        for fpn, (sc_t, Hs, Ws) in ((net.up2, (p4, H4, W4)), (net.up3, (p3, H3, W3)), (net.up4, (p2, H2, W2))):
            t, dl = self.conv(sc_t, fpn.lateral, B, Hs, Ws, shift=fpn.lateral.bias, res=f, res_up2=True, amp=amp, sb=not training)
            if training:
                c, dc, stf = self.conv_stats(t, fpn.conv[0], B, Hs, Ws, fpn.conv[1], amp=amp, sync=sx)
                fn, mf, if_ = self.bn_train(c, fpn.conv[1], stats=stf)
                if rec:
                    fpn_tape.append((fpn, sc_t, (Hs, Ws), dl, t, dc, c, mf, if_, fn))
            else:
                sf, hf = self.bn_fold(fpn.conv[1])
                fn, _ = self.conv(t, fpn.conv[0], B, Hs, Ws, scale=sf, shift=hf, relu=True, sb=True)
            f = fn
        T.pop()

        T.push("fwd:head")
        hc = net.head.conv
        out = torch.empty((B, hc.cout, H2, W2), dtype=torch.float32, device=x.device)
        head_fwd = lib.sd_head_fwd_bf16 if amp else lib.sd_head_fwd
        L.check(head_fwd(f.data_ptr(), hc.weight.data_ptr(), hc.bias.data_ptr(), out.data_ptr(), B, H2 * W2, hc.cin, hc.cout,
                         L.stream()), "sd_head_fwd")
        T.pop()
        if rec:
            tape.update(blocks=blocks_tape, fpn=fpn_tape, p5=(p5, H5, W5), f1=f, B=B, hw=(H2, W2))
        if self._nbt:
            torch._foreach_add_(self._nbt, 1)
            self._nbt = []
        return out

    def _w_bf16(self, conv):
        key = ("w", id(conv))
        w = self.net._folded.get(key)
        if w is None:
            n = conv.weight.numel()
            w = torch.empty(n, dtype=torch.bfloat16, device=conv.weight.device)
            L.check(self.lib.sd_cast_f32_to_bf16(conv.weight.data_ptr(), w.data_ptr(), n, L.stream()), "sd_cast_f32_to_bf16")
            self.net._folded[key] = w
        return w

    def _head_fusable(self, B, Hs, Ws, conv, hc):
        key = (B, Hs, Ws, hc.cout)
        ok = self._head_ok.get(key)
        if ok is None:
            ok = hc.cin == 128 and bool(self.lib.sd_conv2d_fwd_bf16_head_supported(C.byref(_desc(B, Hs, Ws, conv)), hc.cout))
            self._head_ok[key] = ok
        return ok

    def _head_prepared(self, hc):
        key = ("head", id(hc))
        buf = self.net._folded.get(key)
        if buf is None:
            buf = torch.empty(self.lib.sd_head_split_bf16_bytes(), dtype=torch.uint8, device=hc.weight.device)
            L.check(self.lib.sd_head_split_bf16(hc.weight.data_ptr(), hc.bias.data_ptr(), hc.cout, buf.data_ptr(), L.stream()), "sd_head_split_bf16")
            self.net._folded[key] = buf
        return buf

    def conv_bf16(self, x, conv, B, Hi, Wi, scale=None, shift=None, res=None, res_up2=False, relu=False):
        d = _desc(B, Hi, Wi, conv)
        y = torch.empty((B, d.Ho, d.Wo, conv.cout), dtype=torch.bfloat16, device=x.device)
        if self.small_batch_kernel and self.lib.sd_conv2d_fwd_sb_supported(C.byref(d), 1):
            self._conv_sb(x, self._w_bf16(conv), y, d, scale, shift, res, res_up2, relu, 1)
            return y, d
        nws = self.lib.sd_conv2d_fwd_bf16_workspace_bytes(C.byref(d))
        ws = self._ws(nws, x.device) if nws else None
        L.check(self.lib.sd_conv2d_fwd_bf16(x.data_ptr(), self._w_bf16(conv).data_ptr(), y.data_ptr(), C.byref(d), _ptr(scale), _ptr(shift),
                                            _ptr(res), int(res_up2), int(relu), _ptr(ws), ws.numel() if nws else 0, L.stream()),
                "sd_conv2d_fwd_bf16")
        return y, d

    def forward_bf16(self, x):
        net, lib = self.net, self.lib
        L.require_cuda(x)
        x = x.contiguous().float()
        B, _, H, W = x.shape
        if x.dim() != 4 or x.shape[1] != 3 or H % 32 or W % 32:
            raise L.SdError("Network expects (B, 3, H, W) input with H, W multiples of 32")
        stem, bn0 = net.adpater[0], net.adpater[1]
        d0 = _desc(B, H, W, stem)
        sc, sh = self.bn_fold(bn0)
        Hc, Wc = (d0.Ho + 2 - 3) // 2 + 1, (d0.Wo + 2 - 3) // 2 + 1
        cur = torch.empty((B, Hc, Wc, 64), dtype=torch.bfloat16, device=x.device)
        if stem.k == 7 and stem.stride == 2 and stem.pad == 3 and d0.Wo <= 4096:
            L.check(lib.sd_stem_bn_relu_maxpool_fwd_bf16(x.data_ptr(), stem.weight.data_ptr(), sc.data_ptr(), sh.data_ptr(), cur.data_ptr(),
                                                         C.byref(d0), L.stream()), "stem+maxpool")
        else:
            a0 = torch.empty((B, d0.Ho, d0.Wo, 64), dtype=torch.bfloat16, device=x.device)
            wss = self._ws(lib.sd_conv2d_stem_fwd_workspace_bytes(C.byref(d0)), x.device)
            L.check(lib.sd_conv2d_stem_fwd(x.data_ptr(), stem.weight.data_ptr(), a0.data_ptr(), C.byref(d0), sc.data_ptr(), sh.data_ptr(), 1, 1,
                                           wss.data_ptr(), wss.numel(), L.stream()), "stem")
            L.check(lib.sd_maxpool3x3s2_fwd_bf16(a0.data_ptr(), cur.data_ptr(), B, d0.Ho, d0.Wo, 64, L.stream()), "maxpool")
        feats = []
        for layer in (net.down1, net.down2, net.down3, net.down4):
            for blk in layer:
                s1, h1 = self.bn_fold(blk.bn1)
                a1, d1 = self.conv_bf16(cur, blk.conv1, B, Hc, Wc, scale=s1, shift=h1, relu=True)
                if blk.downsample is not None:
                    sd_, hd = self.bn_fold(blk.downsample[1])
                    idt, _ = self.conv_bf16(cur, blk.downsample[0], B, Hc, Wc, scale=sd_, shift=hd)
                else:
                    idt = cur
                s2, h2 = self.bn_fold(blk.bn2)
                cur, _ = self.conv_bf16(a1, blk.conv2, B, d1.Ho, d1.Wo, scale=s2, shift=h2, res=idt, relu=True)
                Hc, Wc = d1.Ho, d1.Wo
            feats.append((cur, Hc, Wc))
        (p2, H2, W2), (p3, H3, W3), (p4, H4, W4), (p5, H5, W5) = feats
        f, _ = self.conv_bf16(p5, net.up1, B, H5, W5, shift=net.up1.bias)
        hc = net.head.conv
        out = torch.empty((B, hc.cout, H2, W2), dtype=torch.float32, device=x.device)
        for fpn, (sc_t, Hs, Ws) in ((net.up2, (p4, H4, W4)), (net.up3, (p3, H3, W3)), (net.up4, (p2, H2, W2))):
            t, _ = self.conv_bf16(sc_t, fpn.lateral, B, Hs, Ws, shift=fpn.lateral.bias, res=f, res_up2=True)
            sf, hf = self.bn_fold(fpn.conv[1])
            if fpn is net.up4 and self.fuse_head and self._head_fusable(B, Hs, Ws, fpn.conv[0], hc):
                dl = _desc(B, Hs, Ws, fpn.conv[0])
                rc = lib.sd_conv2d_fwd_bf16_head(t.data_ptr(), self._w_bf16(fpn.conv[0]).data_ptr(), C.byref(dl), sf.data_ptr(), hf.data_ptr(), 1,
                                                 self._head_prepared(hc).data_ptr(), hc.cout, out.data_ptr(), L.stream())
                if rc == 0:
                    return out
                if rc > 0:
                    L.check(rc, "sd_conv2d_fwd_bf16_head")
                self._head_ok.pop((B, Hs, Ws, hc.cout), None)
            f, _ = self.conv_bf16(t, fpn.conv[0], B, Hs, Ws, scale=sf, shift=hf, relu=True)
        L.check(lib.sd_head_fwd_bf16(f.data_ptr(), hc.weight.data_ptr(), hc.bias.data_ptr(), out.data_ptr(), B, H2 * W2, hc.cin, hc.cout,
                                     L.stream()), "sd_head_fwd_bf16")
        return out

    def _transpose_all(self, amp):
        net = self.net
        if self._wt_plan is None:
            convs = [m for m in net.modules() if isinstance(m, ConvParams) and m.cin % 64 == 0 and m.cout % 64 == 0]
            rows, views, dst, blk = [], {}, 0, 0
            for m in convs:
                taps, n = m.k * m.k, m.weight.numel()
                nbx, nby = (m.cin + 31) // 32, (m.cout + 31) // 32
                rows.append([net._flat_off[id(m.weight)][0], dst, m.cout, taps, m.cin, blk, nbx, nby])
                views[id(m)] = (dst, n)
                dst += n; blk += nbx * nby * taps
            table = torch.tensor(rows, dtype=torch.int32, device=net.flat_params.device).contiguous()
            self._wt_plan = (table, len(convs), blk, views, dst)
        table, nconv, blocks, _, total = self._wt_plan
        key = "bf16" if amp else "f32"
        if key not in self._wt_flat:
            self._wt_flat[key] = torch.empty(total, dtype=torch.bfloat16 if amp else torch.float32, device=net.flat_params.device)
        L.check(self.lib.sd_conv2d_transpose_weights_batched(net.flat_params.data_ptr(), self._wt_flat[key].data_ptr(), table.data_ptr(), nconv, blocks,
                                                             int(amp), L.stream()), "sd_conv2d_transpose_weights_batched")
        self._wt_valid = key

    def _wt(self, conv, amp=False):
        if self._wt_valid == ("bf16" if amp else "f32") and id(conv) in self._wt_plan[3]:
            off, n = self._wt_plan[3][id(conv)]
            return self._wt_flat[self._wt_valid][off:off + n]
        wt = torch.empty(conv.cin * conv.k * conv.k * conv.cout, dtype=torch.bfloat16 if amp else torch.float32, device=conv.weight.device)
        transpose = self.lib.sd_conv2d_transpose_weights_bf16 if amp else self.lib.sd_conv2d_transpose_weights
        L.check(transpose(conv.weight.data_ptr(), wt.data_ptr(), conv.cout, conv.k * conv.k, conv.cin, L.stream()), "transpose_weights")
        return wt

    def _dgrad(self, dy, conv, d, res=None, bn_next=None, res_half=False, sync=None):
        amp = dy.dtype == torch.bfloat16
        dx = torch.empty((d.B, d.Hi, d.Wi, conv.cin), dtype=dy.dtype, device=dy.device)
        wt = self._wt(conv, amp)
        flops = 2.0 * d.B * d.Ho * d.Wo * conv.cout * conv.cin * conv.k * conv.k
        if amp:
            assert bn_next is None, "fuse_bn_bwd is an fp32-path experiment"
            mode = 2 if res_half else (1 if res is not None else 0)
            self._timed("bf16:" + self._kname(d, 17), flops, lambda: L.check(
                self.lib.sd_conv2d_dgrad_bf16(dy.data_ptr(), wt.data_ptr(), dx.data_ptr(), C.byref(d), _ptr(res), mode, L.stream()),
                "sd_conv2d_dgrad_bf16"), phase="dgrad")
            return dx
        if bn_next is None:
            if res_half:
                fn = lambda: L.check(self.lib.sd_conv2d_dgrad_half_res(dy.data_ptr(), wt.data_ptr(), dx.data_ptr(), C.byref(d), res.data_ptr(),
                                                                       L.stream()), "sd_conv2d_dgrad_half_res")
            else:
                fn = lambda: L.check(self.lib.sd_conv2d_dgrad(dy.data_ptr(), wt.data_ptr(), dx.data_ptr(), C.byref(d), _ptr(res), L.stream()),
                                     "sd_conv2d_dgrad")
            self._timed(self._kname(d, 1), flops, fn, phase="dgrad")
            return dx
        assert not res_half
        x, y, relu, bn, mean, invstd = bn_next
        ws = self._ws(self.lib.sd_conv2d_dgrad_bn_reduce_workspace_bytes(C.byref(d)), dy.device)
        if sync is not None:
            sums = sync.take(conv.cin)
            sync.record("sd_conv2d_dgrad_bn_reduce_sums")
            self._timed(self._kname(d, 1), flops, lambda: L.check(
                self.lib.sd_conv2d_dgrad_bn_reduce_sums(dy.data_ptr(), wt.data_ptr(), dx.data_ptr(), C.byref(d), _ptr(res), x.data_ptr(),
                                                        _ptr(y) if int(relu) in (1, 3) else 0, int(relu), mean.data_ptr(), invstd.data_ptr(),
                                                        bn.weight.data_ptr(), bn.bias.data_ptr(), self.net.grad_of(bn.weight).data_ptr(),
                                                        self.net.grad_of(bn.bias).data_ptr(), 0, sums.data_ptr(), ws.data_ptr(), ws.numel(),
                                                        L.stream()), "sd_conv2d_dgrad_bn_reduce_sums"), phase="dgrad")
            return dx, self._means_from_sums(sync, sums, conv.cin, dy.device)
        means = torch.empty(2 * conv.cin, dtype=torch.float32, device=dy.device)
        self._timed(self._kname(d, 1), flops, lambda: L.check(
            self.lib.sd_conv2d_dgrad_bn_reduce(dy.data_ptr(), wt.data_ptr(), dx.data_ptr(), C.byref(d), _ptr(res), x.data_ptr(),
                                               _ptr(y) if int(relu) in (1, 3) else 0, int(relu), mean.data_ptr(), invstd.data_ptr(),
                                               bn.weight.data_ptr(), bn.bias.data_ptr(), self.net.grad_of(bn.weight).data_ptr(),
                                               self.net.grad_of(bn.bias).data_ptr(), 0, means.data_ptr(), ws.data_ptr(), ws.numel(),
                                               L.stream()), "sd_conv2d_dgrad_bn_reduce"), phase="dgrad")
        return dx, means

    def _side_stream(self):
        if self._side is None:
            self._side = torch.cuda.Stream()
        return self._side

    def _wgrad(self, dy, x, conv, d):
        if not self.overlap_wgrad:
            return self._wgrad_now(dy, x, conv, d)
        main, side = torch.cuda.current_stream(), self._side_stream()
        ready = torch.cuda.Event()
        ready.record(main)
        with torch.cuda.stream(side):
            side.wait_event(ready)
            self._wgrad_now(dy, x, conv, d)
        dy.record_stream(side); x.record_stream(side)

    def _join_side(self):
        if self.overlap_wgrad and self._side is not None:
            torch.cuda.current_stream().wait_stream(self._side)

    def _wgrad_now(self, dy, x, conv, d):
        g = self.net.grad_of(conv.weight)
        flops = 2.0 * d.B * d.Ho * d.Wo * conv.cout * conv.cin * conv.k * conv.k
        if dy.dtype == torch.bfloat16:
            ws = self._ws(self.lib.sd_conv2d_wgrad_bf16_workspace_bytes(C.byref(d)), dy.device)
            self._timed("bf16:" + self._kname(d, 2), flops, lambda: L.check(
                self.lib.sd_conv2d_wgrad_bf16(dy.data_ptr(), x.data_ptr(), g.data_ptr(), C.byref(d), 0, ws.data_ptr(), ws.numel(), L.stream()),
                "sd_conv2d_wgrad_bf16"), phase="wgrad")
            return
        nbytes = self.lib.sd_conv2d_wgrad_workspace_bytes(C.byref(d))
        ws = self._ws(nbytes, dy.device)
        self._timed(self._kname(d, 2), flops, lambda: L.check(
            self.lib.sd_conv2d_wgrad(dy.data_ptr(), x.data_ptr(), g.data_ptr(), C.byref(d), 0, ws.data_ptr(), ws.numel(), L.stream()),
            "sd_conv2d_wgrad"), phase="wgrad")

    def _bias_grad(self, dy, conv):
        Mrows, Cc = dy.numel() // dy.shape[-1], dy.shape[-1]
        ws = self._ws(self.lib.sd_col_reduce_workspace_bytes(Mrows, Cc), dy.device)
        col_sum = self.lib.sd_col_sum_bf16 if dy.dtype == torch.bfloat16 else self.lib.sd_col_sum
        L.check(col_sum(dy.data_ptr(), Mrows, Cc, self.net.grad_of(conv.bias).data_ptr(), 0, ws.data_ptr(), ws.numel(), L.stream()),
                "sd_col_sum")

    def _bn_bwd(self, dy, x, y, relu, bn, mean, invstd, want_g=False, means=None, sync=None):
        Mrows, Cc = x.numel() // x.shape[-1], x.shape[-1]
        dx = torch.empty_like(x)
        g = torch.empty_like(x) if want_g else None
        if means is None and sync is not None:
            sums = sync.take(Cc)
            bf16 = x.dtype == torch.bfloat16
            sync.record("sd_bn_bwd_reduce_bf16" if bf16 else "sd_bn_bwd_reduce")
            ws = self._ws(self.lib.sd_col_reduce_workspace_bytes(Mrows, Cc), x.device)
            reduce = self.lib.sd_bn_bwd_reduce_bf16 if bf16 else self.lib.sd_bn_bwd_reduce
            L.check(reduce(dy.data_ptr(), x.data_ptr(), _ptr(y) if int(relu) in (1, 3) else 0, int(relu), Mrows, Cc, mean.data_ptr(),
                           invstd.data_ptr(), bn.weight.data_ptr(), bn.bias.data_ptr(), self.net.grad_of(bn.weight).data_ptr(),
                           self.net.grad_of(bn.bias).data_ptr(), 0, sums.data_ptr(), ws.data_ptr(), ws.numel(), L.stream()), "sd_bn_bwd_reduce")
            means = self._means_from_sums(sync, sums, Cc, x.device)
            apply = self.lib.sd_bn_bwd_apply_bf16 if bf16 else self.lib.sd_bn_bwd_apply
            L.check(apply(dy.data_ptr(), x.data_ptr(), _ptr(y) if int(relu) in (1, 3) else 0, int(relu), Mrows, Cc, mean.data_ptr(),
                          invstd.data_ptr(), bn.weight.data_ptr(), bn.bias.data_ptr(), means.data_ptr(), dx.data_ptr(), _ptr(g), L.stream()),
                    "sd_bn_bwd_apply")
            return dx, g
        if means is not None:
            L.check(self.lib.sd_bn_bwd_apply(dy.data_ptr(), x.data_ptr(), _ptr(y) if int(relu) in (1, 3) else 0, int(relu), Mrows, Cc,
                                             mean.data_ptr(), invstd.data_ptr(), bn.weight.data_ptr(), bn.bias.data_ptr(), means.data_ptr(),
                                             dx.data_ptr(), _ptr(g), L.stream()), "sd_bn_bwd_apply")
            return dx, g
        ws = self._ws(self.lib.sd_col_reduce_workspace_bytes(Mrows, Cc), x.device)
        bn_bwd = self.lib.sd_bn_bwd_bf16 if x.dtype == torch.bfloat16 else self.lib.sd_bn_bwd
        L.check(bn_bwd(dy.data_ptr(), x.data_ptr(), _ptr(y) if int(relu) in (1, 3) else 0, int(relu), Mrows, Cc, mean.data_ptr(),
                                   invstd.data_ptr(), bn.weight.data_ptr(), bn.bias.data_ptr(), dx.data_ptr(), _ptr(g),
                                   self.net.grad_of(bn.weight).data_ptr(),
                                   self.net.grad_of(bn.bias).data_ptr(), 0, ws.data_ptr(), ws.numel(), L.stream()), "sd_bn_bwd")
        return dx, g

    def backward(self, tape, dhead, on_stage=None):
        net, lib = self.net, self.lib
        B = tape["B"]
        H2, W2 = tape["hw"]
        dhead = dhead.contiguous().float()
        hc = net.head.conv
        amp = bool(tape.get("amp"))
        if amp and self.fuse_bn_bwd:
            raise L.SdError("fuse_bn_bwd is an fp32-path experiment; switch it off for mixed-precision training")
        sx = tape.get("bn_sync")
        if sx is not None:
            sx.begin("bwd")
        T.push("bwd:fpn_head")
        self._transpose_all(amp)
        ws = self._ws(lib.sd_head_bwd_workspace_bytes(B, H2 * W2, hc.cin, hc.cout), dhead.device)
        if amp and hc.cin in (64, 128) and hc.cout <= 8:
            f1 = tape["f1"]
            df = torch.empty_like(f1)
            L.check(lib.sd_head_bwd_bf16(dhead.data_ptr(), f1.data_ptr(), hc.weight.data_ptr(), df.data_ptr(), net.grad_of(hc.weight).data_ptr(),
                                         net.grad_of(hc.bias).data_ptr(), B, H2 * W2, hc.cin, hc.cout, 0, ws.data_ptr(), ws.numel(), L.stream()),
                    "sd_head_bwd_bf16")
        else:
            f1 = self._to_f32(tape["f1"]) if amp else tape["f1"]
            df = torch.empty_like(f1)
            L.check(lib.sd_head_bwd(dhead.data_ptr(), f1.data_ptr(), hc.weight.data_ptr(), df.data_ptr(), net.grad_of(hc.weight).data_ptr(),
                                    net.grad_of(hc.bias).data_ptr(), B, H2 * W2, hc.cin, hc.cout, 0, ws.data_ptr(), ws.numel(), L.stream()),
                    "sd_head_bwd")
            if amp:
                df = self._to_bf16(df)

        lateral_grad = {}
        for (fpn, sc_t, (Hs, Ws), dl, t, dc, c, mf, if_, fn) in reversed(tape["fpn"]):
            dcv, _ = self._bn_bwd(df, c, fn, 2, fpn.conv[1], mf, if_, sync=sx)
            dt = self._dgrad(dcv, fpn.conv[0], dc)
            self._wgrad(dcv, t, fpn.conv[0], dc)
            self._wgrad(dt, sc_t, fpn.lateral, dl)
            self._bias_grad(dt, fpn.lateral)
            lateral_grad[sc_t.data_ptr()] = (dt, fpn.lateral, dl)
            dfp = torch.empty((B, Hs // 2, Ws // 2, fpn.lateral.cout), dtype=dt.dtype, device=dt.device)
            up2_bwd = lib.sd_upsample2x_bwd_bf16 if amp else lib.sd_upsample2x_bwd
            L.check(up2_bwd(dt.data_ptr(), 0, dfp.data_ptr(), B, Hs // 2, Ws // 2, fpn.lateral.cout, L.stream()), "up2_bwd")
            df = dfp
        p5, H5, W5 = tape["p5"]
        d5 = _desc(B, H5, W5, net.up1)
        self._wgrad(df, p5, net.up1, d5)
        self._bias_grad(df, net.up1)
        blocks = tape["blocks"]

        def bn2_of(i):
            if i < 0 or not self.fuse_bn_bwd:
                return None
            b = blocks[i]
            return (b[9], b[17], 3, b[0].bn2, b[10], b[11])

        last = len(blocks) - 1
        has_lateral = blocks[last][12].data_ptr() in lateral_grad
        nxt = None if has_lateral else bn2_of(last)
        r = self._dgrad(df, net.up1, d5, bn_next=nxt, sync=sx)
        dcur, mcur = r if nxt is not None else (r, None)
        T.pop()
        if on_stage:
            self._join_side()
            on_stage("fpn_head")

        first_of = {id(net.down4[0]): "down4", id(net.down3[0]): "down3", id(net.down2[0]): "down2"}
        T.push("bwd:down4")
        for bi in range(last, -1, -1):
            (blk, xin, (Hc, Wc), d1, c1, a1, m1, i1, d2, c2, m2, i2, out, dd, cd, md, idd, msk) = blocks[bi]
            extra = lateral_grad.pop(out.data_ptr(), None)
            if extra is not None:
                nxt = bn2_of(bi)
                r = self._dgrad(extra[0], extra[1], extra[2], res=dcur, bn_next=nxt, sync=sx)
                dcur, mcur = r if nxt is not None else (r, None)
            dc2, g = self._bn_bwd(dcur, c2, msk, 3, blk.bn2, m2, i2, want_g=True, means=mcur, sync=sx)
            nxt = (c1, None, 2, blk.bn1, m1, i1) if self.fuse_bn_bwd else None
            r = self._dgrad(dc2, blk.conv2, d2, bn_next=nxt, sync=sx)
            da1, ma1 = r if nxt is not None else (r, None)
            self._wgrad(dc2, a1, blk.conv2, d2)
            dc1, _ = self._bn_bwd(da1, c1, a1, 2, blk.bn1, m1, i1, means=ma1, sync=sx)
            half = False
            if blk.downsample is not None:
                dcd, _ = self._bn_bwd(g, cd, None, False, blk.downsample[1], md, idd, sync=sx)
                ds = blk.downsample[0]
                half = ds.k == 1 and ds.stride == 2 and ds.pad == 0 and Hc % 2 == 0 and Wc % 2 == 0 and not self.fuse_bn_bwd
                if half:
                    dsm = L.ConvDesc()
                    dsm.B, dsm.Hi, dsm.Wi, dsm.Cin, dsm.Cout, dsm.R, dsm.S, dsm.stride, dsm.pad = B, dd.Ho, dd.Wo, ds.cin, ds.cout, 1, 1, 1, 0
                    dsm.Ho, dsm.Wo = dd.Ho, dd.Wo
                    skip = self._dgrad(dcd, ds, dsm)
                else:
                    skip = self._dgrad(dcd, ds, dd)
                self._wgrad(dcd, xin, ds, dd)
            else:
                skip = g
            prev_lateral = bi > 0 and blocks[bi - 1][12].data_ptr() in lateral_grad
            nxt = None if (bi == 0 or prev_lateral) else bn2_of(bi - 1)
            r = self._dgrad(dc1, blk.conv1, d1, res=skip, bn_next=nxt, res_half=half, sync=sx)
            dcur, mcur = r if nxt is not None else (r, None)
            self._wgrad(dc1, xin, blk.conv1, d1)
            if id(blk) in first_of:
                T.pop()
                if on_stage:
                    self._join_side()
                    on_stage(first_of[id(blk)])
                T.push("bwd:" + {"down4": "down3", "down3": "down2", "down2": "down1_stem"}[first_of[id(blk)]])

        d0, s0, m0, i0, pidx = tape["stem"]
        bn0 = net.adpater[1]
        amp_stem = s0.dtype == torch.bfloat16
        if amp and not amp_stem:
            dcur = self._to_f32(dcur)
        ring = amp_stem and self.stem_ring and d0.Wi % 4 == 0
        ds0 = torch.empty(s0.shape, dtype=torch.bfloat16 if ring else torch.float32, device=s0.device)
        ws = self._ws(lib.sd_col_reduce_workspace_bytes(B * d0.Ho * d0.Wo, 64), s0.device)
        if sx is None:
            pool_bwd = lib.sd_maxpool_bn_relu_bwd_bf16_dx16 if ring else (lib.sd_maxpool_bn_relu_bwd_bf16 if amp_stem else lib.sd_maxpool_bn_relu_bwd)
            L.check(pool_bwd(dcur.data_ptr(), pidx.data_ptr(), s0.data_ptr(), B, d0.Ho, d0.Wo, 64, m0.data_ptr(), i0.data_ptr(),
                             bn0.weight.data_ptr(), bn0.bias.data_ptr(), ds0.data_ptr(), net.grad_of(bn0.weight).data_ptr(),
                             net.grad_of(bn0.bias).data_ptr(), 0, ws.data_ptr(), ws.numel(), L.stream()), "sd_maxpool_bn_relu_bwd")
        else:
            sums = sx.take(64)
            sx.record("sd_maxpool_bn_relu_bwd_reduce")
            pool_reduce = lib.sd_maxpool_bn_relu_bwd_reduce_bf16 if amp_stem else lib.sd_maxpool_bn_relu_bwd_reduce
            L.check(pool_reduce(dcur.data_ptr(), pidx.data_ptr(), s0.data_ptr(), B, d0.Ho, d0.Wo, 64, m0.data_ptr(), i0.data_ptr(),
                                bn0.weight.data_ptr(), bn0.bias.data_ptr(), net.grad_of(bn0.weight).data_ptr(), net.grad_of(bn0.bias).data_ptr(), 0,
                                sums.data_ptr(), ws.data_ptr(), ws.numel(), L.stream()), "sd_maxpool_bn_relu_bwd_reduce")
            means = self._means_from_sums(sx, sums, 64, s0.device)
            pool_apply = lib.sd_maxpool_bn_relu_bwd_apply_bf16_dx16 if ring else (lib.sd_maxpool_bn_relu_bwd_apply_bf16 if amp_stem
                                                                                  else lib.sd_maxpool_bn_relu_bwd_apply)
            L.check(pool_apply(dcur.data_ptr(), pidx.data_ptr(), s0.data_ptr(), B, d0.Ho, d0.Wo, 64, m0.data_ptr(), i0.data_ptr(),
                               bn0.weight.data_ptr(), bn0.bias.data_ptr(), means.data_ptr(), ds0.data_ptr(), L.stream()), "sd_maxpool_bn_relu_bwd_apply")
        stem = net.adpater[0]
        ws = self._ws(lib.sd_conv2d_stem_wgrad_workspace_bytes(C.byref(d0)), ds0.device)
        stem_wgrad = lib.sd_conv2d_stem_wgrad_bf16 if ring else (lib.sd_conv2d_stem_wgrad_bf16mm if amp else lib.sd_conv2d_stem_wgrad)
        L.check(stem_wgrad(ds0.data_ptr(), tape["x"].data_ptr(), net.grad_of(stem.weight).data_ptr(), C.byref(d0), 0,
                           ws.data_ptr(), ws.numel(), L.stream()), "sd_conv2d_stem_wgrad")
        self._join_side()
        self._wt_valid = None
        T.pop()
        if on_stage:
            on_stage("down1_stem")


class _NetFn(torch.autograd.Function):

    @staticmethod
    def forward(ctx, net, x, *params):
        tape = {}
        out = net._engine.forward(x, True, tape)
        ctx.net, ctx.tape = net, tape
        return out

    @staticmethod
    def backward(ctx, dhead):
        net = ctx.net
        net._engine.backward(ctx.tape, dhead)
        ctx.tape = None
        return (None, None) + tuple(net.grad_of(p) for p in net._flat_order)


class Network(nn.Module):
    def __init__(self, args, pretrained=True, raw_output: bool = False, init_weights: bool = True):
        super().__init__()
        self.raw_output = raw_output
        self.bf16_inference = bool(getattr(args, "use_amp", False) or getattr(args, "bf16_inference", False))
        self.label_count = len(args.labels)
        self.part_count = len(args.parts)
        self.out_channels = self.label_count + self.part_count + 4
        self.fpn_depth = args.fpn_depth
        if self.fpn_depth % 64:
            raise L.SdError("fpn_depth must be a multiple of 64 for the MFMA tiles")
        if self.out_channels > 256:
            raise L.SdError(f"labels + parts + 4 must be <= 256 (head kernel limit SD_HEAD_MAX_CO); got {self.out_channels}")
        if self.out_channels > 32 and self.fpn_depth not in (64, 128, 256):
            raise L.SdError(f"labels + parts + 4 > 32 needs fpn_depth in (64, 128, 256) (the wide head kernels); got {self.fpn_depth}")

        self.adpater = nn.Sequential(ConvParams(3, 64, 7, 2, 3), BNParams(64), Slot(), Slot())
        self.down1 = _layer(64, 64, 3, 1)
        self.down2 = _layer(64, 128, 4, 2)
        self.down3 = _layer(128, 256, 6, 2)
        self.down4 = _layer(256, 512, 3, 2)
        self.up1 = ConvParams(512, self.fpn_depth, 1, bias=True)
        self.up2 = Fpn(256, self.fpn_depth)
        self.up3 = Fpn(128, self.fpn_depth)
        self.up4 = Fpn(64, self.fpn_depth)
        self.head = Head(self.fpn_depth, self.out_channels)
# ... 168 lines not shown
```

Baseline: 873.3.

## Fuse final FPN BatchNorm+ReLU into head conv forward and backward

In fp32 training, the last FPN stage's BatchNorm+ReLU is no longer materialized. The head 1x1 conv applies the BN affine and ReLU on the fly from the pre-BN conv output. In backward, the head weight gradient reads the BN inputs directly, and the BN backward recomputes the head's input gradient (dy·W) inside its column-reduce and apply kernels instead of storing it. This removes writing and rereading the full-resolution 128-channel activation and its gradient. The price is recomputing the head dgrad twice, plus new kernel variants tied to C=128 and alignment checks.

```diff
diff --git a/include/sdnet_hip.h b/include/sdnet_hip.h
--- a/include/sdnet_hip.h
+++ b/include/sdnet_hip.h
@@ -313,6 +313,17 @@
                 int B, int HW, int C, int Co, int accumulate, void* workspace, size_t workspace_bytes, sd_stream_t stream);
 int sd_head_bwd_bf16(const float* dy, const void* x_bf16, const float* w, void* dx_bf16, float* dw, float* dbias, int B, int HW, int C, int Co,
                      int accumulate, void* workspace, size_t workspace_bytes, sd_stream_t stream);
+
+int sd_head_tail_supported(int B, int HW, int C, int Co);
+int sd_head_fwd_bn(const float* c_nhwc, const float* mean, const float* invstd, const float* gamma, const float* beta, const float* w,
+                   const float* bias, float* y_nchw, int B, int HW, int C, int Co, sd_stream_t stream);
+int sd_head_wgrad_bn(const float* dy_nchw, const float* c_nhwc, const float* mean, const float* invstd, const float* gamma, const float* beta,
+                     float* dw, float* dbias, int B, int HW, int C, int Co, int accumulate, void* workspace, size_t workspace_bytes,
+                     sd_stream_t stream);
+size_t sd_head_bn_bwd_workspace_bytes(int B, int HW, int C, int Co);
+int sd_head_bn_bwd(const float* dhead_nchw, const float* w, const float* c_nhwc, const float* mean, const float* invstd, const float* gamma,
+                   const float* beta, float* dcv, float* dgamma, float* dbeta, int accumulate, int B, int HW, int C, int Co, void* workspace,
+                   size_t workspace_bytes, sd_stream_t stream);
 
 int sd_adam_step(float* param, const float* grad, float* exp_avg, float* exp_avg_sq, int64_t n, int step,
                  float lr, float beta1, float beta2, float eps, float grad_scale, sd_stream_t stream);
diff --git a/structuredetector_amd/_lib.py b/structuredetector_amd/_lib.py
--- a/structuredetector_amd/_lib.py
+++ b/structuredetector_amd/_lib.py
@@ -150,6 +150,11 @@
     "sd_head_bwd_workspace_bytes": (c_size, [c_int] * 4),
     "sd_head_bwd": (c_int, [c_vp] * 6 + [c_int] * 5 + [c_vp, c_size, c_vp]),
     "sd_head_bwd_bf16": (c_int, [c_vp] * 6 + [c_int] * 5 + [c_vp, c_size, c_vp]),
+    "sd_head_tail_supported": (c_int, [c_int] * 4),
+    "sd_head_fwd_bn": (c_int, [c_vp] * 8 + [c_int] * 4 + [c_vp]),
+    "sd_head_wgrad_bn": (c_int, [c_vp] * 8 + [c_int] * 5 + [c_vp, c_size, c_vp]),
+    "sd_head_bn_bwd_workspace_bytes": (c_size, [c_int] * 4),
+    "sd_head_bn_bwd": (c_int, [c_vp] * 10 + [c_int] * 5 + [c_vp, c_size, c_vp]),
     "sd_adam_step": (c_int, [c_vp, c_vp, c_vp, c_vp, c_i64, c_int, c_float, c_float, c_float, c_float, c_float, c_vp]),
     "sd_grad_sumsq_workspace_bytes": (c_size, [c_i64]),
     "sd_grad_sumsq": (c_int, [c_vp, c_i64, c_vp, c_size, c_vp]),
diff --git a/structuredetector_amd/csrc/sd_nn.hip b/structuredetector_amd/csrc/sd_nn.hip
--- a/structuredetector_amd/csrc/sd_nn.hip
+++ b/structuredetector_amd/csrc/sd_nn.hip
@@ -6,11 +6,43 @@
 
 constexpr int RED_ROWS_PER_BLOCK = 256;
 
-template <int MODE, typename T = float>
-__global__ __launch_bounds__(256) void k_col_reduce(const T* __restrict__ a, const T* __restrict__ b, const T* __restrict__ y,
-                                                     const float* __restrict__ mean, const float* __restrict__ invstd,
-                                                     const float* __restrict__ gamma, const float* __restrict__ beta, int relu,
-                                                     int64_t M, int C, float* __restrict__ partial, int rpb) {
+__device__ __forceinline__ float bn_affine(float v, float mu, float is, float ga, float be) { return (v - mu) * is * ga + be; }
+__device__ __forceinline__ float4 bn_affine4(const float4 v, const float4 mu, const float4 is, const float4 ga, const float4 be) {
+    return make_float4(bn_affine(v.x, mu.x, is.x, ga.x, be.x), bn_affine(v.y, mu.y, is.y, ga.y, be.y), bn_affine(v.z, mu.z, is.z, ga.z, be.z),
+                       bn_affine(v.w, mu.w, is.w, ga.w, be.w));
+}
+__device__ __forceinline__ void head_dgrad_term(float4& o, float g, const float4 ww) { o.x += g * ww.x; o.y += g * ww.y; o.z += g * ww.z; o.w += g * ww.w; }
+
+struct HeadSrc {
+    const float* dhead;
+    const float* w;
+    int HW, Co;
+};
+template <int NCO>
+__device__ __forceinline__ void head_src_weights(const HeadSrc& hs, int col, float4 (&wr)[NCO]) {
+#pragma unroll
+    for (int co = 0; co < NCO; ++co)
+        wr[co] = co < hs.Co ? reinterpret_cast<const float4*>(hs.w + co * 128)[col] : make_float4(0.f, 0.f, 0.f, 0.f);
+}
+template <int NCO>
+__device__ __forceinline__ float4 head_src_dy(const HeadSrc& hs, uint32_t b, uint32_t pix, const float4 (&wr)[NCO]) {
+    const float* p = hs.dhead + (int64_t)b * hs.Co * hs.HW + pix;
+    float g[NCO];
+#pragma unroll
+    for (int co = 0; co < NCO; ++co)
+        if (co < hs.Co) g[co] = p[(int64_t)co * hs.HW];
+    float4 o = make_float4(0.f, 0.f, 0.f, 0.f);
+#pragma unroll
+    for (int co = 0; co < NCO; ++co)
+        if (co < hs.Co) head_dgrad_term(o, g[co], wr[co]);
+    return o;
+}
+
+template <int MODE, typename T, int NCO>
+__device__ __forceinline__ void col_reduce_body(const T* __restrict__ a, const T* __restrict__ b, const T* __restrict__ y,
+                                                const float* __restrict__ mean, const float* __restrict__ invstd,
+                                                const float* __restrict__ gamma, const float* __restrict__ beta, int relu,
+                                                int64_t M, int C, float* __restrict__ partial, int rpb, const HeadSrc hs) {
     __shared__ float4 red[2][256];
     const int cols = C >> 2;
     const int lanes = 256 / cols;
@@ -24,10 +56,25 @@
         is = reinterpret_cast<const float4*>(invstd)[col];
         if (relu == 2) { ga = reinterpret_cast<const float4*>(gamma)[col]; be = reinterpret_cast<const float4*>(beta)[col]; }
     }
+    constexpr bool HEAD = NCO > 0;
+    float4 wr[HEAD ? NCO : 1];
+    uint32_t hb = 0, hpix = 0;
+    if constexpr (HEAD) {
+        head_src_weights(hs, col, wr);
+        hb = (uint32_t)(r0 + rl) / (uint32_t)hs.HW;
+        hpix = (uint32_t)(r0 + rl) - hb * (uint32_t)hs.HW;
+    }
     if (rl < lanes) {
 #pragma unroll 4
         for (int64_t r = r0 + rl; r < r1; r += lanes) {
-            const float4 v = ld4(a, r * cols + col);
+            float4 v;
+            if constexpr (HEAD) {
+                v = head_src_dy(hs, hb, hpix, wr);
+                hpix += (uint32_t)lanes;
+                if (hpix >= (uint32_t)hs.HW) { hpix -= (uint32_t)hs.HW; ++hb; }
+            } else {
+                v = ld4(a, r * cols + col);
+            }
             if (MODE == 0) {
                 s0.x += v.x; s0.y += v.y; s0.z += v.z; s0.w += v.w;
                 s1.x += v.x * v.x; s1.y += v.y * v.y; s1.z += v.z * v.z; s1.w += v.w * v.w;
@@ -41,8 +88,8 @@
                     g.x = yy.x > 0.f ? g.x : 0.f; g.y = yy.y > 0.f ? g.y : 0.f;
                     g.z = yy.z > 0.f ? g.z : 0.f; g.w = yy.w > 0.f ? g.w : 0.f;
                 } else if (relu == 2) {
-                    g.x = ((xv.x - mu.x) * is.x * ga.x + be.x) > 0.f ? g.x : 0.f; g.y = ((xv.y - mu.y) * is.y * ga.y + be.y) > 0.f ? g.y : 0.f;
-                    g.z = ((xv.z - mu.z) * is.z * ga.z + be.z) > 0.f ? g.z : 0.f; g.w = ((xv.w - mu.w) * is.w * ga.w + be.w) > 0.f ? g.w : 0.f;
+                    const float4 o = bn_affine4(xv, mu, is, ga, be);
+                    g.x = o.x > 0.f ? g.x : 0.f; g.y = o.y > 0.f ? g.y : 0.f; g.z = o.z > 0.f ? g.z : 0.f; g.w = o.w > 0.f ? g.w : 0.f;
                 } else if (relu == 3) {
                     const uint8_t mb = reinterpret_cast<const uint8_t*>(y)[r * cols + col];
                     g.x = (mb & 1) ? g.x : 0.f; g.y = (mb & 2) ? g.y : 0.f; g.z = (mb & 4) ? g.z : 0.f; g.w = (mb & 8) ? g.w : 0.f;
@@ -66,6 +113,22 @@
         reinterpret_cast<float4*>(dst)[col] = s0;
         reinterpret_cast<float4*>(dst + C)[col] = s1;
     }
+}
+
+template <int MODE, typename T = float>
+__global__ __launch_bounds__(256) void k_col_reduce(const T* __restrict__ a, const T* __restrict__ b, const T* __restrict__ y,
+                                                     const float* __restrict__ mean, const float* __restrict__ invstd,
+                                                     const float* __restrict__ gamma, const float* __restrict__ beta, int relu,
+                                                     int64_t M, int C, float* __restrict__ partial, int rpb) {
+    col_reduce_body<MODE, T, 0>(a, b, y, mean, invstd, gamma, beta, relu, M, C, partial, rpb, HeadSrc{});
+}
+
+template <int NCO>
+__global__ __launch_bounds__(256) void k_col_reduce_head(const float* __restrict__ x, const float* __restrict__ mean,
+                                                          const float* __restrict__ invstd, const float* __restrict__ gamma,
+                                                          const float* __restrict__ beta, int64_t M, float* __restrict__ partial, int rpb,
+                                                          const HeadSrc hs) {
+    col_reduce_body<1, float, NCO>((const float*)nullptr, x, (const float*)nullptr, mean, invstd, gamma, beta, 2, M, 128, partial, rpb, hs);
 }
 
 __global__ __launch_bounds__(256) void k_rows_fold(const float* __restrict__ in, int rows, int W, int slab, float* __restrict__ out) {
@@ -208,9 +271,7 @@
             mu = reinterpret_cast<const float4*>(mean)[col]; is = reinterpret_cast<const float4*>(invstd)[col];
             g = reinterpret_cast<const float4*>(gamma)[col]; b = reinterpret_cast<const float4*>(beta)[col];
         }
-        float4 o;
-        o.x = (v.x - mu.x) * is.x * g.x + b.x; o.y = (v.y - mu.y) * is.y * g.y + b.y;
-        o.z = (v.z - mu.z) * is.z * g.z + b.z; o.w = (v.w - mu.w) * is.w * g.w + b.w;
+        float4 o = bn_affine4(v, mu, is, g, b);
         if (res) {
             const float4 r = ld4(res, i);
             o.x += r.x; o.y += r.y; o.z += r.z; o.w += r.w;
@@ -230,12 +291,12 @@
     shift[c] = beta[c] - rm[c] * s;
 }
 
-template <typename T>
-__global__ __launch_bounds__(256) void k_bn_bwd_apply(const T* __restrict__ dy, const T* __restrict__ x, const T* __restrict__ y,
-                                                       int relu, int64_t n4, int C, const float* __restrict__ mean,
-                                                       const float* __restrict__ invstd, const float* __restrict__ gamma,
-                                                       const float* __restrict__ beta, const float* __restrict__ mg,
-                                                       const float* __restrict__ mgx, T* __restrict__ dx, T* __restrict__ g_out) {
+template <typename T, int NCO>
+__device__ __forceinline__ void bn_bwd_apply_body(const T* __restrict__ dy, const T* __restrict__ x, const T* __restrict__ y,
+                                                  int relu, int64_t n4, int C, const float* __restrict__ mean,
+                                                  const float* __restrict__ invstd, const float* __restrict__ gamma,
+                                                  const float* __restrict__ beta, const float* __restrict__ mg,
+                                                  const float* __restrict__ mgx, T* __restrict__ dx, T* __restrict__ g_out, const HeadSrc hs) {
     const int64_t stride = (int64_t)gridDim.x * 256;
     const int cols = C >> 2;
     const bool fixed = stride % cols == 0;
@@ -244,8 +305,24 @@
     float4 ga = reinterpret_cast<const float4*>(gamma)[col0];
     float4 be = relu == 2 ? reinterpret_cast<const float4*>(beta)[col0] : make_float4(0.f, 0.f, 0.f, 0.f);
     float4 a = reinterpret_cast<const float4*>(mg)[col0], b = reinterpret_cast<const float4*>(mgx)[col0];
+    constexpr bool HEAD = NCO > 0;
+    float4 wr[HEAD ? NCO : 1];
+    uint32_t hb = 0, hpix = 0, hdb = 0, hdp = 0;
+    if constexpr (HEAD) {
+        head_src_weights(hs, col0, wr);
+        const uint32_t row = (uint32_t)(((int64_t)blockIdx.x * 256 + threadIdx.x) >> 5), drow = (uint32_t)(stride >> 5);
+        hb = row / (uint32_t)hs.HW; hpix = row - hb * (uint32_t)hs.HW;
+        hdb = drow / (uint32_t)hs.HW; hdp = drow - hdb * (uint32_t)hs.HW;
+    }
     for (int64_t i = (int64_t)blockIdx.x * 256 + threadIdx.x; i < n4; i += stride) {
-        float4 g = ld4(dy, i);
+        float4 g;
+        if constexpr (HEAD) {
+            g = head_src_dy(hs, hb, hpix, wr);
+            hb += hdb; hpix += hdp;
+            if (hpix >= (uint32_t)hs.HW) { hpix -= (uint32_t)hs.HW; ++hb; }
+        } else {
+            g = ld4(dy, i);
+        }
         const float4 xv = ld4(x, i);
         if (!fixed) {
             const int col = (int)(i % cols);
@@ -261,8 +338,8 @@
             const uint8_t mb = reinterpret_cast<const uint8_t*>(y)[i];
             g.x = (mb & 1) ? g.x : 0.f; g.y = (mb & 2) ? g.y : 0.f; g.z = (mb & 4) ? g.z : 0.f; g.w = (mb & 8) ? g.w : 0.f;
         } else if (relu == 2) {
-            g.x = ((xv.x - mu.x) * is.x * ga.x + be.x) > 0.f ? g.x : 0.f; g.y = ((xv.y - mu.y) * is.y * ga.y + be.y) > 0.f ? g.y : 0.f;
-            g.z = ((xv.z - mu.z) * is.z * ga.z + be.z) > 0.f ? g.z : 0.f; g.w = ((xv.w - mu.w) * is.w * ga.w + be.w) > 0.f ? g.w : 0.f;
+            const float4 o = bn_affine4(xv, mu, is, ga, be);
+            g.x = o.x > 0.f ? g.x : 0.f; g.y = o.y > 0.f ? g.y : 0.f; g.z = o.z > 0.f ? g.z : 0.f; g.w = o.w > 0.f ? g.w : 0.f;
         }
         float4 o;
         o.x = ga.x * is.x * (g.x - a.x - (xv.x - mu.x) * is.x * b.x);
@@ -272,6 +349,24 @@
         st4(dx, i, o);
         if (g_out) st4(g_out, i, g);
     }
+}
+
+template <typename T>
+__global__ __launch_bounds__(256) void k_bn_bwd_apply(const T* __restrict__ dy, const T* __restrict__ x, const T* __restrict__ y,
+                                                       int relu, int64_t n4, int C, const float* __restrict__ mean,
+                                                       const float* __restrict__ invstd, const float* __restrict__ gamma,
+                                                       const float* __restrict__ beta, const float* __restrict__ mg,
+                                                       const float* __restrict__ mgx, T* __restrict__ dx, T* __restrict__ g_out) {
+    bn_bwd_apply_body<T, 0>(dy, x, y, relu, n4, C, mean, invstd, gamma, beta, mg, mgx, dx, g_out, HeadSrc{});
+}
+
+template <int NCO>
+__global__ __launch_bounds__(256) void k_bn_bwd_apply_head(const float* __restrict__ x, int64_t n4, const float* __restrict__ mean,
+                                                            const float* __restrict__ invstd, const float* __restrict__ gamma,
+                                                            const float* __restrict__ beta, const float* __restrict__ mg,
+                                                            const float* __restrict__ mgx, float* __restrict__ dx, const HeadSrc hs) {
+    bn_bwd_apply_body<float, NCO>((const float*)nullptr, x, (const float*)nullptr, 2, n4, 128, mean, invstd, gamma, beta, mg, mgx, dx,
+                                   (float*)nullptr, hs);
 }
 
 __global__ __launch_bounds__(256) void k_maxpool_fwd(const float* __restrict__ x, float* __restrict__ y, uint8_t* __restrict__ idx, int B,
@@ -722,8 +817,15 @@
 }
 
 constexpr int HF_NST = 4;
-__global__ __launch_bounds__(256) void k_head_fwd_f32_c128(const float* __restrict__ x, const float* __restrict__ w, const float* __restrict__ bias,
-                                                            float* __restrict__ y, int HW, int Co, int ntiles) {
+struct BnParams4 { const float* mean; const float* invstd; const float* gamma; const float* beta; };
+__device__ __forceinline__ f32x4 ldp4(const float* p, int c) { return *reinterpret_cast<const f32x4*>(p + c); }
+__device__ __forceinline__ f32x4 bn_relu_frag(const f32x4 v, const f32x4 mu, const f32x4 is, const f32x4 ga, const f32x4 be) {
+    return f32x4{fmaxf(bn_affine(v[0], mu[0], is[0], ga[0], be[0]), 0.f), fmaxf(bn_affine(v[1], mu[1], is[1], ga[1], be[1]), 0.f),
+                 fmaxf(bn_affine(v[2], mu[2], is[2], ga[2], be[2]), 0.f), fmaxf(bn_affine(v[3], mu[3], is[3], ga[3], be[3]), 0.f)};
+}
+template <bool BN>
+__device__ __forceinline__ void head_fwd_f32_c128_body(const float* __restrict__ x, const BnParams4 bn, const float* __restrict__ w,
+                                                       const float* __restrict__ bias, float* __restrict__ y, int HW, int Co, int ntiles) {
     extern __shared__ __attribute__((aligned(16))) float hf_lds[];
     const int lane = threadIdx.x & 63, wave = __builtin_amdgcn_readfirstlane(threadIdx.x >> 6);
     float* const T = hf_lds + wave * (HF_NST * 2048);
@@ -736,6 +838,14 @@
         if (row < Co) bw[j] = *reinterpret_cast<const f32x4*>(w + row * 128 + 16 * j + 4 * kq);
     }
     const float bv = row < Co ? bias[row] : 0.f;
+    f32x4 pmu[BN ? 8 : 1], pis[BN ? 8 : 1], pga[BN ? 8 : 1], pbe[BN ? 8 : 1];
+    if constexpr (BN) {
+#pragma unroll
+        for (int j = 0; j < 8; ++j) {
+            const int c = 16 * j + 4 * kq;
+            pmu[j] = ldp4(bn.mean, c); pis[j] = ldp4(bn.invstd, c); pga[j] = ldp4(bn.gamma, c); pbe[j] = ldp4(bn.beta, c);
+        }
+    }
     const int nwaves = gridDim.x * 4;
     const int dr = lane >> 5, dsl = lane & 31;
 #define HF_ISSUE(t_, st_)                                                                                          \
@@ -760,6 +870,10 @@
         for (int j = 0; j < 8; ++j) a[j] = lds_read128_async<0>(a0 + (uint32_t)(((4 * j + kq) ^ row) << 4));
         SD_LDS_WAIT4(0, a[0], a[1], a[2], a[3]);
         SD_LDS_WAIT4(0, a[4], a[5], a[6], a[7]);
+        if constexpr (BN) {
+#pragma unroll
+            for (int j = 0; j < 8; ++j) a[j] = bn_relu_frag(a[j], pmu[j], pis[j], pga[j], pbe[j]);
+        }
         f32x4 acc0 = {0.f, 0.f, 0.f, 0.f}, acc1 = {0.f, 0.f, 0.f, 0.f};
 #pragma unroll
         for (int j = 0; j < 8; j += 2)
@@ -778,6 +892,14 @@
     }
     wait_vmcnt<0>();
 #undef HF_ISSUE
+}
+__global__ __launch_bounds__(256) void k_head_fwd_f32_c128(const float* __restrict__ x, const float* __restrict__ w, const float* __restrict__ bias,
+                                                            float* __restrict__ y, int HW, int Co, int ntiles) {
+    head_fwd_f32_c128_body<false>(x, BnParams4{}, w, bias, y, HW, Co, ntiles);
+}
+__global__ __launch_bounds__(256) void k_head_fwd_bn_f32_c128(const float* __restrict__ x, const BnParams4 bn, const float* __restrict__ w,
+                                                               const float* __restrict__ bias, float* __restrict__ y, int HW, int Co, int ntiles) {
+    head_fwd_f32_c128_body<true>(x, bn, w, bias, y, HW, Co, ntiles);
 }
 
 constexpr int HEAD_WG_PIX = 1024;
@@ -806,7 +928,7 @@
         for (int co = 0; co < Co; ++co) {
             const float g = gs[co][row];
             const float4 ww = *reinterpret_cast<const float4*>(ws + co * C + col * 4);
-            o.x += g * ww.x; o.y += g * ww.y; o.z += g * ww.z; o.w += g * ww.w;
+            head_dgrad_term(o, g, ww);
         }
         if constexpr (sizeof(T) == 2) {
             uint2 pk;
@@ -952,8 +1074,9 @@
 }
 
 constexpr int HWG_STAGE = 2048 + 256;
-__global__ __launch_bounds__(256) void k_head_wgrad_f32_c128(const float* __restrict__ dy, const float* __restrict__ x, float* __restrict__ partial,
-                                                              int HW, int Co, int ntiles) {
+template <bool BN>
+__device__ __forceinline__ void head_wgrad_f32_c128_body(const float* __restrict__ dy, const float* __restrict__ x, const BnParams4 bn,
+                                                         float* __restrict__ partial, int HW, int Co, int ntiles) {
     extern __shared__ __attribute__((aligned(16))) float hw_lds[];
     const int lane = threadIdx.x & 63, wave = __builtin_amdgcn_readfirstlane(threadIdx.x >> 6);
     float* const T = hw_lds + wave * (HF_NST * HWG_STAGE);
@@ -962,6 +1085,14 @@
     const int gw = blockIdx.x * 4 + wave, nwaves = gridDim.x * 4;
     const int dr = lane >> 5, dsl = lane & 31;
     const int nco = min(n, Co - 1);
+    f32x4 pmu[2], pis[2], pga[2], pbe[2];
+    if constexpr (BN) {
+#pragma unroll
+        for (int h = 0; h < 2; ++h) {
+            const int c = 64 * h + 4 * n;
+            pmu[h] = ldp4(bn.mean, c); pis[h] = ldp4(bn.invstd, c); pga[h] = ldp4(bn.gamma, c); pbe[h] = ldp4(bn.beta, c);
+        }
+    }
 #define HWG_ISSUE(t_, st_)                                                                                         \
     {                                                                                                              \
         const uint32_t m0_ = (uint32_t)min((t_), ntiles - 1) * 16u;                              \
@@ -997,6 +1128,13 @@
         SD_LDS_WAIT4(0, xb[0], xb[1], xb[2], xb[3]);
         SD_LDS_WAIT2(0, a, xa[0]);
         if (n >= Co) a = f32x4{0.f, 0.f, 0.f, 0.f};
+        if constexpr (BN) {
+#pragma unroll
+            for (int i = 0; i < 4; ++i) {
+                xa[i] = bn_relu_frag(xa[i], pmu[0], pis[0], pga[0], pbe[0]);
+                xb[i] = bn_relu_frag(xb[i], pmu[1], pis[1], pga[1], pbe[1]);
+            }
+        }
 #pragma unroll
         for (int i = 0; i < 4; ++i)
 #pragma unroll
@@ -1021,6 +1159,14 @@
     bsum += __shfl_xor(bsum, 16);
     bsum += __shfl_xor(bsum, 32);
     if (kq == 0 && n < Co) dst[Co * 128 + n] = bsum;
+}
+__global__ __launch_bounds__(256) void k_head_wgrad_f32_c128(const float* __restrict__ dy, const float* __restrict__ x, float* __restrict__ partial,
+                                                              int HW, int Co, int ntiles) {
+    head_wgrad_f32_c128_body<false>(dy, x, BnParams4{}, partial, HW, Co, ntiles);
+}
+__global__ __launch_bounds__(256) void k_head_wgrad_bn_f32_c128(const float* __restrict__ dy, const float* __restrict__ x, const BnParams4 bn,
+                                                                 float* __restrict__ partial, int HW, int Co, int ntiles) {
+    head_wgrad_f32_c128_body<true>(dy, x, bn, partial, HW, Co, ntiles);
 }
 
 __global__ __launch_bounds__(256) void k_head_wgrad_fin(const float* __restrict__ partial, int nblocks, int n, float* __restrict__ dw,
@@ -2145,6 +2291,89 @@
     return 0;
 }
 
+int sd_head_tail_supported(int B, int HW, int C, int Co) {
+    return B > 0 && HW > 0 && C == 128 && Co > 0 && Co <= 16 && HW % 16 == 0 && (int64_t)B * HW < (1ll << 31);
+}
+
+static int head_tail_check(const char* what, int B, int HW, int C, int Co) {
+    SD_REQUIRE(sd_head_tail_supported(B, HW, C, Co), SD_ERR_INVALID,
+               "%s: needs C == 128, 1 <= Co <= 16, HW %% 16 == 0 and B * HW < 2^31 (got B=%d HW=%d C=%d Co=%d)", what, B, HW, C, Co);
+    return 0;
+}
+
+int sd_head_fwd_bn(const float* c, const float* mean, const float* invstd, const float* gamma, const float* beta, const float* w,
+                   const float* bias, float* y, int B, int HW, int C, int Co, sd_stream_t stream) {
+    SD_REQUIRE(c && mean && invstd && gamma && beta && w && bias && y, SD_ERR_INVALID, "sd_head_fwd_bn: null pointer");
+    if (int e = head_tail_check("sd_head_fwd_bn", B, HW, C, Co)) return e;
+    SD_REQUIRE(aligned16(c) && aligned16(mean) && aligned16(invstd) && aligned16(gamma) && aligned16(beta) && aligned16(w) && aligned16(y),
+               SD_ERR_INVALID, "sd_head_fwd_bn: c, the BatchNorm vectors, w and y must be 16-byte aligned");
+    const int ntiles = (int)((int64_t)B * HW / 16);
+    const size_t lds_b = (size_t)4 * HF_NST * 2048 * sizeof(float);
+    static const hipError_t attr_once = hipFuncSetAttribute(reinterpret_cast<const void*>(&k_head_fwd_bn_f32_c128), hipFuncAttributeMaxDynamicSharedMemorySize, (int)lds_b);
+    SD_HIP(attr_once);
+    hipLaunchKernelGGL(k_head_fwd_bn_f32_c128, dim3(std::min(cdiv(ntiles, 4), 256)), dim3(256), lds_b, (hipStream_t)stream, c,
+                       BnParams4{mean, invstd, gamma, beta}, w, bias, y, HW, Co, ntiles);
+    SD_LAUNCH_CHECK();
+    return 0;
+}
+
+int sd_head_wgrad_bn(const float* dy, const float* c, const float* mean, const float* invstd, const float* gamma, const float* beta, float* dw,
+                     float* dbias, int B, int HW, int C, int Co, int accumulate, void* workspace, size_t workspace_bytes, sd_stream_t stream) {
+    SD_REQUIRE(dy && c && mean && invstd && gamma && beta && dw && dbias && workspace, SD_ERR_INVALID, "sd_head_wgrad_bn: null pointer");
+    if (int e = head_tail_check("sd_head_wgrad_bn", B, HW, C, Co)) return e;
+    SD_REQUIRE(aligned16(dy) && aligned16(c) && aligned16(mean) && aligned16(invstd) && aligned16(gamma) && aligned16(beta), SD_ERR_INVALID,
+               "sd_head_wgrad_bn: dy, c and the BatchNorm vectors must be 16-byte aligned");
+    SD_REQUIRE(workspace_bytes >= sd_head_bwd_workspace_bytes(B, HW, C, Co), SD_ERR_WORKSPACE, "sd_head_wgrad_bn: workspace too small");
+    const int64_t M = (int64_t)B * HW;
+    hipStream_t st = (hipStream_t)stream;
+    const int nb = head_wgrad_wave_rows(M);
+    const size_t lds_b = (size_t)4 * HF_NST * HWG_STAGE * sizeof(float);
+    static const hipError_t attr_once = hipFuncSetAttribute(reinterpret_cast<const void*>(&k_head_wgrad_bn_f32_c128), hipFuncAttributeMaxDynamicSharedMemorySize, (int)lds_b);
+    SD_HIP(attr_once);
+    hipLaunchKernelGGL(k_head_wgrad_bn_f32_c128, dim3(nb / 4), dim3(256), lds_b, st, dy, c, BnParams4{mean, invstd, gamma, beta}, (float*)workspace,
+                       HW, Co, (int)(M / 16));
+    SD_LAUNCH_CHECK();
+    const int n = Co * C + Co;
+    hipLaunchKernelGGL(k_head_wgrad_fin, dim3(cdiv(n, 8)), dim3(256), 0, st, (const float*)workspace, nb, n, dw, dbias, Co * C, accumulate);
+    SD_LAUNCH_CHECK();
+    return 0;
+}
+
+size_t sd_head_bn_bwd_workspace_bytes(int B, int HW, int C, int Co) {
+    (void)Co;
+    return sd_col_reduce_workspace_bytes((int64_t)B * HW, C);
+}
+
+int sd_head_bn_bwd(const float* dhead, const float* w, const float* c, const float* mean, const float* invstd, const float* gamma,
+                   const float* beta, float* dcv, float* dgamma, float* dbeta, int accumulate, int B, int HW, int C, int Co, void* workspace,
+                   size_t workspace_bytes, sd_stream_t stream) {
+    SD_REQUIRE(dhead && w && c && mean && invstd && gamma && beta && dcv && dgamma && dbeta && workspace, SD_ERR_INVALID,
+               "sd_head_bn_bwd: null pointer");
+    if (int e = head_tail_check("sd_head_bn_bwd", B, HW, C, Co)) return e;
+    SD_REQUIRE(aligned16(w) && aligned16(c) && aligned16(mean) && aligned16(invstd) && aligned16(gamma) && aligned16(beta) && aligned16(dcv) &&
+               aligned16(workspace), SD_ERR_INVALID, "sd_head_bn_bwd: w, c, the BatchNorm vectors, dcv and the workspace must be 16-byte aligned");
+    SD_REQUIRE(workspace_bytes >= sd_head_bn_bwd_workspace_bytes(B, HW, C, Co), SD_ERR_WORKSPACE, "sd_head_bn_bwd: workspace too small");
+    const int64_t M = (int64_t)B * HW;
+    hipStream_t st = (hipStream_t)stream;
+    const HeadSrc hs{dhead, w, HW, Co};
+    const int rpb = red_rows(M), nb = cdiv(M, rpb);
+    float* partial = (float*)workspace;
+    float* mg = partial + (size_t)nb * 2 * C;
+    float* mgx = mg + C;
+    if (Co <= 8) hipLaunchKernelGGL(k_col_reduce_head<8>, dim3(nb), dim3(256), 0, st, c, mean, invstd, gamma, beta, M, partial, rpb, hs);
+    else hipLaunchKernelGGL(k_col_reduce_head<16>, dim3(nb), dim3(256), 0, st, c, mean, invstd, gamma, beta, M, partial, rpb, hs);
+    SD_LAUNCH_CHECK();
+    int rows = nb;
+    const float* fin = fold_partials(partial, rows, C, mgx + C, st);
+    bn_bwd_finish(fin, rows, M, C, dgamma, dbeta, accumulate, mg, mgx, nullptr, st);
+    SD_LAUNCH_CHECK();
+    const int64_t n4 = M * C / 4;
+    if (Co <= 8) hipLaunchKernelGGL(k_bn_bwd_apply_head<8>, dim3(ew_grid(n4)), dim3(256), 0, st, c, n4, mean, invstd, gamma, beta, mg, mgx, dcv, hs);
+    else hipLaunchKernelGGL(k_bn_bwd_apply_head<16>, dim3(ew_grid(n4)), dim3(256), 0, st, c, n4, mean, invstd, gamma, beta, mg, mgx, dcv, hs);
+    SD_LAUNCH_CHECK();
+    return 0;
+}
+
 int sd_head_bwd_bf16(const float* dy, const void* x_bf16, const float* w, void* dx_bf16, float* dw, float* dbias, int B, int HW, int C, int Co,
                      int accumulate, void* workspace, size_t workspace_bytes, sd_stream_t stream) {
     SD_REQUIRE(dy && x_bf16 && w && dx_bf16 && dw && dbias && workspace && B > 0 && HW > 0, SD_ERR_INVALID, "sd_head_bwd_bf16: bad arguments");
diff --git a/structuredetector_amd/model/network.py b/structuredetector_amd/model/network.py
--- a/structuredetector_amd/model/network.py
+++ b/structuredetector_amd/model/network.py
@@ -117,6 +117,7 @@
         self.overlap_wgrad = False
         self._side = None
         self.fuse_bn_bwd = False
+        self.head_tail_fused = True
         self._wt_plan, self._wt_flat, self._wt_valid = None, {}, None
         self._head_ok = {}
         self.stem_ring = True
@@ -277,6 +278,14 @@
         if update_running:
             self._nbt.append(bn.num_batches_tracked)
         return (y, mean, invstd, mask) if want_mask else (y, mean, invstd)
+
+    def _head_tail_ok(self, training, amp, sync, B, HW, bn: BNParams):
+        hc = self.net.head.conv
+        if not (self.head_tail_fused and training and not amp and sync is None):
+            return False
+        if any(t.data_ptr() % 16 for t in (bn.weight, bn.bias, hc.weight)):
+            return False
+        return bool(self.lib.sd_head_tail_supported(B, HW, hc.cin, hc.cout))
 
     def bn_fold(self, bn: BNParams):
         cached = self.net._folded.get(id(bn))
@@ -386,11 +395,17 @@
         T.push("fwd:fpn")
         f, _ = self.conv(p5, net.up1, B, H5, W5, shift=net.up1.bias, amp=amp, sb=not training)
         fpn_tape = []
+        tail = None
         for fpn, (sc_t, Hs, Ws) in ((net.up2, (p4, H4, W4)), (net.up3, (p3, H3, W3)), (net.up4, (p2, H2, W2))):
             t, dl = self.conv(sc_t, fpn.lateral, B, Hs, Ws, shift=fpn.lateral.bias, res=f, res_up2=True, amp=amp, sb=not training)
             if training:
                 c, dc, stf = self.conv_stats(t, fpn.conv[0], B, Hs, Ws, fpn.conv[1], amp=amp, sync=sx)
-                fn, mf, if_ = self.bn_train(c, fpn.conv[1], stats=stf)
+                if fpn is net.up4 and self._head_tail_ok(training, amp, sx, B, Hs * Ws, fpn.conv[1]):
+                    (mf, if_), fn = stf, None
+                    self._nbt.append(fpn.conv[1].num_batches_tracked)
+                    tail = (c, mf, if_, fpn.conv[1])
+                else:
+                    fn, mf, if_ = self.bn_train(c, fpn.conv[1], stats=stf)
                 if rec:
                     fpn_tape.append((fpn, sc_t, (Hs, Ws), dl, t, dc, c, mf, if_, fn))
             else:
@@ -402,9 +417,14 @@
         T.push("fwd:head")
         hc = net.head.conv
         out = torch.empty((B, hc.cout, H2, W2), dtype=torch.float32, device=x.device)
-        head_fwd = lib.sd_head_fwd_bf16 if amp else lib.sd_head_fwd
-        L.check(head_fwd(f.data_ptr(), hc.weight.data_ptr(), hc.bias.data_ptr(), out.data_ptr(), B, H2 * W2, hc.cin, hc.cout,
-                         L.stream()), "sd_head_fwd")
+        if tail is not None:
+            c, mf, if_, bnf = tail
+            L.check(lib.sd_head_fwd_bn(c.data_ptr(), mf.data_ptr(), if_.data_ptr(), bnf.weight.data_ptr(), bnf.bias.data_ptr(), hc.weight.data_ptr(),
+                                       hc.bias.data_ptr(), out.data_ptr(), B, H2 * W2, hc.cin, hc.cout, L.stream()), "sd_head_fwd_bn")
+        else:
+            head_fwd = lib.sd_head_fwd_bf16 if amp else lib.sd_head_fwd
+            L.check(head_fwd(f.data_ptr(), hc.weight.data_ptr(), hc.bias.data_ptr(), out.data_ptr(), B, H2 * W2, hc.cin, hc.cout,
+                             L.stream()), "sd_head_fwd")
         T.pop()
         if rec:
             tape.update(blocks=blocks_tape, fpn=fpn_tape, p5=(p5, H5, W5), f1=f, B=B, hw=(H2, W2))
@@ -671,7 +691,21 @@
         T.push("bwd:fpn_head")
         self._transpose_all(amp)
         ws = self._ws(lib.sd_head_bwd_workspace_bytes(B, H2 * W2, hc.cin, hc.cout), dhead.device)
-        if amp and hc.cin in (64, 128) and hc.cout <= 8:
+        dcv_tail = None
+        if tape["f1"] is None:
+            fpn, c, mf, if_ = tape["fpn"][-1][0], *tape["fpn"][-1][6:9]
+            bnf = fpn.conv[1]
+            L.check(lib.sd_head_wgrad_bn(dhead.data_ptr(), c.data_ptr(), mf.data_ptr(), if_.data_ptr(), bnf.weight.data_ptr(), bnf.bias.data_ptr(),
+                                         net.grad_of(hc.weight).data_ptr(), net.grad_of(hc.bias).data_ptr(), B, H2 * W2, hc.cin, hc.cout, 0,
+                                         ws.data_ptr(), ws.numel(), L.stream()), "sd_head_wgrad_bn")
+            ws = self._ws(lib.sd_head_bn_bwd_workspace_bytes(B, H2 * W2, hc.cin, hc.cout), dhead.device)
+            dcv_tail = torch.empty_like(c)
+            L.check(lib.sd_head_bn_bwd(dhead.data_ptr(), hc.weight.data_ptr(), c.data_ptr(), mf.data_ptr(), if_.data_ptr(), bnf.weight.data_ptr(),
+                                       bnf.bias.data_ptr(), dcv_tail.data_ptr(), net.grad_of(bnf.weight).data_ptr(),
+                                       net.grad_of(bnf.bias).data_ptr(), 0, B, H2 * W2, hc.cin, hc.cout, ws.data_ptr(), ws.numel(), L.stream()),
+                    "sd_head_bn_bwd")
+            df = None
+        elif amp and hc.cin in (64, 128) and hc.cout <= 8:
             f1 = tape["f1"]
             df = torch.empty_like(f1)
             L.check(lib.sd_head_bwd_bf16(dhead.data_ptr(), f1.data_ptr(), hc.weight.data_ptr(), df.data_ptr(), net.grad_of(hc.weight).data_ptr(),
@@ -688,7 +722,10 @@
 
         lateral_grad = {}
         for (fpn, sc_t, (Hs, Ws), dl, t, dc, c, mf, if_, fn) in reversed(tape["fpn"]):
-            dcv, _ = self._bn_bwd(df, c, fn, 2, fpn.conv[1], mf, if_, sync=sx)
+            if dcv_tail is not None:
+                dcv, dcv_tail = dcv_tail, None
+            else:
+                dcv, _ = self._bn_bwd(df, c, fn, 2, fpn.conv[1], mf, if_, sync=sx)
             dt = self._dgrad(dcv, fpn.conv[0], dc)
             self._wgrad(dcv, t, fpn.conv[0], dc)
             self._wgrad(dt, sc_t, fpn.lateral, dl)
```

Result: no change. 877.8 (median of 6 runs) (+0.5%).
